# uzh-rpg/ess

Measured on AMD Instinct MI355X. Metric: UDA train-step throughput (voxel grids/s = N*B*T/step_time), higher is better.
Workload: dtype f16 forward / bf16 backward

## Files before the change

ess_amd/csrc/conv_bf16.hip:

```cpp
#include "conv_bf16_common.h"
#include <atomic>

namespace {

using namespace essconv;

__global__ void pack_weights_bf16_kernel(const float* w, const float* w2, __bf16* out, int64_t total, int cot, int ck,
                                         int n_chunks, int ks, int cin, int cout, int epi, int hid, int w_kind, int split, int f16) {
  const int64_t i = (int64_t)blockIdx.x * blockDim.x + threadIdx.x;
  if (i >= total) return;
  int64_t t = i;
  const int kp = t & 7; t >>= 3;
  const int col = t % cot; t /= cot;
  const int cb8 = ck >> 3;
  const int cb = t % cb8; t /= cb8;
  const int tap = t % (ks * ks); t /= ks * ks;
  int lo = 0;
  if (split) { lo = (int)(t & 1); t >>= 1; }
  const int ch = t % n_chunks;
  const int ct = t / n_chunks;
  const int c = ch * ck + cb * 8 + kp;
  int sel;
  const int row = map_row(ct * cot + col, epi, hid, cout, &sel);
  float v = 0.f;
// ... 339 lines not shown
    const size_t lds2 = 2 * (size_t)pl.lds_bytes;
    WidePick wp;
    if (wide_pick(d, pl, g, a, c8, &wp)) {
      ConvKArgs t = a;
      t.tiles_x = wp.tiles_x; t.n_tiles = wp.tiles_x * wp.tiles_y;
      const int cus = tuning().cus;
      t.persist = wp.tiles > cus ? 1 : 0;
      t.slab = pl.cout_tile;
      conv_bf16_launch_wide(wp.mbw, wp.cw, d->epilogue, dim3((unsigned)(wp.tiles > cus ? cus : wp.tiles)), st, t);
      return ess_launch_status("conv2d_forward(bf16, wide tile)");
    }
    if (lds2 <= 160 * 1024) {
      static const int persist = [] { const char* e = getenv("ESS_WS_PERSIST"); return e ? atoi(e) : 1; }();
      const int per_cu_lds = (int)((160 * 1024) / lds2), per_cu = (mb == 4 ? 1 : 2) < per_cu_lds ? (mb == 4 ? 1 : 2) : per_cu_lds;
      const int slots = tuning().cus * per_cu;
      if (persist && (int)grid.x > slots) {
        ConvKArgs t = a;
        t.persist = 1;
        conv_bf16_launch_ws(mb, d->epilogue, c8, dim3((unsigned)slots), lds2, st, t);
        return ess_launch_status("conv2d_forward(bf16, wave-specialised, persistent)");
      }
      conv_bf16_launch_ws(mb, d->epilogue, c8, grid, lds2, st, a);
      return ess_launch_status("conv2d_forward(bf16, wave-specialised)");
    }
  }
  const int key = d->ksize * 10 + d->stride;
  ESS_CHECK_ARG(!a.split || split_generic, "conv(bf16): split operands reached the generic tile kernel (k%d s%d, %zu B of LDS for two stages)",
                d->ksize, d->stride, 2 * (size_t)pl.lds_bytes);
  if (c8)
    ESS_CHECK_ARG(d->epilogue == ESS_EPI_LINEAR && (key == 11 || key == 12 || key == 31 || key == 32),
                  "conv(bf16): the generic tile kernel stages BF16_C8 sources for 1x1 and 3x3 LINEAR convolutions only");
  ESS_CHECK_ARG(key == 11 || key == 12 || key == 31 || key == 32 || key == 51 || key == 52 || key == 71 || key == 72,
                "conv: no kernel for k%d s%d", d->ksize, d->stride);
  conv_bf16_launch_generic(key, mb, pl.ck / 8, d->epilogue, c8, grid, pl.lds_bytes, st, a);
  return ess_launch_status("conv2d_forward(bf16)");
}

}
```

ess_amd/csrc/conv_bf16_generic.hip:

```cpp
#include "conv_bf16_common.h"

namespace {

using namespace essconv;

template <int KS, int S, int MB, int EPI, int CB8, bool SRCBF = false, bool H = false>
__global__ __launch_bounds__(256) void conv_bf16_kernel(const ConvKArgs a) {
  static_assert(!H || SRCBF, "half operands come as F16_C8 tensors");
  extern __shared__ __attribute__((aligned(16))) u32x4 smem16[];
  constexpr int COT = MB * 32;
  constexpr int CK = CB8 * 8;
  constexpr int KPC = kpc(KS, S);
  constexpr int WSZ = KS * KS * CB8 * COT;
  constexpr int WV = (WSZ + 255) / 256;
  constexpr bool WPRE = WV <= 5;
  const int tid = threadIdx.x, lane = tid & 63, wave = tid >> 6, half = lane >> 5, p = lane & 31;
  const int BW = 1 << a.bwl, WX = 1 << a.wxl, RB = 32 >> a.bwl;
  const int TW = WX << a.bwl, TH = (4 >> a.wxl) * NBW * RB;
  const int logical = xcd_remap(blockIdx.x, gridDim.x);
  const int ct = logical % a.n_cout_tiles;
  const int sp = logical / a.n_cout_tiles;
  const int tile = sp % a.n_tiles, n = sp / a.n_tiles;
  const int ty = tile / a.tiles_x, tx = tile - ty * a.tiles_x;
  const int y0 = ty * TH, x0 = tx * TW;
  u32x4* in_t = smem16;
  u32x4* w_t = smem16 + CB8 * a.plane;

  const int ox = p & (BW - 1), oy = p >> a.bwl;
  const int wx = wave & (WX - 1), wy = wave >> a.wxl;
  const int lx = wx * BW + ox;
  int ly[NBW], boff[NBW];
#pragma unroll
  for (int nb = 0; nb < NBW; ++nb) {
    ly[nb] = (wy * NBW + nb) * RB + oy;
    boff[nb] = half * a.plane + ly[nb] * S * a.row_pitch + lx;
  }

  f32x16 acc[MB][NBW];
#pragma unroll
  for (int mb = 0; mb < MB; ++mb)
#pragma unroll
// ... 33 lines not shown
    }
  }
  struct Raw8 { float v[8]; };
  struct Pre { typename std::conditional<SRCBF, u32x4, Raw8>::type d; };
  const size_t hw0 = pl0 / 4, hw1 = pl1 / 4;
  const int nb0 = (a.C0 + 7) >> 3, nb1 = (a.C1 + 7) >> 3;
  const u32x4* s0 = (const u32x4*)a.src0 + (size_t)n * nb0 * hw0;
  const u32x4* s1 = a.C1 ? (const u32x4*)a.src1 + (size_t)n * nb1 * hw1 : s0;
  auto load_vec = [&](int ch, int cb, int k) -> Pre {
    const int c0 = ch * CK + cb * 8;
    const bool first = c0 < a.C0 || a.C1 == 0;
    Pre r;
    if constexpr (SRCBF) {
      const int bi = (first ? c0 : c0 - a.C0) >> 3, nbs = first ? nb0 : nb1;
      const u32x4* sp = (first ? s0 : s1) + (size_t)(bi < nbs ? bi : 0) * (first ? hw0 : hw1);
      r.d = sp[first ? v_o0[k] : v_o1[k]];
    } else {
      const unsigned pls = first ? pl0 : pl1;
      const unsigned cbase = (unsigned)(first ? c0 : c0 - a.C0) * pls;
      const unsigned off = (first ? v_o0[k] : v_o1[k]) + cbase;
#pragma unroll
      for (int j = 0; j < 8; ++j)
        r.d.v[j] = __builtin_bit_cast(float, __builtin_amdgcn_raw_buffer_load_b32(first ? r0 : r1, (int)(off + j * pls), 0, 0));
    }
    return r;
  };
  auto to_lds = [&](int ch, int cb, int k, const Pre& r, bool x_lo = false) -> u32x4 {
    if constexpr (SRCBF) {
      const int c0 = ch * CK + cb * 8;
      const bool first = c0 < a.C0 || a.C1 == 0;
      const unsigned blk_ok = ((first ? c0 : c0 - a.C0) >> 3) < (first ? nb0 : nb1) ? 0xffffffffu : 0u;
      const unsigned m = (first ? v_k0[k] : v_k1[k]) & blk_ok;
      u32x4 v = r.d;
      v[0] &= m; v[1] &= m; v[2] &= m; v[3] &= m;
      return v;
    } else {
      if (x_lo) {
        float lo[8];
#pragma unroll
        for (int j = 0; j < 8; ++j) lo[j] = r.d.v[j] - (float)(__bf16)r.d.v[j];
        return pack8(lo);
      }
      return pack8(r.d.v);
    }
  };

  Pre pre[CB8][KPC];
  u32x4 wpre[WPRE ? WV : 1];
  const bool split = !SRCBF && a.split;
  const int nvc = split ? 3 * a.n_chunks : a.n_chunks;
  const u32x4* wbase = (const u32x4*)a.wpk + (size_t)ct * a.n_chunks * WSZ * (split ? 2 : 1);
  auto wslab = [&](int vc) { return split ? 2 * (vc / 3) + ((vc % 3) == 2 ? 1 : 0) : vc; };
#pragma unroll
  for (int cb = 0; cb < CB8; ++cb)
#pragma unroll
    for (int k = 0; k < KPC; ++k) pre[cb][k] = load_vec(0, cb, k);
  if constexpr (WPRE) {
#pragma unroll
    for (int it = 0; it < WV; ++it) { const int i = tid + it * 256; wpre[it] = wbase[i < WSZ ? i : 0]; }
  }

  for (int vc = 0; vc < nvc; ++vc) {
    const int ch = split ? vc / 3 : vc;
    const bool x_lo = split && (vc - 3 * ch) == 1;
    __syncthreads();
#pragma unroll
// ... 46 lines not shown
#pragma unroll
            for (int nb = 0; nb < NBW; ++nb)
              acc[mb][nb] = ess_mfma16<H>(af[mb], bfr[nb], acc[mb][nb]);
        }
      }
    }
  }
  conv_epilogue<MB, EPI, true, H>(a, acc, ct, n, half, x0 + lx, y0, ly);
}

template <int KS, int S, int MB, int CB8>
void launch_epi(int epi, dim3 grid, size_t lds, hipStream_t st, const ConvKArgs& a) {
  if constexpr (KS == 3 && S == 1) {
    switch (epi) {
      case ESS_EPI_LSTM: { ess_allow_lds(conv_bf16_kernel<KS, S, MB, ESS_EPI_LSTM, CB8>, lds); hipLaunchKernelGGL((conv_bf16_kernel<KS, S, MB, ESS_EPI_LSTM, CB8>), grid, dim3(256), lds, st, a); } return;
      case ESS_EPI_GRU_UR: { ess_allow_lds(conv_bf16_kernel<KS, S, MB, ESS_EPI_GRU_UR, CB8>, lds); hipLaunchKernelGGL((conv_bf16_kernel<KS, S, MB, ESS_EPI_GRU_UR, CB8>), grid, dim3(256), lds, st, a); } return;
      case ESS_EPI_GRU_OUT: { ess_allow_lds(conv_bf16_kernel<KS, S, MB, ESS_EPI_GRU_OUT, CB8>, lds); hipLaunchKernelGGL((conv_bf16_kernel<KS, S, MB, ESS_EPI_GRU_OUT, CB8>), grid, dim3(256), lds, st, a); } return;
      default: break;
    }
  }
  { ess_allow_lds(conv_bf16_kernel<KS, S, MB, ESS_EPI_LINEAR, CB8>, lds); hipLaunchKernelGGL((conv_bf16_kernel<KS, S, MB, ESS_EPI_LINEAR, CB8>), grid, dim3(256), lds, st, a); }
}

template <int KS, int S, int MB, int CB8>
void launch_c8(dim3 grid, size_t lds, hipStream_t st, const ConvKArgs& a) {
  if (a.f16) {
    ess_allow_lds(conv_bf16_kernel<KS, S, MB, ESS_EPI_LINEAR, CB8, true, true>, lds);
    hipLaunchKernelGGL((conv_bf16_kernel<KS, S, MB, ESS_EPI_LINEAR, CB8, true, true>), grid, dim3(256), lds, st, a);
    return;
  }
  ess_allow_lds(conv_bf16_kernel<KS, S, MB, ESS_EPI_LINEAR, CB8, true>, lds);
  hipLaunchKernelGGL((conv_bf16_kernel<KS, S, MB, ESS_EPI_LINEAR, CB8, true>), grid, dim3(256), lds, st, a);
}
template <int KS, int S>
void launch_mb_c8(int mb, int cb8, dim3 grid, size_t lds, hipStream_t st, const ConvKArgs& a) {
  if constexpr (KS == 1 && S == 1) {
    if (cb8 == 4) {
      if (mb == 2) launch_c8<KS, S, 2, 4>(grid, lds, st, a);
      else launch_c8<KS, S, 1, 4>(grid, lds, st, a);
      return;
    }
  }
  if (mb == 2) launch_c8<KS, S, 2, 2>(grid, lds, st, a);
  else launch_c8<KS, S, 1, 2>(grid, lds, st, a);
}

template <int KS, int S>
void launch_mb(int mb, int cb8, int epi, dim3 grid, size_t lds, hipStream_t st, const ConvKArgs& a) {
  if constexpr (KS == 1 && S == 1) {
    if (cb8 == 4) {
      if (mb == 2) launch_epi<KS, S, 2, 4>(epi, grid, lds, st, a);
      else launch_epi<KS, S, 1, 4>(epi, grid, lds, st, a);
      return;
    }
  }
  if (mb == 2) launch_epi<KS, S, 2, 2>(epi, grid, lds, st, a);
  else launch_epi<KS, S, 1, 2>(epi, grid, lds, st, a);
}
}

namespace essconv {

void conv_bf16_launch_generic(int key, int mb, int cb8, int epi, bool c8, dim3 grid, size_t lds, hipStream_t st, const ConvKArgs& a) {
  if (c8) {
    switch (key) {
      case 11: launch_mb_c8<1, 1>(mb, cb8, grid, lds, st, a); break;
      case 12: launch_mb_c8<1, 2>(mb, cb8, grid, lds, st, a); break;
      case 31: launch_mb_c8<3, 1>(mb, cb8, grid, lds, st, a); break;
      default: launch_mb_c8<3, 2>(mb, cb8, grid, lds, st, a); break;
// ... 17 lines not shown
```

ess_amd/csrc/conv_common.h:

```cpp
#pragma once
#include "common.h"
#include <stdlib.h>

#ifndef ESS_EPI_AUX
#define ESS_EPI_AUX 2
#endif
#ifndef ESS_GRU_AUX
#define ESS_GRU_AUX 2
#endif
#ifndef ESS_C8_AUX
#define ESS_C8_AUX 0
#endif
namespace essconv {

constexpr int NBW = 2;

struct ConvKArgs {
  const float* src0;
  const float* src1;
  const void* wpk;
  const float* scale;
  const float* shift;
  const float* residual;
  const float* aux0;
  const float* aux1;
  float* out;
  float* out2;
  int N, Hin, Win, C0, C1, mode0, mode1;
  int Cout, Hout, Wout, pad;
  int bwl, wxl, tiles_x, n_tiles, n_cout_tiles;
  int IH, IW, row_pitch, par_off, plane;
  int ck, n_chunks;
  int act, hid, out_split;
  void* out_bf;
  int fmt0, fmt1;
  int fmt_out;
  int fmt_res;
  int out_f16;
  int persist;
  int slab;
  int split;
  int deep;
  int f16;
  int hilo;
};

template <bool H> __device__ __forceinline__ uint2 ess_cvt4(float v0, float v1, float v2, float v3);
template <bool H> __device__ __forceinline__ void ess_up4(uint2 r, float (&f)[4]);


#ifndef ESS_EPI_STAMP
#define ESS_EPI_STAMP(i_) do { } while (0)
#endif
typedef __amdgpu_buffer_rsrc_t ess_rsrc;
constexpr unsigned ESS_OOB = 0x80000000u;
__device__ __forceinline__ ess_rsrc ess_make_rsrc(const void* p, size_t bytes) {
  return __builtin_amdgcn_make_buffer_rsrc((void*)p, 0, (int)(unsigned)bytes, 0x00020000);
}
__device__ __forceinline__ _Float16 ess_f16_sat(float v) {
  const float c = __builtin_amdgcn_fmed3f(v, -65504.f, 65504.f);
  return (_Float16)(v != v ? v : c);
}
template <> __device__ __forceinline__ uint2 ess_cvt4<false>(float v0, float v1, float v2, float v3) {
  typedef __bf16 bf16x4 __attribute__((ext_vector_type(4)));
  bf16x4 b;
  b[0] = (__bf16)v0; b[1] = (__bf16)v1; b[2] = (__bf16)v2; b[3] = (__bf16)v3;
  return __builtin_bit_cast(uint2, b);
}
template <> __device__ __forceinline__ uint2 ess_cvt4<true>(float v0, float v1, float v2, float v3) {
  typedef _Float16 f16x4 __attribute__((ext_vector_type(4)));
  f16x4 h;
  h[0] = ess_f16_sat(v0); h[1] = ess_f16_sat(v1); h[2] = ess_f16_sat(v2); h[3] = ess_f16_sat(v3);
  return __builtin_bit_cast(uint2, h);
}
__device__ __forceinline__ uint2 ess_cvt4_lo(float v0, float v1, float v2, float v3) {
  typedef _Float16 f16x4 __attribute__((ext_vector_type(4)));
  f16x4 h;
// ... 1253 lines not shown
          if (S == 1) {
            int rp = IW;
            if (BW == 16) while (rp & 15) ++rp;
            if (BW == 8) while ((rp & 15) != 8) ++rp;
            g.row_pitch = rp; g.par_off = 0;
          } else {
            int pw = (IW + 1) / 2;
            if (BW == 16) while (pw & 3) ++pw;
            if (BW == 8) while ((pw & 3) != 2) ++pw;
            g.row_pitch = 2 * pw; g.par_off = pw;
          }
          g.plane = IH * g.row_pitch;
        } else {
          if (S == 1) {
            int rp = IW;
            if (BW < 32) while ((rp & 31) != BW) ++rp;
            g.row_pitch = rp; g.par_off = 0;
          } else {
            int pw = (IW + 1) / 2;
            if (BW < 32) while (((4 * pw) & 31) != BW) ++pw;
            g.row_pitch = 2 * pw; g.par_off = pw;
          }
          g.plane = (IH * g.row_pitch + 3) & ~3;
        }
        best = g;
      }
    }
  }
  return best;
}

inline int validate(const EssConvDesc* d) {
  ESS_CHECK_ARG(d != nullptr, "conv: null descriptor");
  if (d->compute == ESS_COMPUTE_F16) {
    ESS_CHECK_ARG(d->fmt0 != ESS_FMT_BF16_C8 && d->fmt1 != ESS_FMT_BF16_C8 && d->fmt_out != ESS_FMT_BF16_C8 && d->fmt_res != ESS_FMT_BF16_C8,
                  "conv(f16): 16-bit tensors of a half-operand convolution are ESS_FMT_F16_C8");
    ESS_CHECK_ARG(d->act != ESS_ACT_SUMPOOL2 || d->epilogue != ESS_EPI_LINEAR, "conv(f16): no pooled (data-gradient) form");
    ESS_CHECK_ARG(d->mode0 != ESS_SRC_ZERO_UP2 && d->mode1 != ESS_SRC_ZERO_UP2, "conv(f16): no zero-inserted sources");
    if (d->epilogue == ESS_EPI_LINEAR && d->fmt_out == ESS_FMT_F16_C8_HILO) {
      ESS_CHECK_ARG(d->out_split == 0 && (d->act == ESS_ACT_NONE || d->act == ESS_ACT_RELU) && (d->C_out % 64) == 0,
                    "conv(f16): a [hi | lo] output needs act in {none, relu}, no out_split, C_out %% 64 == 0");
      const ResolvedDesc rt = resolve_compute(d);
      const int cot = pick_mb(&rt.d) * 32;
      ESS_CHECK_ARG((d->C_out % cot) == 0, "conv(f16): a [hi | lo] output needs whole channel tiles: C_out %d is not a multiple of the plan's %d-channel tile",
                    d->C_out, cot);
    }
    if (d->epilogue == ESS_EPI_LSTM) ESS_CHECK_ARG(d->act == 0 || d->act == ESS_LSTM_H_HILO, "conv(f16, LSTM): act is 0 or ESS_LSTM_H_HILO");
    if (d->epilogue == ESS_EPI_GRU_UR) ESS_CHECK_ARG(d->act == ESS_GRU_U_F32 || d->act == ESS_GRU_U_F16, "conv(f16, GRU_UR): act is ESS_GRU_U_F32 or ESS_GRU_U_F16");
    const ResolvedDesc r = resolve_compute(d);
    return validate(&r.d);
  }
  ESS_CHECK_ARG(d->fmt_out != ESS_FMT_F16_C8_HILO, "conv: ESS_FMT_F16_C8_HILO is an output format of ESS_COMPUTE_F16");
  ESS_CHECK_ARG(d->N > 0 && d->H_in > 0 && d->W_in > 0 && d->C0 > 0 && d->C1 >= 0 && d->C_out > 0, "conv: bad extents");
  ESS_CHECK_ARG(d->ksize == 1 || d->ksize == 3 || d->ksize == 5 || d->ksize == 7, "conv: ksize %d unsupported", d->ksize);
  ESS_CHECK_ARG(d->stride == 1 || d->stride == 2, "conv: stride %d unsupported", d->stride);
  ESS_CHECK_ARG(d->H_out == (d->H_in + 2 * d->pad - d->ksize) / d->stride + 1 &&
                    d->W_out == (d->W_in + 2 * d->pad - d->ksize) / d->stride + 1,
                "conv: output extent %dx%d inconsistent with input %dx%d k%d s%d p%d", d->H_out, d->W_out, d->H_in,
                d->W_in, d->ksize, d->stride, d->pad);
  for (int s = 0; s < 2; ++s) {
    const int m = s ? d->mode1 : d->mode0;
    ESS_CHECK_ARG(m >= 0 && m <= (s ? 2 : 3), "conv: bad source mode");
    if (m == ESS_SRC_NEAREST_UP2 || m == ESS_SRC_ZERO_UP2) ESS_CHECK_ARG(!(d->H_in & 1) && !(d->W_in & 1), "conv: x2 source needs even extent");
  }
  if (d->mode0 == ESS_SRC_S2D)
    ESS_CHECK_ARG(d->ksize == 3 && d->stride == 1 && d->pad == 1 && d->C1 == 0 && (d->C0 % 128) == 0 && (d->C_out % 64) == 0 &&
// ... 150 lines not shown
```

ess_amd/csrc/conv_fwd.hip:

```cpp
#include "conv_common.h"

namespace {

using namespace essconv;

constexpr int kpc32(int ks, int s) { return stage_kpc(ks, s); }
constexpr unsigned OOB32 = 0x80000000u;

template <int KS, int S, int MB, int EPI, int CB>
__global__ __launch_bounds__(256) void conv_f32_kernel(const ConvKArgs a) {
  extern __shared__ __attribute__((aligned(16))) float smem[];
  constexpr int COT = MB * 32;
  constexpr int KPC = kpc32(KS, S);
  constexpr int WSZ = KS * KS * CB * COT;
  constexpr int WV = (WSZ / 4 + 255) / 256;
  const int tid = threadIdx.x, lane = tid & 63, wave = tid >> 6, half = lane >> 5, p = lane & 31;
  const int BW = 1 << a.bwl, WX = 1 << a.wxl, RB = 32 >> a.bwl;
  const int TW = WX << a.bwl, TH = (4 >> a.wxl) * NBW * RB;
  const int logical = xcd_remap(blockIdx.x, gridDim.x);
  const int ct = logical % a.n_cout_tiles;
  const int sp = logical / a.n_cout_tiles;
  const int tile = sp % a.n_tiles, n = sp / a.n_tiles;
  const int ty = tile / a.tiles_x, tx = tile - ty * a.tiles_x;
  const int y0 = ty * TH, x0 = tx * TW;
// ... 157 lines not shown
  const ResolvedDesc rd = resolve_compute(d);
  d = &rd.d;
  EssConvPlan pl;
  make_plan(d, &pl, rd.split);
  if (is_bf16(d)) return conv_bf16_pack_weights(d, pl, w_kind, w, w2, packed, (hipStream_t)stream, rd.split, rd.f16);
  const int64_t total = pl.packed_elems;
  hipLaunchKernelGGL(pack_weights_kernel, dim3((unsigned)ceil_div64(total, 256)), dim3(256), 0, (hipStream_t)stream, w, w2,
                     (float*)packed, total, pl.cout_tile, pl.ck, pl.n_chunks, d->ksize, d->C0 + d->C1, d->C_out, d->epilogue,
                     d->hidden, w_kind);
  return ess_launch_status("pack_weights");
}

extern "C" int ess_conv2d_pack_weights_multi(const EssConvDesc* descs, const int32_t* w_kinds, const float* const* w,
                                             void* const* packed, int32_t count, ess_stream_t stream) {
  ESS_CHECK_ARG(descs && w_kinds && w && packed && count > 0, "pack_weights_multi: bad arguments");
  return conv_bf16_pack_weights_multi(descs, w_kinds, w, packed, count, (hipStream_t)stream);
}

extern "C" int ess_conv2d_pack_rows(const EssConvDesc* d, const float* v, const float* v2, float fill, float* packed,
                                    ess_stream_t stream) {
  int rc = validate(d);
  if (rc) return rc;
  ESS_CHECK_ARG(v && packed, "pack_rows: null pointer");
  ESS_CHECK_ARG(d->epilogue != ESS_EPI_GRU_UR || v2, "pack_rows: GRU_UR needs the reset-gate vector as v2");
  const ResolvedDesc rd = resolve_compute(d);
  d = &rd.d;
  EssConvPlan pl;
  make_plan(d, &pl, rd.split);
  hipLaunchKernelGGL(pack_rows_kernel, dim3(ceil_div(pl.rows_padded, 256)), dim3(256), 0, (hipStream_t)stream, v, v2, fill,
                     packed, pl.rows_padded, d->epilogue, d->hidden, d->C_out);
  return ess_launch_status("pack_rows");
}

extern "C" int ess_conv2d_forward(const EssConvDesc* d, const void* src0, const void* src1, const void* packed_w,
                                  const float* scale, const float* shift, const void* residual, const float* aux0,
                                  const float* aux1, void* out, void* out2, void* out_bf16, ess_stream_t stream) {
  EssConvDesc dcopy;
  bool out_f16 = false;
  if (d && d->fmt_out == ESS_FMT_F16_C8 && d->compute != ESS_COMPUTE_F16) {
    ESS_CHECK_ARG(d->act != ESS_ACT_SUMPOOL2 && d->out_split == 0 && (d->fmt_res == ESS_FMT_F32_NCHW || d->fmt_res == ESS_FMT_BF16_C8),
                  "conv: an F16_C8 output takes no SUMPOOL2 / out_split; a residual comes as BF16_C8");
    dcopy = *d;
    dcopy.fmt_out = ESS_FMT_BF16_C8;
    if (residual) dcopy.fmt_res = ESS_FMT_BF16_C8;
    d = &dcopy;
    out_f16 = true;
  }
  int rc = validate(d);
  if (rc) return rc;
  const ResolvedDesc rd = resolve_compute(d);
  d = &rd.d;
  ESS_CHECK_ARG(src0 && packed_w, "conv: null pointer");
  ESS_CHECK_ARG(d->mode0 != ESS_SRC_S2D || (d->fmt0 == ESS_FMT_BF16_C8 && d->fmt_out == ESS_FMT_BF16_C8), "conv: an ESS_SRC_S2D source is a BF16_C8 tensor, and so is the output");
  ESS_CHECK_ARG(out || (out_bf16 && d->out_split == 0 && (d->epilogue == ESS_EPI_LINEAR || d->epilogue == ESS_EPI_LSTM || d->epilogue == ESS_EPI_GRU_OUT)),
                "conv: `out` may only be NULL when the BF16_C8 copy is requested (LINEAR / LSTM / GRU_OUT epilogues)");
  ESS_CHECK_ARG(d->C1 == 0 || src1, "conv: second source missing");
  if (d->epilogue != ESS_EPI_LINEAR) ESS_CHECK_ARG(shift && !scale && !residual, "conv: a recurrent epilogue takes a bias (shift) and no scale / residual");
  if (d->epilogue == ESS_EPI_LSTM) ESS_CHECK_ARG(out2, "conv: the LSTM epilogue needs the second output (c')");
  if (d->epilogue == ESS_EPI_GRU_UR) ESS_CHECK_ARG(out2 || out_bf16 || !aux0, "conv: GRU_UR needs an output for r*h (out2 or out_bf16)");
  if (d->epilogue == ESS_EPI_GRU_OUT) ESS_CHECK_ARG(aux1, "conv: GRU_OUT needs u (aux1); h_prev (aux0) may be NULL = zeros");
  if (d->out_split > 0) ESS_CHECK_ARG(out2, "conv: out_split needs out2");
  if (out_bf16)
    ESS_CHECK_ARG(d->compute == ESS_COMPUTE_BF16 && d->out_split == 0, "conv: the BF16_C8 output copy exists for bf16 compute, no out_split");
  if (d->act == ESS_ACT_SUMPOOL2)
    ESS_CHECK_ARG(out && !scale && !residual && !out_bf16, "conv: SUMPOOL2 takes no scale / residual / BF16_C8 copy");
  if (d->fmt_out == ESS_FMT_BF16_C8) {
    ESS_CHECK_ARG(out && !out_bf16, "conv: a BF16_C8 output goes to `out` (no separate copy)");
    ESS_CHECK_ARG(((((uintptr_t)out) | ((uintptr_t)out2) | ((uintptr_t)residual)) & 15) == 0, "conv: BF16_C8 tensors must be 16-byte aligned");
  }
  ESS_CHECK_ARG(!residual || d->fmt_res == d->fmt_out, "conv: the residual must come in the output's format");
  EssConvPlan pl;
  make_plan(d, &pl, rd.split);
  ESS_CHECK_ARG(pl.lds_bytes <= 160 * 1024, "conv: LDS tile %d B exceeds 160 KiB", pl.lds_bytes);
  if (d->epilogue == ESS_EPI_GRU_UR && d->act == ESS_GRU_U_F16 && d->fmt_out == ESS_FMT_F32_C8)
    ESS_CHECK_ARG(shift && d->fmt0 == ESS_FMT_BF16_C8 && (d->hidden % (pl.cout_tile / 2)) == 0 && out && !out2 && (!aux0 || d->fmt_res == ESS_FMT_F32_C8),
                  "conv(GRU_UR): an F16_C8 update gate (ESS_GRU_U_F16 with channel-blocked outputs) needs BF16_C8 sources, a bias, hidden %% %d == 0, "
                  "no fp32 r*h output and a channel-blocked h_prev", pl.cout_tile / 2);
  const Geom g = choose_geom(d);
  ConvKArgs a{};
  a.src0 = (const float*)src0; a.src1 = (const float*)src1; a.wpk = packed_w;
  a.out_bf = out_bf16; a.fmt0 = d->fmt0; a.fmt1 = d->C1 ? d->fmt1 : d->fmt0; a.scale = scale; a.shift = shift; a.residual = (const float*)residual;
  a.aux0 = aux0; a.aux1 = aux1; a.out = (float*)out; a.out2 = (float*)out2; a.fmt_out = d->fmt_out; a.fmt_res = d->fmt_res;
#ifdef ESS_ABLATE
  { static const int abl = [] { const char* b = getenv("ESS_WS_ABL"); return b ? atoi(b) & ~1 : 0; }(); a.deep = abl; }
#endif
  a.out_f16 = out_f16 ? 1 : 0;
  a.split = rd.split ? 1 : 0;
  a.f16 = rd.f16 ? 1 : 0;
  a.hilo = rd.hilo ? 1 : 0;
  if (rd.hilo && d->epilogue == ESS_EPI_LINEAR)
    ESS_CHECK_ARG(!residual && (d->C_out % pl.cout_tile) == 0 && d->fmt_out == ESS_FMT_BF16_C8, "conv(f16): a [hi | lo] output takes no residual and whole channel tiles");
  if (rd.hilo && d->epilogue == ESS_EPI_GRU_OUT)
    ESS_CHECK_ARG(out_bf16 && shift && d->fmt_res == ESS_FMT_F32_C8 && aux1 && (!out || d->fmt_out == ESS_FMT_F32_C8) && (d->hidden % pl.cout_tile) == 0,
                  "conv(f16, GRU_OUT): a [hi | lo] copy of h' exists in the straight-line form only (channel-blocked states, whole tiles of hidden channels)");
  if (rd.hilo && d->epilogue == ESS_EPI_LSTM)
    ESS_CHECK_ARG(out_bf16 && shift && d->fmt_out == ESS_FMT_F32_C8 && (!aux0 || d->fmt_res == ESS_FMT_F32_C8) && (d->hidden % (8 * (pl.cout_tile / 32))) == 0 && pl.cout_tile >= 64,
                  "conv(f16, LSTM): a [hi | lo] copy of h' exists in the lean form only (channel-blocked cell states, whole hidden blocks per tile)");
  a.N = d->N; a.Hin = d->H_in; a.Win = d->W_in; a.C0 = d->C0; a.C1 = d->C1; a.mode0 = d->mode0; a.mode1 = d->mode1;
  a.Cout = d->C_out; a.Hout = d->H_out; a.Wout = d->W_out; a.pad = d->pad;
  a.bwl = g.bwl; a.wxl = g.wxl; a.tiles_x = g.tiles_x; a.n_tiles = g.tiles_x * g.tiles_y; a.n_cout_tiles = pl.n_cout_tiles;
  a.IH = g.IH; a.IW = g.IW; a.row_pitch = g.row_pitch; a.par_off = g.par_off; a.plane = g.plane;
  a.ck = pl.ck; a.n_chunks = pl.n_chunks; a.act = d->act; a.hid = d->hidden; a.out_split = d->out_split;
  hipStream_t st = (hipStream_t)stream;
  if (is_bf16(d)) return conv_bf16_launch(d, pl, g, a, st);
  ESS_CHECK_ARG(g.IH * g.IW <= kpc32(d->ksize, d->stride) * 256, "conv: input tile of %d positions exceeds the staging capacity",
                g.IH * g.IW);
  ESS_CHECK_ARG((int64_t)(d->C0 > d->C1 ? d->C0 : d->C1) * d->H_in * d->W_in * 4 < (int64_t)1 << 31,
                "conv: one sample of a source must stay below 2 GiB (32-bit buffer offsets)");
  const dim3 grid((unsigned)(g.tiles_x * g.tiles_y * pl.n_cout_tiles * d->N));
  const int mb = pl.cout_tile / 32;
  const int key = d->ksize * 10 + d->stride;
  switch (key) {
    case 11: launch_mb<1, 1>(mb, pl.ck, d->epilogue, grid, pl.lds_bytes, st, a); break;
    case 12: launch_mb<1, 2>(mb, pl.ck, d->epilogue, grid, pl.lds_bytes, st, a); break;
    case 31: launch_mb<3, 1>(mb, pl.ck, d->epilogue, grid, pl.lds_bytes, st, a); break;
    case 32: launch_mb<3, 2>(mb, pl.ck, d->epilogue, grid, pl.lds_bytes, st, a); break;
    case 51: launch_mb<5, 1>(mb, pl.ck, d->epilogue, grid, pl.lds_bytes, st, a); break;
    case 52: launch_mb<5, 2>(mb, pl.ck, d->epilogue, grid, pl.lds_bytes, st, a); break;
    case 71: launch_mb<7, 1>(mb, pl.ck, d->epilogue, grid, pl.lds_bytes, st, a); break;
    case 72: launch_mb<7, 2>(mb, pl.ck, d->epilogue, grid, pl.lds_bytes, st, a); break;
    default: ess_set_error("conv: no kernel for k%d s%d", d->ksize, d->stride); return ESS_ENOTSUP;
  }
  return ess_launch_status("conv2d_forward");
}
```

ess_amd/csrc/conv_wgrad.hip:

```cpp
#include "conv_wgrad_common.h"
#include <stdlib.h>

namespace {


__device__ __forceinline__ float load_virtual(const WgradArgs& a, int n, int c, int gy, int gx) {
  const bool first = c < a.C0;
  const int mode = first ? a.mode0 : a.mode1;
  const int sh = mode != ESS_SRC_DIRECT ? 1 : 0;
  const int Hp = a.Hin >> sh, Wp = a.Win >> sh;
  const float* sp = first ? a.src0 : a.src1;
  const int cc = first ? c : c - a.C0, Cs = first ? a.C0 : a.C1;
  const bool ok = gy >= 0 && gy < a.Hin && gx >= 0 && gx < a.Win && !(mode == ESS_SRC_ZERO_UP2 && ((gy | gx) & 1));
  const int cy = min(max(gy, 0), a.Hin - 1) >> sh, cx = min(max(gx, 0), a.Win - 1) >> sh;
  const float t = sp[(((size_t)n * Cs + cc) * Hp + cy) * Wp + cx];
  return ok ? t : 0.f;
}

__device__ __forceinline__ void load8_virtual(const WgradArgs& a, int n, int c, int gy, int gx, bool valid, float (&f)[8]) {
  const bool first = c < a.C0;
  const int mode = first ? a.mode0 : a.mode1;
  const float* sp = first ? a.src0 : a.src1;
  const int cc = first ? c : c - a.C0, Cs = first ? a.C0 : a.C1;
  const bool rowok = valid && gy >= 0 && gy < a.Hin;
// ... 762 lines not shown
struct WPlan {
  EssConvDesc d;
  WRoute route;
  bool phases;
  WgradBArgs args;
  unsigned grid;
  int lds_bytes;
  size_t ws_bytes;
};

inline bool k3s1p1(const EssConvDesc* d) { return d->ksize == 3 && d->stride == 1 && d->pad == 1; }

inline bool s2_phases(const EssConvDesc* d) {
  return d->fmt0 == ESS_FMT_BF16_C8 && d->fmt_out == ESS_FMT_BF16_C8 && d->ksize == 3 && d->stride == 2 && d->pad == 1 && d->C1 == 0 &&
         d->mode0 == ESS_SRC_DIRECT && d->H_in == 2 * d->H_out && d->W_in == 2 * d->W_out;
}
inline EssConvDesc s2_phase_desc(const EssConvDesc* d) {
  EssConvDesc p = *d;
  p.stride = 1; p.H_in = d->H_out; p.W_in = d->W_out; p.mode1 = ESS_SRC_DIRECT;
  return p;
}
inline TapMap s2_phase_taps(int p, int q) {
  TapMap tm{};
  tm.mapped = 1;
  for (int t = 0; t < 9; ++t) {
    const int kyp = t / 3, kxp = t % 3;
    const int ky = p == 0 ? (kyp == 1 ? 1 : -1) : (kyp == 0 ? 0 : kyp == 1 ? 2 : -1);
    const int kx = q == 0 ? (kxp == 1 ? 1 : -1) : (kxp == 0 ? 0 : kxp == 1 ? 2 : -1);
    tm.m[t] = (signed char)((ky < 0 || kx < 0) ? -1 : ky * 3 + kx);
  }
  return tm;
}

int wvalidate(const EssConvDesc* d) {
  ESS_CHECK_ARG(d != nullptr, "wgrad: null descriptor");
  ESS_CHECK_ARG(d->epilogue == ESS_EPI_LINEAR && d->out_split == 0, "wgrad: only plain convolutions have a weight gradient here");
  ESS_CHECK_ARG(d->mode0 >= ESS_SRC_DIRECT && d->mode0 <= ESS_SRC_ZERO_UP2 && d->mode1 >= ESS_SRC_DIRECT && d->mode1 <= ESS_SRC_ZERO_UP2,
                "wgrad: source modes DIRECT / NEAREST_UP2 / ZERO_UP2 only (the space-to-depth form exists for the frozen encoder's forward)");
  const int cin = d->C0 + d->C1;
  const bool taps = cin == 1 && d->ksize == 7;
  ESS_CHECK_ARG(taps || d->ksize == 1 || d->ksize == 3, "wgrad: k=%d with C_in=%d unsupported", d->ksize, cin);
  ESS_CHECK_ARG(d->stride == 1 || d->stride == 2, "wgrad: stride %d unsupported", d->stride);
  const bool xc8 = d->fmt0 == ESS_FMT_BF16_C8, dc8 = d->fmt_out == ESS_FMT_BF16_C8;
  ESS_CHECK_ARG(d->compute == ESS_COMPUTE_FP32 || d->compute == ESS_COMPUTE_BF16 || d->compute == ESS_COMPUTE_BF16X3, "wgrad: bad compute type");
  if (xc8 || dc8) {
    ESS_CHECK_ARG(d->compute == ESS_COMPUTE_BF16, "wgrad: BF16_C8 tensors need bf16 compute");
    ESS_CHECK_ARG(d->C1 == 0 || d->fmt1 == d->fmt0, "wgrad: both sources of a concat must use the same format");
    ESS_CHECK_ARG(d->C1 == 0 || (d->C0 % 8) == 0, "wgrad: the first BF16_C8 source of a concat must have a multiple of 8 channels");
    if (xc8 && dc8)
      ESS_CHECK_ARG(k3s1p1(d) || (d->ksize == 1 && d->pad == 0 && d->mode0 == ESS_SRC_DIRECT && d->C1 == 0) || s2_phases(d),
                    "wgrad(BF16_C8): 3x3 / stride 1 / pad 1, 3x3 / stride 2 / pad 1 on even extents (one direct source) and 1x1 / pad 0 convolutions only");
    else if (xc8)
      ESS_CHECK_ARG(d->ksize == 1 && d->stride == 1 && d->pad == 0 && d->C1 == 0 && d->mode0 == ESS_SRC_DIRECT && d->C_out <= 32 && cin <= 32,
                    "wgrad(BF16_C8 X, fp32 dY): the 1x1 head only (C_in, C_out <= 32)");
    else
      ESS_CHECK_ARG(taps, "wgrad(fp32 X, BF16_C8 dY): the 7x7 single-channel stem only");
  }
  return ESS_OK;
}

WRoute wroute(const EssConvDesc* d) {
  const int cin = d->C0 + d->C1, KS = d->ksize;
  const bool xc8 = d->fmt0 == ESS_FMT_BF16_C8, dc8 = d->fmt_out == ESS_FMT_BF16_C8;
  if (xc8 && dc8) return KS == 3 ? W_C8_K3 : W_C8_K1;
  if (xc8) return W_SMALL1X1_C8X;
  const bool k1s1p0 = KS == 1 && d->stride == 1 && d->pad == 0;
  if (k1s1p0 && d->C1 == 0 && d->mode0 == ESS_SRC_DIRECT && d->C_out <= 16 && cin <= 64)
    return cin <= 32 && ((d->H_out * d->W_out) % 64) == 0 ? W_SMALL1X1_MFMA : W_SMALL1X1;
  const bool rows8 = (d->W_in % 8) == 0 && (d->W_out % 8) == 0 && d->mode0 != ESS_SRC_ZERO_UP2 && d->mode1 != ESS_SRC_ZERO_UP2;
  if (d->compute == ESS_COMPUTE_BF16 && k3s1p1(d)) return rows8 ? W_BF16_K3_FAST : W_BF16_K3;
  if (d->compute == ESS_COMPUTE_BF16 && k1s1p0 && rows8) return W_BF16_K1;
  if (cin == 1 && KS == 7) return W_TAPS7;
  return W_F32_TILE;
}

WPlan wplan(const EssConvDesc* desc) {
  WPlan w{};
  w.d = *desc;
  if (desc->compute == ESS_COMPUTE_BF16X3) {
    w.args.split = k3s1p1(desc);
    w.d.compute = w.args.split ? ESS_COMPUTE_BF16 : ESS_COMPUTE_FP32;
  }
  w.phases = s2_phases(&w.d);
  if (w.phases) w.d = s2_phase_desc(&w.d);
  const EssConvDesc* d = &w.d;
  w.route = wroute(d);
  WgradArgs& a = w.args.w;
  a.N = d->N; a.Hin = d->H_in; a.Win = d->W_in; a.C0 = d->C0; a.C1 = d->C1; a.mode0 = d->mode0; a.mode1 = d->mode1;
  a.Cout = d->C_out; a.Hout = d->H_out; a.Wout = d->W_out;
  a.pad = (w.route == W_BF16_K1 || w.route == W_C8_K1) ? 1 : d->pad;
  a.dy_c8 = d->fmt_out == ESS_FMT_BF16_C8;
  a.ps = w.phases;
  const int cin = d->C0 + d->C1, KS = d->ksize, S = d->stride;
  const bool wide = tile128(w.route);
  const int npx = wide ? 128 : 64;
  double best = 1e300;
  for (int twl = 5; twl >= (wide ? 4 : 3); --twl) {
    const int tw = 1 << twl, th = npx >> twl;
    const double c = (double)ceil_div(d->W_out, tw) * tw * ceil_div(d->H_out, th) * th + 1e-3 * (5 - twl);
    if (c < best) { best = c; a.twl = twl; }
  }
  if (w.route == W_C8_K3) a.twl = 4;
  const int tw = 1 << a.twl, th = npx >> a.twl;
  a.tiles_x = ceil_div(d->W_out, tw); a.tiles_y = ceil_div(d->H_out, th);
  a.ntiles = d->N * a.tiles_x * a.tiles_y;
  a.IH = (th - 1) * S + KS; a.IW = (tw - 1) * S + KS;
  a.plx = (a.IH * a.IW) | 1;
  a.ci_tiles = w.route == W_TAPS7 ? 1 : ceil_div(cin, 64);
  a.npairs = ceil_div(d->C_out, 64) * a.ci_tiles;
  const size_t slab_floats = (size_t)KS * KS * d->C_out * cin + d->C_out;
  int ns = wide ? ceil_div(256, a.npairs) : ceil_div(2048, a.npairs);
  if (ns > a.ntiles) ns = a.ntiles;
  const size_t cap = ((size_t)64 << 20) / (slab_floats * 4);
  if ((size_t)ns > cap) ns = (int)(cap ? cap : 1);
  if (ns < 1) ns = 1;
  if (w.route == W_SMALL1X1 || w.route == W_SMALL1X1_C8X) {
    const int chunks = d->N * ceil_div(d->H_out * d->W_out, 128);
    ns = chunks < 1024 ? chunks : 1024;
  } else if (w.route == W_SMALL1X1_MFMA) {
    const int groups = d->N * (d->H_out * d->W_out / 64);
    ns = groups < 4 * 512 ? ceil_div(groups, 4) : 512;
  }
  a.nsplit = ns;
  w.grid = (unsigned)(a.npairs * ns);
  w.ws_bytes = (size_t)ns * slab_floats * 4;
  w.lds_bytes = (64 * 65 + (w.route == W_TAPS7 ? a.IH * a.IW : 64 * a.plx)) * 4;
  if (wide) {
    w.args.rv = tw / 8 + 2;
    w.args.pyv = (th * tw / 8) | 1;
    w.args.pxv = ((th + 2) * w.args.rv) | 1;
    w.lds_bytes = 64 * (w.args.pyv + w.args.pxv) * 16 * (w.route == W_BF16_K3 ? 1 : 2);
  }
  return w;
}

struct WgradSet { const void* x0; const void* x1; const void* dy; };

WgradBArgs wfill(const WPlan& w, const WgradSet& s, void* workspace, bool bias, int ph) {
  WgradBArgs b = w.args;
  WgradArgs& a = b.w;
  a.src0 = (const float*)s.x0; a.src1 = a.C1 ? (const float*)s.x1 : nullptr; a.dy = (const float*)s.dy;
  a.ws = (float*)workspace;
  a.ws_b = bias ? a.ws + (size_t)a.nsplit * w.d.ksize * w.d.ksize * a.Cout * (a.C0 + a.C1) : nullptr;
  a.pp = ph >> 1; a.pq = ph & 1;
  return b;
}

template <typename K, typename... A>
int wgo(K kernel, dim3 grid, int lds_bytes, hipStream_t st, const A&... args) {
  const int rc = wgrad_raise_lds(kernel, lds_bytes);
  if (rc) return rc;
  hipLaunchKernelGGL(kernel, grid, dim3(256), lds_bytes, st, args...);
  return ESS_OK;
}

int wlaunch(const WPlan& w, WRoute route, const WgradBArgs& b, hipStream_t st) {
  const EssConvDesc& d = w.d;
  const dim3 grid(w.grid);
  const int px = d.H_out * d.W_out, nsplit = b.w.nsplit;
  int rc = ESS_OK;
  switch (route) {
    case W_F32_TILE: {
      const auto kernel = d.ksize == 3 ? (d.stride == 1 ? wgrad_f32_kernel<3, 1> : wgrad_f32_kernel<3, 2>)
                                       : (d.stride == 1 ? wgrad_f32_kernel<1, 1> : wgrad_f32_kernel<1, 2>);
      rc = wgo(kernel, grid, w.lds_bytes, st, b.w);
      break;
    }
    case W_TAPS7: rc = wgo(wgrad_taps_kernel<7, 2>, grid, w.lds_bytes, st, b.w); break;
    case W_BF16_K3: rc = wgo(wgrad_bf16_k3s1_kernel, grid, w.lds_bytes, st, b); break;
    case W_BF16_K3_FAST: rc = wgo(wgrad_bf16_k3s1_fast_kernel<9>, grid, w.lds_bytes, st, b); break;
    case W_BF16_K1: rc = wgo(wgrad_bf16_k3s1_fast_kernel<1>, grid, w.lds_bytes, st, b); break;
    case W_C8_K3: rc = wgrad_c8_k3_launch(b, grid, st); break;
    case W_C8_K1: rc = wgrad_c8_k1_launch(b, d.stride, w.lds_bytes, grid, st); break;
    case W_SMALL1X1: rc = wgo(wgrad_small1x1_kernel, dim3(nsplit), 0, st, b.w, ceil_div(px, 128), d.N * ceil_div(px, 128)); break;
// ... 29 lines not shown
  EssConvDesc c = *d;
  c.compute = ESS_COMPUTE_BF16;
  c.fmt0 = c.fmt1 = c.fmt_out = ESS_FMT_BF16_C8;
  return c;
}
struct SplitCopy { int C, H, W; size_t bytes; };
struct SplitLayout { size_t slabs, total; SplitCopy t[3]; };
SplitLayout split_layout(const EssConvDesc* d) {
  const EssConvDesc dc = c8_desc(d);
  const int s0 = d->mode0 != ESS_SRC_DIRECT ? 1 : 0, s1 = d->mode1 != ESS_SRC_DIRECT ? 1 : 0;
  SplitLayout s{(wplan(&dc).ws_bytes + 255) & ~(size_t)255, 0,
                {{d->C0, d->H_in >> s0, d->W_in >> s0, 0}, {d->C1, d->H_in >> s1, d->W_in >> s1, 0}, {d->C_out, d->H_out, d->W_out, 0}}};
  s.total = s.slabs;
  for (SplitCopy& t : s.t) {
    t.bytes = (((size_t)d->N * ((t.C + 7) / 8) * t.H * t.W * 16) + 255) & ~(size_t)255;
    s.total += 2 * t.bytes;
  }
  return s;
}

int wgrad_split_via_c8(const EssConvDesc* d, const WgradSet& s, float* dw, float* db, int accumulate, void* workspace, size_t workspace_bytes,
                       hipStream_t st);

int wgrad_run(const EssConvDesc* d, int n_sets, const WgradSet* sets, int bias_mask, float* dw, float* db, int accumulate, void* workspace,
              size_t workspace_bytes, hipStream_t st) {
  int rc = wvalidate(d);
  if (rc) return rc;
  ESS_CHECK_ARG(dw && workspace, "wgrad: null pointer");
  uintptr_t bits = 0;
  for (int q = 0; q < n_sets; ++q) {
    ESS_CHECK_ARG(sets[q].x0 && sets[q].dy, "wgrad: null pointer");
    ESS_CHECK_ARG(d->C1 == 0 || sets[q].x1, "wgrad: second source missing");
    bits |= (uintptr_t)sets[q].x0 | (uintptr_t)sets[q].dy | (d->C1 ? (uintptr_t)sets[q].x1 : 0);
  }
  if (split_via_c8(d)) {
    for (int q = 0; q < n_sets; ++q)
      if ((rc = wgrad_split_via_c8(d, sets[q], dw, ((bias_mask >> q) & 1) ? db : nullptr, q ? 1 : accumulate, workspace, workspace_bytes, st))) return rc;
    return ESS_OK;
  }
  const WPlan w = wplan(d);
  ESS_CHECK_ARG(workspace_bytes >= w.ws_bytes, "wgrad: workspace too small");
  ESS_CHECK_ARG(w.lds_bytes <= 160 * 1024, "wgrad: LDS tile %d B too large", w.lds_bytes);
  if (w.d.fmt0 == ESS_FMT_BF16_C8 || w.d.fmt_out == ESS_FMT_BF16_C8)
    ESS_CHECK_ARG((bits & 15) == 0, "wgrad: BF16_C8 tensors must be 16-byte aligned");
  if (w.route == W_TAPS7) {
    ESS_CHECK_ARG(w.d.stride == 2, "wgrad: 7x7 stem variant is stride 2 only");
    ESS_CHECK_ARG(!db, "wgrad: the stem variant has no bias gradient");
  }
  const bool one_launch = n_sets > 1 && w.route == W_C8_K3 && !w.phases;
  for (int q = 0; q < (one_launch ? 1 : n_sets); ++q) {
    const bool misaligned = (((uintptr_t)sets[q].x0 | (uintptr_t)sets[q].dy) & 15) != 0;
    const WRoute route = (w.route == W_SMALL1X1_MFMA && misaligned) ? W_SMALL1X1 : w.route;
    for (int ph = 0; ph < (w.phases ? 4 : 1); ++ph) {
      const bool bias = db && ph == 0 && (one_launch || ((bias_mask >> q) & 1));
      WgradBArgs b = wfill(w, sets[q], workspace, bias, ph);
      if (one_launch) {
        b.npass = n_sets; b.bias_mask = bias_mask;
        for (int i = 0; i < n_sets; ++i) { b.p_dy[i] = sets[i].dy; b.p_x0[i] = sets[i].x0; b.p_x1[i] = d->C1 ? sets[i].x1 : nullptr; }
      }
      if ((rc = wlaunch(w, route, b, st))) return rc;
      if ((rc = wreduce(w, b.w, dw, db, (q || accumulate) ? 1 : 0, w.phases ? s2_phase_taps(ph >> 1, ph & 1) : TapMap{}, st))) return rc;
    }
  }
  return ESS_OK;
}

int wgrad_split_via_c8(const EssConvDesc* d, const WgradSet& s, float* dw, float* db, int accumulate, void* workspace,
                              size_t workspace_bytes, hipStream_t st) {
  int rc;
  ESS_CHECK_ARG((((uintptr_t)workspace) & 255) == 0, "wgrad: the workspace must be 256-byte aligned");
  const SplitLayout sl = split_layout(d);
  ESS_CHECK_ARG(workspace_bytes >= sl.total, "wgrad: workspace too small");
  const void* src[3] = {s.x0, s.x1, s.dy};
  char* hi[3]; char* lo[3];
  char* p = (char*)workspace + sl.slabs;
  for (int i = 0; i < 3; ++i) {
    const SplitCopy& t = sl.t[i];
    hi[i] = p; lo[i] = p + t.bytes; p += 2 * t.bytes;
    if (t.C && (rc = ess_split_bf16_c8_internal((const float*)src[i], hi[i], lo[i], d->N, t.C, t.H, t.W, st))) return rc;
  }
  const EssConvDesc dc = c8_desc(d);
  const WgradSet sets[3] = {{hi[0], hi[1], hi[2]}, {lo[0], lo[1], hi[2]}, {hi[0], hi[1], lo[2]}};
  const int bias_mask = 0b101;
  static const bool fused = env_on("ESS_X3_WGRAD_FUSED");
  if (fused) return wgrad_run(&dc, 3, sets, bias_mask, dw, db, accumulate, workspace, sl.slabs, st);
  for (int q = 0; q < 3; ++q)
    if ((rc = wgrad_run(&dc, 1, &sets[q], (bias_mask >> q) & 1, dw, db, q ? 1 : accumulate, workspace, sl.slabs, st))) return rc;
  return ESS_OK;
}

}

extern "C" size_t ess_conv2d_wgrad_workspace(const EssConvDesc* d) {
  if (wvalidate(d)) return 0;
  return split_via_c8(d) ? split_layout(d).total : wplan(d).ws_bytes;
}

extern "C" int ess_conv2d_wgrad(const EssConvDesc* d, const void* src0, const void* src1, const void* dy, float* dw, float* db,
                                int accumulate, void* workspace, size_t workspace_bytes, ess_stream_t stream) {
  const WgradSet s{src0, src1, dy};
  return wgrad_run(d, 1, &s, 1, dw, db, accumulate, workspace, workspace_bytes, (hipStream_t)stream);
}

extern "C" int ess_conv2d_wgrad_sets(const EssConvDesc* d, int32_t n_sets, const void* const* src0, const void* const* src1,
                                     const void* const* dy, float* dw, float* db, int32_t accumulate, void* workspace,
                                     size_t workspace_bytes, ess_stream_t stream) {
  ESS_CHECK_ARG(d && src0 && dy && n_sets >= 1 && n_sets <= 3, "wgrad_sets: 1 to 3 sets");
  WgradSet sets[3];
  for (int q = 0; q < n_sets; ++q) {
    ESS_CHECK_ARG(src0[q] && dy[q] && (d->C1 == 0 || (src1 && src1[q])), "wgrad_sets: null tensor in set %d", q);
    sets[q] = WgradSet{src0[q], d->C1 ? src1[q] : nullptr, dy[q]};
  }
  return wgrad_run(d, n_sets, sets, (1 << n_sets) - 1, dw, db, accumulate, workspace, workspace_bytes, (hipStream_t)stream);
}
```

ess_amd/csrc/conv_wgrad_c8.hip:

```cpp
#include "conv_wgrad_common.h"
#include <stdlib.h>
#include <type_traits>

namespace {

struct Quad { u32x4w v[4]; };

__device__ __forceinline__ void quad_transpose(const Quad& q, uint2 (&out)[8]) {
#pragma unroll
  for (int d = 0; d < 4; ++d) {
    out[2 * d].x = __builtin_amdgcn_perm(q.v[1][d], q.v[0][d], 0x05040100u);
    out[2 * d].y = __builtin_amdgcn_perm(q.v[3][d], q.v[2][d], 0x05040100u);
    out[2 * d + 1].x = __builtin_amdgcn_perm(q.v[1][d], q.v[0][d], 0x07060302u);
    out[2 * d + 1].y = __builtin_amdgcn_perm(q.v[3][d], q.v[2][d], 0x07060302u);
  }
}

template <int OFF>
__device__ __forceinline__ void lds_read128(u32x4w& d, unsigned addr) {
  asm volatile("ds_read_b128 %0, %1 offset:%2" : "=v"(d) : "v"(addr), "n"(OFF));
}

template <int TAPS, int TWL>
__global__ __launch_bounds__(256) void wgrad_c8_kernel(const WgradBArgs b, int sx_abl) {
// ... 433 lines not shown
    unit(std::integral_constant<int, 22>{}, Yes{});
    unit(std::integral_constant<int, 23>{}, Yes{});
    a_addr = a_next;
    x_addr = x_next;
  }
  if (ntl > 0) {
    if (ntl - 1 < 30) ESS_TR(3 + ntl - 1);
    if (b.npass > 1) want_b = want_b0 && ((b.bias_mask >> ((split + (ntl - 1) * nsplit) / a.ntiles)) & 1);
    static_for<0, 24>([&](auto uc) { unit(uc, No{}); });
  }
  ESS_TR(34);
  const int ci = cit * 64 + ib * 32 + p, co0 = cot * 64 + cb * 32 + 4 * half;
  float* wsp = a.ws + ((size_t)split * 9 * a.Cout + co0) * Cin + ci;
  const int tap_stride = a.Cout * Cin;
  if (ci < Cin) {
#pragma unroll
    for (int r = 0; r < 16; ++r) {
      const int dco = (r & 3) + 8 * (r >> 2);
      if (co0 + dco < a.Cout) {
        float* q = wsp + dco * Cin;
#pragma unroll
        for (int t = 0; t < 9; ++t) q[t * tap_stride] = acc[t][r];
      }
    }
  }
  if (want_b) {
    bsum += __shfl_xor(bsum, 32, 64);
    const int co = cot * 64 + cb * 32 + p;
    if (half == 0 && co < a.Cout) a.ws_b[(size_t)split * a.Cout + co] = bsum;
  }
  ESS_TR(37);
}

__global__ __launch_bounds__(256) void wgrad_small1x1_c8_kernel(const WgradArgs a, int chunks_per_img, int total_chunks) {
  constexpr int P = 128, PP = P + 1;
  __shared__ float dy_s[32 * PP];
  __shared__ float x_s[32 * PP];
  float* red = dy_s;
  const int tid = threadIdx.x, lane = tid & 63, wave = tid >> 6, half = lane >> 5, p = lane & 31;
  const int Cin = a.C0, Cout = a.Cout, nbi = (Cin + 7) >> 3;
  const size_t HW = (size_t)a.Hout * a.Wout;
  f32x16 acc;
#pragma unroll
  for (int r = 0; r < 16; ++r) acc[r] = 0.f;
  float bsum = 0.f;
  for (int i = tid; i < 32 * PP; i += 256) { dy_s[i] = 0.f; x_s[i] = 0.f; }
  for (int chunk = blockIdx.x; chunk < total_chunks; chunk += gridDim.x) {
    const int n = chunk / chunks_per_img;
    const size_t px0 = (size_t)(chunk - n * chunks_per_img) * P;
    __syncthreads();
    for (int i = tid; i < nbi * P; i += 256) {
      const int blk = i / P, j = i - blk * P;
      const size_t px = px0 + j;
      const u32x4w v = ((const u32x4w*)a.src0)[((size_t)n * nbi + blk) * HW + (px < HW ? px : HW - 1)];
      const unsigned m = px < HW ? 0xffffffffu : 0u;
#pragma unroll
      for (int q = 0; q < 4; ++q) {
        x_s[(blk * 8 + 2 * q) * PP + j] = __builtin_bit_cast(float, (v[q] << 16) & m);
        x_s[(blk * 8 + 2 * q + 1) * PP + j] = __builtin_bit_cast(float, v[q] & 0xffff0000u & m);
      }
    }
    for (int i = tid; i < Cout * P; i += 256) {
      const int r = i / P, j = i - r * P;
      const size_t px = px0 + j;
      const float t = a.dy[((size_t)n * Cout + r) * HW + (px < HW ? px : HW - 1)];
      dy_s[r * PP + j] = px < HW ? t : 0.f;
    }
    __syncthreads();
    const float* dp = dy_s + p * PP + wave * 32 + half;
    const float* xp = x_s + p * PP + wave * 32 + half;
#pragma unroll 8
    for (int kk = 0; kk < 16; ++kk) {
      const float d1 = dp[2 * kk], x1 = xp[2 * kk];
      bsum += d1;
      acc = __builtin_amdgcn_mfma_f32_32x32x2f32(d1, x1, acc, 0, 0, 0);
    }
  }
  __syncthreads();
  float* redb = x_s;
#pragma unroll
  for (int r = 0; r < 16; ++r) red[wave * 1024 + r * 64 + lane] = acc[r];
  bsum += __shfl_xor(bsum, 32, 64);
  if (half == 0) redb[wave * 32 + p] = bsum;
  __syncthreads();
  for (int i = tid; i < 16 * 64; i += 256) {
    const int r = i >> 6, l = i & 63;
    const int co = (r & 3) + 8 * (r >> 2) + 4 * (l >> 5), ci = l & 31;
    if (co < Cout && ci < Cin)
      a.ws[(size_t)blockIdx.x * Cout * Cin + co * Cin + ci] = (red[i] + red[1024 + i]) + (red[2048 + i] + red[3072 + i]);
  }
  if (a.ws_b && tid < Cout) a.ws_b[(size_t)blockIdx.x * Cout + tid] = (redb[tid] + redb[32 + tid]) + (redb[64 + tid] + redb[96 + tid]);
}

}

int wgrad_c8_k3_launch(const WgradBArgs& b, dim3 grid, hipStream_t st) {
  if (b.w.twl != 4) { ess_set_error("wgrad(BF16_C8, 3x3): stride 1, 16-wide pixel tiles"); return ESS_EINVAL; }
  constexpr int NST = 4, lds = NST * DmaGeom::STAGE;
  static_assert(lds <= 160 * 1024, "LDS stages of the weight-gradient kernel");
  const int rc = wgrad_raise_lds(wgrad_c8_ws_kernel<NST>, lds);
  if (rc) return rc;
  hipLaunchKernelGGL((wgrad_c8_ws_kernel<NST>), grid, dim3(512), lds, st, b);
  return ess_launch_status("conv2d_wgrad(BF16_C8, LDS-DMA, loader waves)");
}

int wgrad_c8_k1_launch(const WgradBArgs& b, int sx, int lds_bytes, dim3 grid, hipStream_t st) {
  if (b.w.twl != 4 && b.w.twl != 5) { ess_set_error("wgrad(BF16_C8): pixel tiles are 16 or 32 wide"); return ESS_EINVAL; }
  const auto kernel = b.w.twl == 5 ? wgrad_c8_kernel<1, 5> : wgrad_c8_kernel<1, 4>;
  const int rc = wgrad_raise_lds(kernel, lds_bytes);
  if (rc) return rc;
  hipLaunchKernelGGL(kernel, grid, dim3(256), lds_bytes, st, b, sx);
  return ess_launch_status("conv2d_wgrad(BF16_C8)");
}

int wgrad_small1x1_c8_launch(const WgradArgs& a, int nsplit, hipStream_t st) {
  const int per_img = ceil_div(a.Hout * a.Wout, 128);
  hipLaunchKernelGGL(wgrad_small1x1_c8_kernel, dim3(nsplit), dim3(256), 0, st, a, per_img, a.N * per_img);
  return ess_launch_status("conv2d_wgrad(1x1 head, BF16_C8)");
}

#ifdef ESS_WG_TRACE
extern "C" int ess_debug_wgrad_trace(unsigned long long* host_out, size_t n) {
  return (int)hipMemcpyFromSymbol(host_out, HIP_SYMBOL(g_wg_trace), n * sizeof(unsigned long long));
}
#endif
```

ess_amd/csrc/conv_wgrad_common.h:

```cpp
#pragma once
#include "common.h"

struct WgradArgs {
  const float* src0;
  const float* src1;
  const float* dy;
  float* ws;
  float* ws_b;
  int N, Hin, Win, C0, C1, mode0, mode1, Cout, Hout, Wout, pad;
  int twl;
  int tiles_x, tiles_y, ntiles;
  int IH, IW, plx;
  int ci_tiles, npairs, nsplit;
  int dy_c8;
  int ps, pp, pq;
};

constexpr unsigned OOBW = 0x80000000u;
typedef __bf16 bf16x8w __attribute__((ext_vector_type(8)));
typedef unsigned int u32x4w __attribute__((ext_vector_type(4)));


__device__ __forceinline__ u32x4w cvt8(const float (&v)[8]) {
  bf16x8w b;
#pragma unroll
  for (int j = 0; j < 8; ++j) b[j] = (__bf16)v[j];
  return __builtin_bit_cast(u32x4w, b);
}
__device__ __forceinline__ u32x4w cvt8_lo(const float (&v)[8]) {
  bf16x8w b;
#pragma unroll
  for (int j = 0; j < 8; ++j) b[j] = (__bf16)(v[j] - (float)(__bf16)v[j]);
  return __builtin_bit_cast(u32x4w, b);
}
__device__ __forceinline__ u32x4w shift_left1(u32x4w lo, u32x4w hi) {
  u32x4w r;
  r[0] = __builtin_amdgcn_alignbyte(hi[0], lo[3], 2);
  r[1] = __builtin_amdgcn_alignbyte(hi[1], hi[0], 2);
  r[2] = __builtin_amdgcn_alignbyte(hi[2], hi[1], 2);
  r[3] = __builtin_amdgcn_alignbyte(hi[3], hi[2], 2);
  return r;
}
__device__ __forceinline__ u32x4w shift_right1(u32x4w lo, u32x4w hi) {
  u32x4w r;
  r[0] = __builtin_amdgcn_alignbyte(lo[1], lo[0], 2);
  r[1] = __builtin_amdgcn_alignbyte(lo[2], lo[1], 2);
  r[2] = __builtin_amdgcn_alignbyte(lo[3], lo[2], 2);
  r[3] = __builtin_amdgcn_alignbyte(hi[0], lo[3], 2);
// ... 32 lines not shown
```

ess_amd/csrc/norm_c8.hip:

```cpp
#include <atomic>
#include "common.h"
#include <stdlib.h>

#ifndef ESS_REDUCE1_U
#define ESS_REDUCE1_U 4
#endif
namespace {

typedef unsigned int u32x4n __attribute__((ext_vector_type(4)));
typedef __bf16 bf16x8n __attribute__((ext_vector_type(8)));

__device__ __forceinline__ void unpack8(u32x4n v, float (&f)[8]) {
#pragma unroll
  for (int q = 0; q < 4; ++q) {
    f[2 * q] = __builtin_bit_cast(float, v[q] << 16);
    f[2 * q + 1] = __builtin_bit_cast(float, v[q] & 0xffff0000u);
  }
}
__device__ __forceinline__ void unpack8h(u32x4n v, float (&f)[8]) {
  typedef _Float16 f16x2n __attribute__((ext_vector_type(2)));
#pragma unroll
  for (int q = 0; q < 4; ++q) {
    const unsigned w = v[q];
    const f16x2n h = __builtin_bit_cast(f16x2n, w);
// ... 389 lines not shown
  for (int j = 0; j < 8; ++j) {
    const double a = wave_sum_d(s0[j]), b = wave_sum_d(s1[j]);
    if (lane == 0) { redd[w * 16 + 2 * j] = a; redd[w * 16 + 2 * j + 1] = b; }
  }
  __syncthreads();
  if (threadIdx.x < 16) {
    double t = 0;
    for (int i = 0; i < 4; ++i) t += redd[i * 16 + threadIdx.x];
    sums[((size_t)g * nsl + sl) * 16 + threadIdx.x] = t;
  }
}

__device__ __forceinline__ void group_total8(const double* sums, int g, int nsl, double (&t0)[8], double (&t1)[8]) {
  __shared__ double part[64 * 16];
  __shared__ double tot[16];
  const int j = threadIdx.x & 15, k0 = threadIdx.x >> 4, ng = blockDim.x >> 4;
  {
    const double* p = sums + (size_t)g * nsl * 16 + j;
    double t = 0;
    for (int k = k0; k < nsl; k += ng) t += p[(size_t)k * 16];
    part[k0 * 16 + j] = t;
  }
  __syncthreads();
  if (threadIdx.x < 16) {
    double t = 0;
    for (int i = 0; i < ng; ++i) t += part[i * 16 + threadIdx.x];
    tot[threadIdx.x] = t;
  }
  __syncthreads();
#pragma unroll
  for (int jj = 0; jj < 8; ++jj) { t0[jj] = tot[2 * jj]; t1[jj] = tot[2 * jj + 1]; }
}

__global__ __launch_bounds__(256) void in_apply_c8_kernel(const u32x4n* __restrict__ x, const u32x4n* __restrict__ res,
                                                          u32x4n* __restrict__ y, float* __restrict__ stats, const double* sums,
                                                          int nsl, int CB, int C, int hw, float eps, int relu) {
  const int xf16 = relu >> 8;
  relu &= 0xff;
  const int g = blockIdx.x, n = g / CB, cb = g - n * CB;
  double t0[8], t1[8];
  group_total8(sums, g, nsl, t0, t1);
  float mean[8], rstd[8];
#pragma unroll
  for (int j = 0; j < 8; ++j) {
    const double m = t0[j] / hw;
    double var = t1[j] / hw - m * m;
    if (var < 0) var = 0;
    mean[j] = (float)m;
    rstd[j] = (float)(1.0 / sqrt(var + (double)eps));
  }
  if (blockIdx.y == 0 && threadIdx.x == 0) {
#pragma unroll
    for (int j = 0; j < 8; ++j)
      if (cb * 8 + j < C) { stats[2 * ((size_t)n * C + cb * 8 + j)] = mean[j]; stats[2 * ((size_t)n * C + cb * 8 + j) + 1] = rstd[j]; }
  }
  const size_t base = (size_t)g * hw;
  constexpr int U = 4;
  const int stride = gridDim.y * 256;
  for (int i = blockIdx.y * 256 + threadIdx.x; i < hw; i += stride * U) {
    u32x4n xv[U], rv[U];
#pragma unroll
    for (int u = 0; u < U; ++u) {
      const int ii = i + u * stride, ic = ii < hw ? ii : hw - 1;
      xv[u] = x[base + ic];
      if (res) rv[u] = res[base + ic];
    }
#pragma unroll
    for (int u = 0; u < U; ++u) {
      const int ii = i + u * stride;
      if (ii >= hw) continue;
      float f[8], rf[8];
      unpack8x(xv[u], f, xf16);
      if (res) unpack8(rv[u], rf);
#pragma unroll
      for (int j = 0; j < 8; ++j) {
        float t = (f[j] - mean[j]) * rstd[j];
        if (relu) t = fmaxf(t, 0.f);
        if (res) t += rf[j];
        f[j] = cb * 8 + j < C ? t : 0.f;
      }
      y[base + ii] = pack8n(f);
    }
  }
}

__global__ __launch_bounds__(256) void in_apply_c8_mix_kernel(const u32x4n* __restrict__ x, const u32x4n* __restrict__ res,
                                                              u32x4n* __restrict__ y, u32x4n* __restrict__ y16, float* __restrict__ stats,
                                                              const double* sums, int nsl, int CB, int C, int hw, float eps, int flags) {
  const int relu = flags & 1, xf16 = (flags >> 8) & 1, rf16 = (flags >> 9) & 1, hilo = (flags >> 10) & 1, rpair = (flags >> 11) & 1;
  const int g = blockIdx.x, n = g / CB, cb = g - n * CB;
  double t0[8], t1[8];
  group_total8(sums, g, nsl, t0, t1);
  float mean[8], rstd[8];
#pragma unroll
  for (int j = 0; j < 8; ++j) {
    const double m = t0[j] / hw;
    double var = t1[j] / hw - m * m;
    if (var < 0) var = 0;
    mean[j] = (float)m;
    rstd[j] = (float)(1.0 / sqrt(var + (double)eps));
  }
  if (blockIdx.y == 0 && threadIdx.x == 0) {
#pragma unroll
    for (int j = 0; j < 8; ++j)
      if (cb * 8 + j < C) { stats[2 * ((size_t)n * C + cb * 8 + j)] = mean[j]; stats[2 * ((size_t)n * C + cb * 8 + j) + 1] = rstd[j]; }
  }
  const size_t base = (size_t)g * hw;
  const size_t xbase = hilo ? ((size_t)n * 2 * CB + cb) * hw : base, xlo = xbase + (size_t)CB * hw;
  const size_t rbase = rpair ? ((size_t)n * 2 * CB + cb) * hw : base;
  constexpr int U = 4;
  const int stride = gridDim.y * 256;
  for (int i = blockIdx.y * 256 + threadIdx.x; i < hw; i += stride * U) {
    u32x4n xv[U], rv[U], xl[U];
#pragma unroll
    for (int u = 0; u < U; ++u) {
      const int ii = i + u * stride, ic = ii < hw ? ii : hw - 1;
      xv[u] = x[xbase + ic];
      if (hilo) xl[u] = x[xlo + ic];
      if (res) rv[u] = res[rbase + ic];
    }
#pragma unroll
    for (int u = 0; u < U; ++u) {
      const int ii = i + u * stride;
      if (ii >= hw) continue;
      float f[8], rf[8];
      unpack8x(xv[u], f, xf16);
      if (hilo) {
        float l[8];
        unpack8h(xl[u], l);
#pragma unroll
        for (int j = 0; j < 8; ++j) f[j] += l[j];
      }
      if (res) unpack8x(rv[u], rf, rf16);
#pragma unroll
      for (int j = 0; j < 8; ++j) {
        float t = (f[j] - mean[j]) * rstd[j];
        if (relu) t = fmaxf(t, 0.f);
        if (res) t += rf[j];
        f[j] = cb * 8 + j < C ? t : 0.f;
// ... 269 lines not shown
  return ess_launch_status("instnorm_forward_c8(split)");
}

extern "C" int ess_instnorm_forward_c8_mixed(const void* x, const void* residual, void* y, void* y16, float* stats, int32_t N, int32_t C,
                                             int32_t hw, float eps, int32_t relu, int32_t x_fmt, int32_t res_f16, void* workspace,
                                             size_t workspace_bytes, ess_stream_t stream) {
  ESS_CHECK_ARG(x && y16 && stats && N > 0 && C > 0 && hw > 0, "instnorm_forward_c8_mixed: bad arguments");
  ESS_CHECK_ARG(relu == 0 || relu == 1, "instnorm_forward_c8_mixed: relu must be 0 or 1");
  ESS_CHECK_ARG(x_fmt >= 0 && x_fmt <= 2, "instnorm_forward_c8_mixed: x_fmt is 0 (BF16_C8), 1 (F16_C8) or 2 (F16_C8 [hi | lo])");
  ESS_CHECK_ARG(res_f16 >= 0 && res_f16 <= 2, "instnorm_forward_c8_mixed: res_f16 is 0 (BF16_C8), 1 (F16_C8) or 2 (a [hi | lo] half pair: its hi parts are added)");
  ESS_CHECK_ARG(al16(x, residual, y, y16), "instnorm_forward_c8_mixed: C8 tensors must be 16-byte aligned");
  hipStream_t st = (hipStream_t)stream;
  const int flags = (relu & 1) | (x_fmt ? 0x100 : 0) | (res_f16 ? 0x200 : 0) | (res_f16 == 2 ? 0x800 : 0);
  const int CB = (C + 7) / 8, groups = N * CB;
  const u32x4n* xs = (const u32x4n*)x; const u32x4n* rs = (const u32x4n*)residual; u32x4n* ys = (u32x4n*)y; u32x4n* hs = (u32x4n*)y16;
  if (hw <= 256 * MAXV) {
    if (x_fmt == 2) {
      if (hw <= 512 * 10) hipLaunchKernelGGL((in_fwd_c8_mix_kernel<512, 10, true>), dim3(groups), dim3(512), 0, st, xs, rs, ys, hs, stats, CB, C, hw, eps, flags);
      else hipLaunchKernelGGL((in_fwd_c8_mix_kernel<256, MAXV, true>), dim3(groups), dim3(256), 0, st, xs, rs, ys, hs, stats, CB, C, hw, eps, flags);
    } else {
      if (hw <= 512 * 10) hipLaunchKernelGGL((in_fwd_c8_mix_kernel<512, 10, false>), dim3(groups), dim3(512), 0, st, xs, rs, ys, hs, stats, CB, C, hw, eps, flags);
      else hipLaunchKernelGGL((in_fwd_c8_mix_kernel<256, MAXV, false>), dim3(groups), dim3(256), 0, st, xs, rs, ys, hs, stats, CB, C, hw, eps, flags);
    }
    return ess_launch_status("instnorm_forward_c8_mixed");
  }
  int rc = need_ws(workspace, ess_norm_workspace_c8(groups), workspace_bytes, "instnorm_forward_c8_mixed");
  if (rc) return rc;
  const int nsl = split_for8(groups, hw);
  hipLaunchKernelGGL((c8_reduce_kernel<0>), dim3(groups, nsl), dim3(256), 0, st, xs, nullptr, nullptr, nullptr, (double*)workspace, hw, 1,
                     0, CB, C, 1, flags & 0x100, 0, nullptr, nullptr, x_fmt == 2 ? 2 * CB : 0);
  hipLaunchKernelGGL(in_apply_c8_mix_kernel, dim3(groups, chunks_for8(groups, hw)), dim3(256), 0, st, xs, rs, ys, hs, stats,
                     (const double*)workspace, nsl, CB, C, hw, eps, flags | (x_fmt == 2 ? 0x400 : 0));
  return ess_launch_status("instnorm_forward_c8_mixed(split)");
}

extern "C" int ess_instnorm_backward_c8(const void* x, const void* dy, const float* stats, void* dx, int32_t N, int32_t C,
                                        int32_t hw, int32_t relu, int32_t x_f16, void* workspace, size_t workspace_bytes, ess_stream_t stream) {
  ESS_CHECK_ARG(x && dy && stats && dx && N > 0 && C > 0 && hw > 0, "instnorm_backward_c8: bad arguments");
  ESS_CHECK_ARG(relu == 0 || relu == 1, "instnorm_backward_c8: relu must be 0 or 1");
  ESS_CHECK_ARG(al16(x, dy, dx), "instnorm_backward_c8: BF16_C8 tensors must be 16-byte aligned");
  hipStream_t st = (hipStream_t)stream;
  ESS_CHECK_ARG(x_f16 >= 0 && x_f16 <= 2, "instnorm_backward_c8: x_f16 is 0 (BF16_C8), 1 (F16_C8) or 2 (a [hi | lo] half pair: its hi parts are read)");
  const int xcb = x_f16 == 2 ? 2 * ((C + 7) / 8) : 0;
  relu = (relu & 1) | (x_f16 ? 0x100 : 0);
  const int CB = (C + 7) / 8, groups = N * CB;
  const u32x4n* xs = (const u32x4n*)x; const u32x4n* gs = (const u32x4n*)dy; u32x4n* ds = (u32x4n*)dx;
  if (hw <= 256 * MAXV) {
    const int th = in_small_threads();
    if (th == 1024 && hw <= 1024 * 5) hipLaunchKernelGGL((in_bwd_c8_kernel<1024, 5>), dim3(groups), dim3(1024), 0, st, xs, gs, stats, ds, CB, C, hw, relu, xcb);
    else if (th == 512 && hw <= 512 * 10) hipLaunchKernelGGL((in_bwd_c8_kernel<512, 10>), dim3(groups), dim3(512), 0, st, xs, gs, stats, ds, CB, C, hw, relu, xcb);
    else hipLaunchKernelGGL((in_bwd_c8_kernel<256, MAXV>), dim3(groups), dim3(256), 0, st, xs, gs, stats, ds, CB, C, hw, relu, xcb);
    return ess_launch_status("instnorm_backward_c8");
  }
  int rc = need_ws(workspace, ess_norm_workspace_c8(groups), workspace_bytes, "instnorm_backward_c8");
  if (rc) return rc;
  const int nsl = split_for8(groups, hw);
  hipLaunchKernelGGL((c8_reduce_kernel<1>), dim3(groups, nsl), dim3(256), 0, st, xs, nullptr, gs, stats, (double*)workspace, hw, 1, 0, CB,
                     C, 1, relu, 0, nullptr, nullptr, xcb);
  hipLaunchKernelGGL(in_bwd_apply_c8_kernel, dim3(groups, chunks_for8(groups, hw)), dim3(256), 0, st, xs, gs, stats,
                     (const double*)workspace, nsl, ds, CB, C, hw, relu, xcb);
  return ess_launch_status("instnorm_backward_c8(split)");
}

extern "C" int ess_batchnorm_train_forward_c8(const void* x, const void* residual, const float* gamma, const float* beta,
                                              float* running_mean, float* running_var, float momentum, float eps, void* y,
                                              float* stats, int32_t N, int32_t C, int32_t hw, int32_t relu, int32_t x_f16, void* workspace,
// ... 40 lines not shown
```

ess_amd/csrc/seg_head.hip:

```cpp
#include "common.h"

namespace {

typedef __bf16 bf16x8 __attribute__((ext_vector_type(8)));
typedef _Float16 f16x8 __attribute__((ext_vector_type(8)));

struct SegHeadArgs {
  const void* x;
  const float* w;
  const float* b;
  const uint8_t* palette;
  uint8_t* labels;
  uint8_t* colour;
  float* conf;
  int N, C, K, Hs, Ws, y0, x0, h, w_, Ho, Wo;
};

template <int FMT>
__device__ __forceinline__ float round_operand(float v) {
  if constexpr (FMT == ESS_FMT_BF16_C8) return (float)(__bf16)v;
  else if constexpr (FMT == ESS_FMT_F16_C8) {
    const float c = __builtin_amdgcn_fmed3f(v, -65504.f, 65504.f);
    return (float)(_Float16)(v != v ? v : c);
  } else return v;
}

constexpr int SH_PALETTE_BYTES = 64 * 3;

__device__ __forceinline__ float exp_nonpos(float x) {
  x = fmaxf(x, -87.3f);
  const float L2E_HI = 1.44269502e+0f, L2E_LO = 1.92596299e-8f;
  const float t = x * L2E_HI;
  const float e = fmaf(x, L2E_HI, -t) + x * L2E_LO;
  const float p = __builtin_amdgcn_exp2f(t);
  return fmaf(p, e * 0.693147181f, p);
}

template <int FMT, int KM>
__global__ __launch_bounds__(256) void seg_head_kernel(const SegHeadArgs a) {
  extern __shared__ float lds[];
  const int CB = (a.C + 7) >> 3, CP = CB * 8;
  float* lw = lds;
  float* lb = lds + KM * CP;
  uint8_t* lp = (uint8_t*)(lb + KM);
  for (int i = threadIdx.x; i < KM * CP; i += blockDim.x) {
    const int cb = i / (KM * 8), k = (i >> 3) % KM, c = cb * 8 + (i & 7);
    lw[i] = (k < a.K && c < a.C) ? round_operand<FMT>(a.w[k * a.C + c]) : 0.f;
  }
  for (int i = threadIdx.x; i < KM; i += blockDim.x) lb[i] = i < a.K ? a.b[i] : -INFINITY;
  if (a.palette)
    for (int i = threadIdx.x; i < a.K * 3; i += blockDim.x) lp[i] = a.palette[i];
  __syncthreads();

  const float sy = (float)a.h / (float)a.Ho, sx = (float)a.w_ / (float)a.Wo;
  const size_t plane = (size_t)a.Hs * a.Ws;
  const size_t total = (size_t)a.N * a.Ho * a.Wo;
  for (size_t i = (size_t)blockIdx.x * blockDim.x + threadIdx.x; i < total; i += (size_t)gridDim.x * blockDim.x) {
    const int ox = (int)(i % a.Wo);
    const size_t r = i / a.Wo;
    const int oy = (int)(r % a.Ho);
    const size_t n = r / a.Ho;
    const int iy = a.y0 + min((int)floorf(oy * sy), a.h - 1), ix = a.x0 + min((int)floorf(ox * sx), a.w_ - 1);
    const size_t px = (size_t)iy * a.Ws + ix;
    float z[KM];
#pragma unroll
    for (int k = 0; k < KM; ++k) z[k] = lb[k];
    for (int cb = 0; cb < CB; ++cb) {
      float v[8];
      if constexpr (FMT == ESS_FMT_F32_NCHW) {
        const float* xp = (const float*)a.x + (n * a.C + (size_t)cb * 8) * plane + px;
#pragma unroll
        for (int j = 0; j < 8; ++j) v[j] = (cb * 8 + j < a.C) ? xp[(size_t)j * plane] : 0.f;
      } else {
        const uint4 q = ((const uint4*)a.x)[(n * CB + cb) * plane + px];
        if constexpr (FMT == ESS_FMT_BF16_C8) {
          const bf16x8 t = __builtin_bit_cast(bf16x8, q);
#pragma unroll
          for (int j = 0; j < 8; ++j) v[j] = (float)t[j];
        } else {
          const f16x8 t = __builtin_bit_cast(f16x8, q);
#pragma unroll
          for (int j = 0; j < 8; ++j) v[j] = (float)t[j];
        }
      }
      const float* wr = lw + cb * (KM * 8);
#pragma unroll
      for (int k = 0; k < KM; ++k) {
        const f32x4 w0 = *(const f32x4*)(wr + k * 8), w1 = *(const f32x4*)(wr + k * 8 + 4);
        float s = z[k];
        s = fmaf(w0[0], v[0], s);
        s = fmaf(w0[1], v[1], s);
        s = fmaf(w0[2], v[2], s);
        s = fmaf(w0[3], v[3], s);
        s = fmaf(w1[0], v[4], s);
        s = fmaf(w1[1], v[5], s);
        s = fmaf(w1[2], v[6], s);
        s = fmaf(w1[3], v[7], s);
        z[k] = s;
      }
    }
    float best = z[0];
    int bi = 0;
#pragma unroll
    for (int k = 1; k < KM; ++k)
      if (z[k] > best) { best = z[k]; bi = k; }
    a.labels[i] = (uint8_t)bi;
    if (a.colour) {
      uint8_t* cp = a.colour + i * 3;
      cp[0] = lp[bi * 3];
      cp[1] = lp[bi * 3 + 1];
      cp[2] = lp[bi * 3 + 2];
    }
    if (a.conf) {
      float s = 0.f;
#pragma unroll
      for (int k = 0; k < KM; ++k) s += exp_nonpos(z[k] - best);
      a.conf[i] = 1.0f / s;
    }
  }
}

inline unsigned wave_uniform_grid(size_t total, int cap) {
  size_t g = (total + 255) / 256;
  if (g > (size_t)cap) g = cap;
  return (unsigned)(g < 1 ? 1 : g);
}

inline int km_of(int K) { return K <= 4 ? 4 : K <= 8 ? 8 : K <= 12 ? 12 : K <= 16 ? 16 : K <= 20 ? 20 : K <= 32 ? 32 : 64; }
inline size_t lds_of(int K, int C) { return (size_t)km_of(K) * (((C + 7) >> 3) * 8) * 4 + (size_t)km_of(K) * 4 + SH_PALETTE_BYTES; }

template <int FMT>
int launch(const SegHeadArgs& a, hipStream_t st) {
  const size_t total = (size_t)a.N * a.Ho * a.Wo;
  const unsigned grid = wave_uniform_grid(total, 2048);
  const size_t lds = lds_of(a.K, a.C);
#define ESS_SH(KM_) hipLaunchKernelGGL((seg_head_kernel<FMT, KM_>), dim3(grid), dim3(256), lds, st, a)
  switch (km_of(a.K)) {
    case 4: ESS_SH(4); break;
    case 8: ESS_SH(8); break;
    case 12: ESS_SH(12); break;
    case 16: ESS_SH(16); break;
    case 20: ESS_SH(20); break;
    case 32: ESS_SH(32); break;
    default: ESS_SH(64); break;
  }
#undef ESS_SH
  return ess_launch_status("seg_head");
}

}

extern "C" int ess_seg_head(const void* x, int32_t fmt, const float* weight, const float* bias, const uint8_t* palette, uint8_t* labels,
                            uint8_t* colour, float* confidence, int32_t N, int32_t C, int32_t K, int32_t H, int32_t W, int32_t win_y0,
                            int32_t win_x0, int32_t win_h, int32_t win_w, int32_t H_out, int32_t W_out, ess_stream_t stream) {
  ESS_CHECK_ARG(x && weight && bias && labels, "seg_head: x, weight, bias and labels are required");
  ESS_CHECK_ARG(fmt == ESS_FMT_F32_NCHW || fmt == ESS_FMT_BF16_C8 || fmt == ESS_FMT_F16_C8, "seg_head: source format %d unsupported", fmt);
  ESS_CHECK_ARG(N > 0 && C > 0 && H > 0 && W > 0 && H_out > 0 && W_out > 0, "seg_head: bad extents N=%d C=%d H=%d W=%d H_out=%d W_out=%d", N, C,
                H, W, H_out, W_out);
  ESS_CHECK_ARG(K > 0 && K <= 64, "seg_head: K=%d unsupported (1..64)", K);
  ESS_CHECK_ARG(C <= 4096 && lds_of(K, C) <= 64 * 1024, "seg_head: K=%d x C=%d weights do not fit 64 KiB of LDS", K, C);
  ESS_CHECK_ARG(win_y0 >= 0 && win_x0 >= 0 && win_h > 0 && win_w > 0 && (int64_t)win_y0 + win_h <= H && (int64_t)win_x0 + win_w <= W,
                "seg_head: window (%d, %d, %d, %d) leaves the %d x %d plane", win_y0, win_x0, win_h, win_w, H, W);
  ESS_CHECK_ARG(!colour || palette, "seg_head: colour needs a palette");
  ESS_CHECK_ARG(fmt == ESS_FMT_F32_NCHW || ((uintptr_t)x & 15) == 0, "seg_head: a C8 source must be 16-byte aligned");
  SegHeadArgs a{x, weight, bias, palette, labels, colour, confidence, N, C, K, H, W, win_y0, win_x0, win_h, win_w, H_out, W_out};
  hipStream_t st = (hipStream_t)stream;
  if (fmt == ESS_FMT_BF16_C8) return launch<ESS_FMT_BF16_C8>(a, st);
  if (fmt == ESS_FMT_F16_C8) return launch<ESS_FMT_F16_C8>(a, st);
  return launch<ESS_FMT_F32_NCHW>(a, st);
}
```

ess_amd/functional.py:

```python
import os
import weakref

import torch

from . import copies, hip

DIRECT_GRAD_ACCUM = False

class direct_grad_accum:

    def __init__(self, on):
        self.on = bool(on)

    def __enter__(self):
        global DIRECT_GRAD_ACCUM
        self.prev, DIRECT_GRAD_ACCUM = DIRECT_GRAD_ACCUM, self.on

    def __exit__(self, *a):
        global DIRECT_GRAD_ACCUM
        DIRECT_GRAD_ACCUM = self.prev


def _direct(p):
    return DIRECT_GRAD_ACCUM and getattr(p, '_ess_direct_grad', False) and p.is_leaf and p.grad is not None and p.grad.is_contiguous()
# ... 378 lines not shown
                wd, c_dg, split = columns(weight, [(0, C0)]), C0, 0
            pool0 = s == 1 and need0 and mode0 == hip.SRC_NEAREST_UP2 and (C1 == 0 or mode1 == hip.SRC_DIRECT) and \
                not (Hv & 1) and not (Wv & 1)
            if c8in and ((mode0 == hip.SRC_NEAREST_UP2 and need0 and not pool0) or (mode1 == hip.SRC_NEAREST_UP2 and need1)):
                raise hip.EssHipError('Conv2dFn(BF16_C8): only the first source may be nearest-upsampled (pooled data-gradient)')
            if s == 1:
                dspec = hip.conv_spec(N, spec.H_out, spec.W_out, Cout, 0, c_dg, k, 1, k - 1 - p, out_split=split,
                                      act=hip.ACT_SUMPOOL2 if pool0 else hip.ACT_NONE)
            else:
                if (Hv & 1) or (Wv & 1):
                    raise hip.EssHipError('data-gradient of a stride-2 conv needs even input extents')
                dspec = hip.conv_spec(N, 2 * spec.H_out, 2 * spec.W_out, Cout, 0, c_dg, k, 1, k - 1 - p,
                                      mode0=hip.SRC_ZERO_UP2, out_split=split)
            assert (dspec.H_out, dspec.W_out) == (Hv, Wv), (dspec.H_out, dspec.W_out, Hv, Wv)
            dv0 = _empty_act(N, C0, Hv // 2 if (s == 1 and pool0) else Hv, Wv // 2 if (s == 1 and pool0) else Wv, dy.device, c8in)
            dv1 = _empty_act(N, C1, Hv, Wv, dy.device, c8in) if split > 0 else None
            fuse_skip = d_skip is not None and need0 and C1 == 0 and mode0 == hip.SRC_DIRECT
            hip.conv_forward(dspec, dy, None, packed_weight(dspec, wd, kind=hip.W_TRANSPOSED),
                             residual=d_skip.contiguous() if fuse_skip else None, out=dv0, out2=dv1, src_fmt=_fmt(dy),
                             out_fmt=_fmt(dv0))
            if fuse_skip:
                d_skip = None
            if need0:
                d0 = hip.sumpool2x2(dv0) if (mode0 == hip.SRC_NEAREST_UP2 and not (s == 1 and pool0)) else dv0
            if need1:
                d1 = hip.sumpool2x2(dv1) if mode1 == hip.SRC_NEAREST_UP2 else dv1
        if needw or needb:
            dw, db = _weight_gradient(ctx, x0, x1, weight, dy, needw, needb)
        if d_skip is not None and need0:
            d0 = d_skip if d0 is None else (hip.add_bf16(d0, d_skip.contiguous()) if c8in else hip.add(d0, d_skip.contiguous()))
        return d0, d1, dw, db, None, None, None, None, None, None, None


def _weight_gradient(ctx, x0, x1, weight, dy, needw, needb):
    spec = ctx.spec
    (N, Hv, Wv, C0, C1, mode0, mode1, Cout, k, s, p, _, _, _, _, _) = spec.key
    c8in = hip.is_c8(x0)
    even2 = s == 2 and C1 == 0 and mode0 == hip.SRC_DIRECT and not (Hv & 1) and not (Wv & 1)
    phases = even2 and k == 3 and p == 1
    wspec, wx0 = spec, x0
    if even2 and k == 1 and p == 0 and not c8in:
        wspec, wx0 = hip.conv_spec(N, Hv // 2, Wv // 2, C0, 0, Cout, 1, 1, 0), x0[:, :, ::2, ::2].contiguous()
    bias = ctx.bias_ref() if ctx.bias_ref is not None else None
    grads = _direct(weight) and (not needb or (bias is not None and _direct(bias)))
    if needw and grads and not (s == 2 and k == 3 and not (phases and c8in)):
        db_t = bias.grad if needb else None
        defer = WGRAD_DEFER is not None and c8in and hip.is_c8(dy) and k == 3 and s == 1 and p == 1
        held = WGRAD_DEFER.pop(id(weight), None) if defer else None
        if held is not None and held[0].key == spec.key and held[4] is weight:
            hip.conv_wgrad_sets(spec, [(held[1], held[2], held[3]), (x0, x1, dy)], weight.grad, db_t, accumulate=True)
        elif defer and held is None and WGRAD_STASHING:
            WGRAD_DEFER[id(weight)] = (spec, x0, x1, dy, weight, db_t)
            return None, None
        else:
            if held is not None:
                hip.conv_wgrad(held[0], held[1], held[2], held[3], weight.grad, held[5], accumulate=True)
            hip.conv_wgrad(wspec, wx0, x1, dy, weight.grad, db_t, accumulate=True)
        if GRAD_READY_HOOK is not None:
            GRAD_READY_HOOK(weight)
        return None, None
    dw = torch.empty_like(weight)
    db = torch.empty(Cout, dtype=torch.float32, device=dy.device) if ctx.has_bias else None
    if phases and not c8in:
        _wgrad_stride2_by_phases(x0, dy, dw, db)
    else:
        hip.conv_wgrad(wspec, wx0, x1, dy, dw, db)
    if not needw:
        dw = None
    if not needb:
        db = None
    if dw is not None and grads:
        hip.add(weight.grad, dw, out=weight.grad)
        if db is not None:
            hip.add(bias.grad, db, out=bias.grad)
        dw = db = None
        if GRAD_READY_HOOK is not None:
            GRAD_READY_HOOK(weight)
    return dw, db


def _wgrad_stride2_by_phases(x, dy, dw, db):
    N, C, H, W = x.shape[0], _channels(x), x.shape[2], x.shape[3]
    Cout = _channels(dy)
    Ho, Wo = H // 2, W // 2
    spec = hip.conv_spec(N, Ho, Wo, C, 0, Cout, 3, 1, 1)
    tmp = torch.empty_like(dw)
    for p in (0, 1):
        for q in (0, 1):
            hip.conv_wgrad(spec, x[:, :, p::2, q::2].contiguous(), None, dy, tmp, db if (p, q) == (0, 0) else None)
            kys = (1,) if p == 0 else (0, 2)
            kxs = (1,) if q == 0 else (0, 2)
            for ky in kys:
                for kx in kxs:
                    dw[:, :, ky, kx] = tmp[:, :, 0 if ky == 0 else 1, 0 if kx == 0 else 1]


def conv2d(x0, weight, bias=None, stride=1, pad=0, x1=None, mode0=hip.SRC_DIRECT, mode1=hip.SRC_DIRECT, out_c8=None, half=False):
    return Conv2dFn.apply(x0, x1, weight, bias, stride, pad, mode0, mode1, False, out_c8, half)

# ... 16 lines not shown
                if h is not None:
                    res = h[0]
            y, y16, stats = hip.instnorm_forward_c8_mixed(xin, _channels(x), res, relu, eps, x_fmt)
            copies.attach(y, h16=(y16, False))
            ctx.relu, ctx.x_f16 = relu, x_fmt
            ctx.save_for_backward(xin, stats)
            return y
        if _blocked(x):
            y, stats = hip.instnorm_forward_c8(x, _channels(x), residual, relu, eps, x_f16)
        else:
            y, stats = hip.instnorm_forward(x, residual, relu, eps)
        ctx.relu, ctx.x_f16 = relu, x_f16
        ctx.save_for_backward(x, stats)
        return y

    @staticmethod
    def backward(ctx, dy):
        x, stats = ctx.saved_tensors
        dy = dy.contiguous()
        dx = None
        if ctx.needs_input_grad[0]:
            if _blocked(dy):
                dx = hip.instnorm_backward_c8(x, _channels(dy), dy, stats, ctx.relu, ctx.x_f16)
            else:
                dx = hip.instnorm_backward(x, dy, stats, ctx.relu)
        dres = dy if ctx.needs_input_grad[1] else None
        return dx, dres, None, None, None


def instance_norm(x, residual=None, relu=False, eps=1e-5, x_f16=False):
    return InstanceNormFn.apply(x, residual, relu, eps, x_f16)


_MASK_FROM_X = os.environ.get('ESS_BN_MASK_FROM_X', '1') != '0'


class BatchNormTrainFn(torch.autograd.Function):

    @staticmethod
    def forward(ctx, x, residual, gamma, beta, running_mean, running_var, momentum, eps, relu, x_f16=False):
        x_f16 = bool(x_f16) or hip.is_f16_c8(x)
        ctx.x_f16 = x_f16
        if _blocked(x):
            y, stats = hip.batchnorm_train_forward_c8(x, _channels(x), residual, gamma.detach(), beta.detach(), running_mean,
                                                      running_var, momentum, eps, relu, x_f16)
        else:
            y, stats = hip.batchnorm_train_forward(x, residual, gamma.detach(), beta.detach(), running_mean, running_var,
                                                   momentum, eps, relu)
        ctx.relu = relu
        ctx.has_res = residual is not None
        ctx.beta_ref = weakref.ref(beta)
        ctx.save_for_backward(x, y, gamma, stats)
        return y

    @staticmethod
    def backward(ctx, dy):
        x, y, gamma, stats = ctx.saved_tensors
        dy = dy.contiguous()
        need_dx, need_dres, need_g, need_b = ctx.needs_input_grad[0:4]
        beta = ctx.beta_ref()
        if _blocked(x):
            C = _channels(x)
            mask_beta = beta.detach() if (ctx.relu and not ctx.has_res and beta is not None and _MASK_FROM_X) else None
            bwd = lambda *a, **k: hip.batchnorm_train_backward_c8(x, C, *a, x_f16=ctx.x_f16, beta=mask_beta, **k)
        else:
            bwd = lambda *a, **k: hip.batchnorm_train_backward(x, *a, **k)
# ... 106 lines not shown
```

ess_amd/hip.py:

```python
import ctypes
import os
from ctypes import POINTER, Structure, byref, c_char_p, c_float, c_int, c_int32, c_int64, c_size_t, c_void_p

import numpy as np
import torch

from . import copies

_HERE = os.path.dirname(os.path.abspath(__file__))
LIB_PATH = os.path.join(_HERE, 'libess_hip.so')

SRC_DIRECT, SRC_NEAREST_UP2, SRC_ZERO_UP2, SRC_S2D = 0, 1, 2, 3
EPI_LINEAR, EPI_LSTM, EPI_GRU_UR, EPI_GRU_OUT = 0, 1, 2, 3
ACT_NONE, ACT_RELU, ACT_SIGMOID, ACT_TANH, ACT_SUMPOOL2 = 0, 1, 2, 3, 4
W_CONV, W_TRANSPOSED, W_ROWS, W_CONV5_S2D = 0, 1, 2, 3
GRU_U_F32, GRU_U_F16 = 0, 1
COMPUTE_FP32, COMPUTE_BF16, COMPUTE_BF16X3, COMPUTE_F16 = 0, 1, 2, 3
FMT_F32_NCHW, FMT_BF16_C8, FMT_F32_C8, FMT_F16_C8, FMT_F16_C8_HILO = 0, 1, 2, 3, 4
LSTM_H_HILO = 1
GRU_H_HILO = 2

_default_compute = COMPUTE_FP32
_mixed = False


def set_compute(kind):
    global _default_compute, _mixed
    _mixed = kind == 'mixed'
    if _mixed:
        kind = 'bf16'
    _default_compute = {'fp32': COMPUTE_FP32, 'bf16': COMPUTE_BF16, 'bf16x3': COMPUTE_BF16X3, COMPUTE_FP32: COMPUTE_FP32,
                        COMPUTE_BF16: COMPUTE_BF16, COMPUTE_BF16X3: COMPUTE_BF16X3}[kind]


def get_compute():
    return {COMPUTE_FP32: 'fp32', COMPUTE_BF16: 'bf16', COMPUTE_BF16X3: 'bf16x3'}[_default_compute]


def mixed():
    return _mixed


def compute_name():
    return 'mixed' if _mixed else get_compute()

EXPORTS = [
    'ess_last_error', 'ess_version', 'ess_conv2d_plan', 'ess_conv2d_pack_weights', 'ess_conv2d_pack_rows',
    'ess_conv2d_forward', 'ess_to_bf16_c8', 'ess_conv2d_wgrad_workspace', 'ess_conv2d_wgrad', 'ess_conv2d_wgrad_sets', 'ess_norm_workspace', 'ess_instnorm_forward',
    'ess_instnorm_backward', 'ess_batchnorm_train_forward', 'ess_batchnorm_train_backward',
    'ess_upsample_bilinear2x_add', 'ess_sumpool2x2', 'ess_add', 'ess_event_normalize', 'ess_task_loss_workspace',
    'ess_task_loss', 'ess_sym_js_loss', 'ess_l1_loss', 'ess_radam_step', 'ess_argmax_confusion', 'ess_resize_nearest', 'ess_conv2d_pack_weights_multi',
    'ess_voxel_grid_trilinear', 'ess_voxel_grid_trilinear_workspace', 'ess_voxel_grid_temporal', 'ess_voxel_normalize_workspace', 'ess_voxel_normalize',
    'ess_from_bf16_c8', 'ess_norm_workspace_c8', 'ess_instnorm_forward_c8', 'ess_instnorm_backward_c8', 'ess_batchnorm_train_forward_c8',
    'ess_batchnorm_train_backward_c8', 'ess_l1_loss_c8', 'ess_augment_image_label', 'ess_radam_step_dev', 'ess_upsample_bilinear2x_add_c8',
    'ess_upsample_bilinear2x_add_c8_from_c8', 'ess_add_bf16', 'ess_event_normalize_slices', 'ess_sum_scalars',
    'ess_label_confusion', 'ess_augment_perspective_filter', 'ess_tuning_set', 'ess_tuning_get', 'ess_conv2d_s2d_preferred',
    'ess_to_f16_c8', 'ess_bf16_c8_to_f16_c8', 'ess_f16_c8_to_bf16_c8', 'ess_instnorm_forward_c8_mixed', 'ess_seg_head',
    'ess_event_normalize_samples', 'ess_state_carry_masked', 'ess_state_carry_indexed',
    'ess_event_ingest_workspace', 'ess_event_ingest', 'ess_event_ingest_columns', 'ess_event_ingest_ring',
    'ess_event_ingest_columns_trilinear', 'ess_event_ingest_ring_trilinear',
]


class EssConvDesc(Structure):
    _fields_ = [(n, c_int32) for n in (
        'N', 'H_in', 'W_in', 'C0', 'C1', 'mode0', 'mode1', 'C_out', 'H_out', 'W_out', 'ksize', 'stride', 'pad',
        'epilogue', 'act', 'hidden', 'out_split', 'compute', 'fmt0', 'fmt1', 'fmt_out', 'fmt_res')]


class EssConvPlan(Structure):
    _fields_ = [('cout_tile', c_int32), ('ck', c_int32), ('n_chunks', c_int32), ('n_cout_tiles', c_int32),
                ('packed_elems', c_int64), ('packed_bytes', c_int64), ('rows_padded', c_int32), ('lds_bytes', c_int32)]


class EssHipError(RuntimeError):
    pass


_lib = None


def lib():
    global _lib
    if _lib is None:
        if not os.path.exists(LIB_PATH):
            raise EssHipError(f'{LIB_PATH} not found: build it with `python -c "import __graft_entry__ as g; g.build()"` '
                              '(hipcc --offload-arch=gfx950). ess_amd has no CPU or eager fallback.')
        L = ctypes.CDLL(LIB_PATH)
        L.ess_last_error.restype = c_char_p
        L.ess_conv2d_wgrad_workspace.restype = c_size_t
        L.ess_conv2d_wgrad_workspace.argtypes = [POINTER(EssConvDesc)]
        L.ess_task_loss_workspace.restype = c_size_t
        L.ess_task_loss_workspace.argtypes = [c_int32]
# ... 32 lines not shown
            'ess_task_loss': [P, P, P, P, F, I, I, I, I, I, I, P, c_size_t, P],
            'ess_sym_js_loss': [P, P, P, P, F, I, I, I, P, c_size_t, P],
            'ess_l1_loss': [P, P, P, P, F, I64, P, c_size_t, P],
            'ess_radam_step': [P, P, P, P, I64, F, F, F, F, F, I, P],
            'ess_argmax_confusion': [P, P, P, P, I, I, I, I, P],
            'ess_resize_nearest': [P, P, I, I, I, I, I, P],
            'ess_conv2d_pack_weights_multi': [P, P, P, P, I, P],
            'ess_voxel_grid_trilinear': [P, P, P, P, P, I64, I, I, I, I, P, P, c_size_t, I64, P],
            'ess_voxel_grid_temporal': [P, P, P, P, P, I64, I, I, I, I, I, P, P],
            'ess_voxel_normalize': [P, I, I64, I, P, c_size_t, P],
            'ess_from_bf16_c8': [P, P, I, I, I, I, P],
            'ess_instnorm_forward_c8': [P, P, P, P, I, I, I, F, I, I, P, c_size_t, P],
            'ess_instnorm_backward_c8': [P, P, P, P, I, I, I, I, I, P, c_size_t, P],
            'ess_batchnorm_train_forward_c8': [P, P, P, P, P, P, F, F, P, P, I, I, I, I, I, P, c_size_t, P],
            'ess_batchnorm_train_backward_c8': [P, P, P, P, P, P, P, P, P, P, I, I, I, I, I, I, P, c_size_t, P],
            'ess_l1_loss_c8': [P, P, P, P, F, I64, I64, P, c_size_t, P],
            'ess_to_f16_c8': [P, P, I, I, I, I, I, P],
            'ess_bf16_c8_to_f16_c8': [P, P, I64, P],
            'ess_f16_c8_to_bf16_c8': [P, P, I, I, I, I, I, P],
            'ess_instnorm_forward_c8_mixed': [P, P, P, P, P, I, I, I, F, I, I, I, P, c_size_t, P],
            'ess_augment_image_label': [P, P, P, P, P, P, I, I, I, I, I, P],
            'ess_radam_step_dev': [P, P, P, P, I64, F, F, F, P, P],
            'ess_upsample_bilinear2x_add_c8': [P, P, P, I, I, I, I, P],
            'ess_upsample_bilinear2x_add_c8_from_c8': [P, P, P, I, I, I, I, P],
            'ess_seg_head': [P, I, P, P, P, P, P, P, I, I, I, I, I, I, I, I, I, I, I, P],
            'ess_event_normalize_samples': [P, P, I, I64, P, P, P],
            'ess_state_carry_masked': [P, P, P, I, I, P, P],
            'ess_state_carry_indexed': [P, P, P, I, I, I, I, P, P, P],
            'ess_event_ingest': [P, P, I64, I, I, I, I, P, c_size_t, P, P],
            'ess_event_ingest_columns': [P, P, P, P, P, P, I64, I, I, I, I, P, c_size_t, P, P],
            'ess_event_ingest_ring': [P, P, P, P, P, P, P, P, I64, I, I, I, I, I, P, c_size_t, P, P],
            'ess_event_ingest_columns_trilinear': [P, P, P, P, P, P, I64, I, I, I, I, P, c_size_t, P, P, P, I, I, I, P],
            'ess_event_ingest_ring_trilinear': [P, P, P, P, P, P, P, P, I64, I, I, I, I, I, P, c_size_t, P, P, P, I, I, I, P],
        }
        for name, argtypes in sig.items():
            fn = getattr(L, name)
            fn.argtypes = argtypes
            fn.restype = c_int
        _lib = L
    return _lib


def _check(rc, what):
    if rc != 0:
        raise EssHipError(f'{what} failed (rc={rc}): {lib().ess_last_error().decode()}')


def stream():
    return c_void_p(torch.cuda.current_stream().cuda_stream)


def ptr(t, dtype=torch.float32, allow_none=True):
    if t is None:
        if not allow_none:
            raise EssHipError('required tensor is None')
        return c_void_p(0)
    if not t.is_cuda:
        raise EssHipError('ess_amd kernels need CUDA(HIP) tensors; there is no CPU path (got a CPU tensor)')
    if t.dtype != dtype:
        raise EssHipError(f'expected {dtype}, got {t.dtype}')
    if not t.is_contiguous():
        raise EssHipError('expected a contiguous tensor')
    return c_void_p(t.data_ptr())


_desc_cache = {}
# ... 243 lines not shown
    dres = torch.empty_like(x) if need_dres else None
    ws = workspace(lib().ess_norm_workspace(C), x.device, 'norm')
    _check(lib().ess_batchnorm_train_backward(ptr(x), ptr(y), ptr(dy), ptr(gamma), ptr(stats), ptr(dx), ptr(dres),
                                              ptr(dgamma), ptr(dbeta), int(accumulate), N, C, H * W, int(relu),
                                              c_void_p(ws.data_ptr()), c_size_t(ws.numel()), stream()),
           'ess_batchnorm_train_backward')
    return dx, dres


def instnorm_forward_c8(x, C, residual, relu, eps=1e-5, x_f16=False):
    N, CB, H, W, _ = x.shape
    y = torch.empty(x.shape, dtype=torch.bfloat16, device=x.device)
    stats = torch.empty(N * C, 2, dtype=torch.float32, device=x.device)
    L = lib()
    xdt, xf = torch.bfloat16, int(bool(x_f16))
    ws = workspace(L.ess_norm_workspace_c8(N * CB), x.device, 'norm8')
    _check(L.ess_instnorm_forward_c8(ptr(x, xdt), ptr(residual, torch.bfloat16), ptr(y, torch.bfloat16), ptr(stats), N, C,
                                     H * W, c_float(eps), int(relu), xf, c_void_p(ws.data_ptr()), c_size_t(ws.numel()), stream()),
           'ess_instnorm_forward_c8')
    return y, stats


def instnorm_backward_c8(x, C, dy, stats, relu, x_f16=False):
    N, CB, H, W, _ = x.shape
    if int(x_f16) == 2:
        CB //= 2
    dx = torch.empty(N, CB, H, W, 8, dtype=torch.bfloat16, device=x.device)
    L = lib()
    xdt, xf = x.dtype, int(x_f16)
    ws = workspace(L.ess_norm_workspace_c8(N * CB), x.device, 'norm8')
    _check(L.ess_instnorm_backward_c8(ptr(x, xdt), ptr(dy, torch.bfloat16), ptr(stats), ptr(dx, torch.bfloat16), N, C, H * W,
                                      int(relu), xf, c_void_p(ws.data_ptr()), c_size_t(ws.numel()), stream()), 'ess_instnorm_backward_c8')
    return dx


def batchnorm_train_forward_c8(x, C, residual, gamma, beta, running_mean, running_var, momentum, eps, relu, x_f16=False):
    N, CB, H, W, _ = x.shape
    y = torch.empty(x.shape, dtype=torch.bfloat16, device=x.device)
    stats = torch.empty(2, C, 2, dtype=torch.float32, device=x.device)
    L = lib()
    xdt, xf = torch.bfloat16, int(bool(x_f16))
    ws = workspace(L.ess_norm_workspace_c8(CB), x.device, 'norm8')
    _check(L.ess_batchnorm_train_forward_c8(ptr(x, xdt), ptr(residual, torch.bfloat16), ptr(gamma), ptr(beta),
                                            ptr(running_mean), ptr(running_var), c_float(momentum), c_float(eps),
                                            ptr(y, torch.bfloat16), ptr(stats), N, C, H * W, int(relu), xf, c_void_p(ws.data_ptr()),
                                            c_size_t(ws.numel()), stream()), 'ess_batchnorm_train_forward_c8')
    return y, stats


def batchnorm_train_backward_c8(x, C, y, dy, gamma, stats, relu, need_dx=True, need_dres=False, dgamma=None, dbeta=None,
                                accumulate=False, x_f16=False, beta=None):
    if stats.numel() != 4 * C:
        raise EssHipError(f'batchnorm_train_backward_c8: stats must be the forward\'s [2, C, 2] tensor, got {tuple(stats.shape)}')
    N, CB, H, W, _ = x.shape
    dx = torch.empty(x.shape, dtype=torch.bfloat16, device=x.device) if need_dx else None
    dres = torch.empty(x.shape, dtype=torch.bfloat16, device=x.device) if need_dres else None
    L = lib()
    xdt, xf = torch.bfloat16, int(bool(x_f16))
    ws = workspace(L.ess_norm_workspace_c8(CB), x.device, 'norm8')
    _check(L.ess_batchnorm_train_backward_c8(ptr(x, xdt), ptr(y, torch.bfloat16), ptr(dy, torch.bfloat16), ptr(gamma), ptr(beta),
                                             ptr(stats), ptr(dx, torch.bfloat16), ptr(dres, torch.bfloat16), ptr(dgamma), ptr(dbeta),
                                             int(accumulate), N, C, H * W, int(relu), xf, c_void_p(ws.data_ptr()), c_size_t(ws.numel()),
                                             stream()), 'ess_batchnorm_train_backward_c8')
    return dx, dres


# ... 496 lines not shown
NORM_SPLIT_BY_PLANE = 1 << 30


def tuning_set(key, value):
    _check(lib().ess_tuning_set(key.encode(), int(value)), 'ess_tuning_set')


def tuning_get(key):
    v = c_int32(0)
    _check(lib().ess_tuning_get(key.encode(), byref(v)), 'ess_tuning_get')
    return v.value


def label_confusion(pred, labels, conf, ignore_index=255):
    if pred.shape != labels.shape or pred.dtype != torch.int64 or labels.dtype != torch.int64:
        raise EssHipError(f'label_confusion: int64 tensors of one shape expected, got {pred.dtype}{tuple(pred.shape)} / {labels.dtype}{tuple(labels.shape)}')
    if pred.numel():
        _check(lib().ess_label_confusion(ptr(pred, torch.int64), ptr(labels, torch.int64), ptr(conf, torch.int64),
                                         c_int64(pred.numel()), conf.shape[0], int(ignore_index), stream()), 'ess_label_confusion')
    return conf


def argmax_confusion(logits, labels=None, conf=None, ignore_index=255, want_pred=True):
    N, K, H, W = logits.shape
    pred = torch.empty(N, H, W, dtype=torch.int64, device=logits.device) if want_pred else None
    _check(lib().ess_argmax_confusion(ptr(logits), ptr(labels, torch.int64), ptr(pred, torch.int64), ptr(conf, torch.int64),
                                      N, K, H * W, int(ignore_index), stream()), 'ess_argmax_confusion')
    return pred


SEG_HEAD_MAX_K = 64


def seg_head(x, C, weight, bias, out_hw=None, window=None, palette=None, want_confidence=False):
    if not torch.is_tensor(x) or not x.is_cuda:
        raise EssHipError('seg_head: x must be a CUDA(HIP) tensor; there is no CPU path')
    if x.dim() == 5 and x.shape[-1] == 8 and x.dtype in (torch.bfloat16, torch.float16):
        fmt = FMT_F16_C8 if (x.dtype == torch.float16 or is_f16_c8(x)) else FMT_BF16_C8
        N, nb, H, W, _ = x.shape
        if not 0 < C <= nb * 8:
            raise EssHipError(f'seg_head: C={C} channels do not fit the source\'s {nb} blocks of 8')
        if nb != (C + 7) // 8:
            raise EssHipError(f'seg_head: C={C} channels need {(C + 7) // 8} blocks of 8, x has {nb}')
    elif x.dim() == 4 and x.dtype == torch.float32:
        fmt = FMT_F32_NCHW
        N, Cx, H, W = x.shape
        if Cx != C:
            raise EssHipError(f'seg_head: C={C} but x has {Cx} channels')
    else:
        raise EssHipError(f'seg_head: x must be fp32 NCHW, BF16_C8 or F16_C8, got {x.dtype}{tuple(x.shape)}')
    if weight.dim() == 4 and weight.shape[2:] == (1, 1):
        weight = weight.view(weight.shape[0], weight.shape[1])
    if weight.dim() != 2 or weight.shape[1] != C:
        raise EssHipError(f'seg_head: weight must be [K, C={C}], got {tuple(weight.shape)}')
    K = weight.shape[0]
    if not 0 < K <= SEG_HEAD_MAX_K:
        raise EssHipError(f'seg_head: weight has K={K} classes, at most {SEG_HEAD_MAX_K} are supported')
    if bias is None or tuple(bias.shape) != (K,):
        raise EssHipError(f'seg_head: bias must be [K={K}], got {None if bias is None else tuple(bias.shape)}')
    if palette is not None and (not torch.is_tensor(palette) or palette.dtype != torch.uint8 or tuple(palette.shape) != (K, 3)):
        got = f'{palette.dtype}{tuple(palette.shape)}' if torch.is_tensor(palette) else type(palette).__name__
        raise EssHipError(f'seg_head: palette must be a uint8 [K={K}, 3] tensor, got {got}')
    y0, x0, h, w = (0, 0, H, W) if window is None else (int(v) for v in window)
    if y0 < 0 or x0 < 0 or h <= 0 or w <= 0 or y0 + h > H or x0 + w > W:
        raise EssHipError(f'seg_head: window {(y0, x0, h, w)} leaves the {H} x {W} source plane')
    Ho, Wo = (h, w) if out_hw is None else (int(out_hw[0]), int(out_hw[1]))
    if Ho <= 0 or Wo <= 0:
        raise EssHipError(f'seg_head: out_hw {(Ho, Wo)} is empty')
    dev = x.device
    labels = torch.empty(N, Ho, Wo, dtype=torch.uint8, device=dev)
    colour = torch.empty(N, Ho, Wo, 3, dtype=torch.uint8, device=dev) if palette is not None else None
    conf = torch.empty(N, Ho, Wo, dtype=torch.float32, device=dev) if want_confidence else None
    _check(lib().ess_seg_head(ptr(x, x.dtype, allow_none=False), fmt, ptr(weight.detach(), allow_none=False), ptr(bias.detach(), allow_none=False),
                              ptr(palette, torch.uint8), ptr(labels, torch.uint8), ptr(colour, torch.uint8), ptr(conf), N, C, K, H, W,
                              y0, x0, h, w, Ho, Wo, stream()), 'ess_seg_head')
    return labels, colour, conf


def f16_blocks_empty(N, C, H, W, device, hilo=False):
    return torch.empty(N, ((C + 7) // 8) * (2 if hilo else 1), H, W, 8, dtype=torch.float16, device=device)


def h16_of(t):
    return copies.of(t).h16


def attach_h16(t, h16, hilo=False):
    return copies.attach(t, h16=(h16, bool(hilo)))


def to_f16_c8(x, hilo=False):
    N, C, H, W = x.shape
    y = f16_blocks_empty(N, C, H, W, x.device, hilo)
    _check(lib().ess_to_f16_c8(ptr(x), ptr(y, torch.float16), N, C, H, W, int(bool(hilo)), stream()), 'ess_to_f16_c8')
    return y


def bf16_c8_to_f16_c8(x):
    y = torch.empty(x.shape, dtype=torch.float16, device=x.device)
    _check(lib().ess_bf16_c8_to_f16_c8(ptr(x, torch.bfloat16), ptr(y, torch.float16), x.numel() // 8, stream()), 'ess_bf16_c8_to_f16_c8')
    return y


def f16_c8_to_bf16_c8(x, hilo=False):
    N, nb, H, W, _ = x.shape
# ... 43 lines not shown
```

ess_amd/models/style_networks.py:

```python
import torch
import torch.nn as nn

from .. import functional as Fn
from .. import copies, hip
from .submodules import InterpolationLayer


def gaussian_weights_init(m):
    if m.__class__.__name__.find('Conv') == 0:
        m.weight.data.normal_(0.0, 0.02)


class ReLUINSConv2d(nn.Module):

    def __init__(self, n_in, n_out, kernel_size, stride, padding=0):
        super().__init__()
        self.model = nn.Sequential(nn.Conv2d(n_in, n_out, kernel_size=kernel_size, stride=stride, padding=padding, bias=True),
                                   nn.InstanceNorm2d(n_out, affine=False), nn.ReLU(inplace=True))
        self.model.apply(gaussian_weights_init)

    def forward_fused(self, x, skip=None, up=False):
        c = self.model[0]
        pre = Fn.pre_norm_fmt() if hip.is_c8(x) else None
        y = Fn.conv2d(x, c.weight, c.bias, c.stride[0], c.padding[0], x1=skip,
                      mode0=hip.SRC_NEAREST_UP2 if up else hip.SRC_DIRECT, out_c8=pre, half=True)
        return Fn.instance_norm(y, None, True, self.model[1].eps, x_f16=pre == Fn.PRE_NORM)

    def forward(self, x):
        return self.forward_fused(x)


class INSResBlock(nn.Module):

    def conv3x3(self, inplanes, out_planes, stride=1):
        return [nn.Conv2d(inplanes, out_planes, kernel_size=3, stride=stride, padding=1)]

    def __init__(self, inplanes, planes, stride=1, dropout=0.0):
        super().__init__()
        if dropout > 0:
            raise NotImplementedError('INSResBlock dropout is never enabled by SemSegE2VID')
        layers = self.conv3x3(inplanes, planes, stride) + [nn.InstanceNorm2d(planes), nn.ReLU(inplace=True)]
        layers += self.conv3x3(planes, planes) + [nn.InstanceNorm2d(planes)]
        self.model = nn.Sequential(*layers)
        self.model.apply(gaussian_weights_init)

    def forward(self, x, first=False):
        c1, c2 = self.model[0], self.model[3]
        pre = Fn.pre_norm_fmt() if hip.is_c8(x) else None
        pre1 = pre
        if first and pre == Fn.PRE_NORM and Fn.mixed() and c1.out_channels % 64 == 0:
            pre1 = Fn.PRE_NORM_HILO
        y, skip = Fn.conv2d_passthrough(x, c1.weight, c1.bias, c1.stride[0], 1, out_c8=pre1, half=True)
        if copies.of(skip).h16 is None:
            copies.carry(skip, x, 'h16')
        y = Fn.instance_norm(y, None, True, self.model[1].eps, x_f16=pre == Fn.PRE_NORM)
        y = Fn.conv2d(y, c2.weight, c2.bias, 1, 1, out_c8=pre, half=True)
        return Fn.instance_norm(y, skip, False, self.model[4].eps, x_f16=pre == Fn.PRE_NORM)


# ... 7 lines not shown
            raise ValueError("skip_connect=True only works with skip_type='concat' (decoder_scale_2 is built for "
                             "2x channels, reference :25)")
        self.skip_connect, self.skip_type, self.input_index_map = skip_connect, skip_type, input_index_map
        self.index_coords = None
        tch = input_c
        if skip_connect:
            blocks = [INSResBlock(tch, tch) for _ in range(5)]
            blocks += [ReLUINSConv2d(tch, tch // 2, kernel_size=3, stride=1, padding=1)]
            self.decoder_scale_1 = nn.Sequential(*blocks)
            self.decoder_scale_2 = nn.Sequential(ReLUINSConv2d(tch, tch // 2, kernel_size=3, stride=1, padding=1),
                                                 ReLUINSConv2d(tch // 2, tch // 4, kernel_size=3, stride=1, padding=1))
            tch //= 2
            self.decoder_scale_3 = nn.Sequential(ReLUINSConv2d(tch, tch // 2, kernel_size=3, stride=1, padding=1),
                                                 ReLUINSConv2d(tch // 2, tch // 2, kernel_size=3, stride=1, padding=1))
            tch //= 2
            self.decoder_scale_4 = nn.Sequential(ReLUINSConv2d(tch, tch // 2, kernel_size=3, stride=1, padding=1))
            tch //= 2
        else:
            self.decoder_scale_1 = nn.Sequential(*[INSResBlock(tch, tch) for _ in range(3)])
            for name in ('decoder_scale_2', 'decoder_scale_3', 'decoder_scale_4'):
                setattr(self, name, nn.Sequential(InterpolationLayer(scale_factor=2, mode='nearest'),
                                                  ReLUINSConv2d(tch, tch // 2, kernel_size=3, stride=1, padding=1)))
                tch //= 2
        self.decoder_scale_5 = nn.Sequential(nn.Conv2d(tch, output_c, kernel_size=1, stride=1, padding=0))

    def update_skip_dict(self, skips, x, sz_in):
        rem, scale = sz_in % x.shape[3], sz_in // x.shape[3]
        assert rem == 0
        skips[scale] = x

    def forward(self, input_dict):
        sz_in = input_dict[1].shape[3]
        out = {8: input_dict[8]}
        x = self._trunk(input_dict, out, sz_in)
        c5 = self.decoder_scale_5[0]
        x = Fn.conv2d(x, c5.weight, c5.bias, 1, 0, out_c8=False, half=True)
        self.update_skip_dict(out, x, sz_in)
        return out

    def _trunk(self, input_dict, out, sz_in):
        x = input_dict[8]
        c8 = Fn.c8_mode()
        lat = (lambda t, deep=False: Fn.as_c8(t, want_hilo=deep).contiguous()) if c8 else (lambda t, deep=False: t.contiguous())
        x = lat(x, True)

        def record(x):
            if out is None:
                return x
            x, xo = Fn.fork(x)
            self.update_skip_dict(out, xo, sz_in)
            return x

        if self.skip_connect:
            x = self.decoder_scale_1[0](x, first=True)
            for blk in list(self.decoder_scale_1)[1:]:
                x = blk(x)
            x = self.decoder_scale_2[0].forward_fused(x, lat(input_dict[4]), up=True)
            x = record(self.decoder_scale_2[1](x))
            x = self.decoder_scale_3[0].forward_fused(x, lat(input_dict[2]), up=True)
            x = record(self.decoder_scale_3[1](x))
            x = self.decoder_scale_4[0].forward_fused(x, None, up=True)
        else:
            x = self.decoder_scale_1[0](x, first=True)
            for blk in list(self.decoder_scale_1)[1:]:
                x = blk(x)
            x = record(self.decoder_scale_2[1].forward_fused(x, None, up=True))
            x = record(self.decoder_scale_3[1].forward_fused(x, None, up=True))
            x = self.decoder_scale_4[1].forward_fused(x, None, up=True)
        return x

    def predict(self, input_dict, out_hw=None, window=None, palette=None, want_confidence=False):
        with torch.no_grad():
            x = self._trunk(input_dict, None, input_dict[1].shape[3])
            c5 = self.decoder_scale_5[0]
            if hip.is_c8(x):
                C = x.shape[1] * 8
                if hip.mixed():
                    h, hilo = Fn.half_of(x)
                    if hilo:
                        raise hip.EssHipError('SemSegE2VID.predict: the last activation came as a [hi | lo] half pair')
                    x = h
            else:
                C = x.shape[1]
            return hip.seg_head(x.contiguous(), C, c5.weight, c5.bias, out_hw=out_hw, window=window, palette=palette,
                                want_confidence=want_confidence)


_PENDING_BN_COUNTERS = []


def flush_bn_counters():
    if _PENDING_BN_COUNTERS:
        with torch.no_grad():
            torch._foreach_add_(_PENDING_BN_COUNTERS, 1)
        _PENDING_BN_COUNTERS.clear()


class _ConvBN(nn.Module):

    @staticmethod
    def run(conv, bn, x, residual=None, relu=True, passthrough=False):
        out_c8 = Fn.c8_mode()
        if bn.training:
            pre = Fn.pre_norm_fmt()
            if passthrough:
                y, skip = Fn.Conv2dFn.apply(x, None, conv.weight, None, conv.stride[0], conv.padding[0], hip.SRC_DIRECT,
                                            hip.SRC_DIRECT, True, pre)
# ... 126 lines not shown
```

include/ess_hip.h:

```cpp
#ifndef ESS_HIP_H
#define ESS_HIP_H

#include <stddef.h>
#include <stdint.h>

#ifdef __cplusplus
extern "C" {
#endif

typedef void* ess_stream_t;

enum { ESS_OK = 0, ESS_EINVAL = -22, ESS_ENOTSUP = -95, ESS_ELAUNCH = -5 };

enum { ESS_SRC_DIRECT = 0, ESS_SRC_NEAREST_UP2 = 1, ESS_SRC_ZERO_UP2 = 2,
       ESS_SRC_S2D = 3  };
enum {
  ESS_EPI_LINEAR = 0,
  ESS_EPI_LSTM = 1,
  ESS_EPI_GRU_UR = 2,
  ESS_EPI_GRU_OUT = 3
};
enum { ESS_ACT_NONE = 0, ESS_ACT_RELU = 1, ESS_ACT_SIGMOID = 2, ESS_ACT_TANH = 3, ESS_ACT_SUMPOOL2 = 4 };
enum { ESS_COMPUTE_FP32 = 0, ESS_COMPUTE_BF16 = 1,
       ESS_COMPUTE_BF16X3 = 2,
       ESS_COMPUTE_F16 = 3 };
enum { ESS_FMT_F32_NCHW = 0, ESS_FMT_BF16_C8 = 1, ESS_FMT_F16_C8 = 3, ESS_FMT_F16_C8_HILO = 4,
       ESS_FMT_F32_C8 = 2  };
enum { ESS_GRU_U_F32 = 0, ESS_GRU_U_F16 = 1 };
enum { ESS_LSTM_H_HILO = 1 };
enum { ESS_GRU_H_HILO = 2 };
enum {
  ESS_W_CONV = 0,
  ESS_W_TRANSPOSED = 1,
  ESS_W_ROWS = 2,
  ESS_W_CONV5_S2D = 3
};

typedef struct EssConvDesc {
  int32_t N;
  int32_t H_in, W_in;
  int32_t C0, C1;
  int32_t mode0, mode1;
  int32_t C_out, H_out, W_out;
  int32_t ksize, stride, pad;
  int32_t epilogue;
  int32_t act;
  int32_t hidden;
  int32_t out_split;
  int32_t compute;
  int32_t fmt0, fmt1;
  int32_t fmt_out;
  int32_t fmt_res;
} EssConvDesc;

typedef struct EssConvPlan {
  int32_t cout_tile;
  int32_t ck;
  int32_t n_chunks, n_cout_tiles;
  int64_t packed_elems;
  int64_t packed_bytes;
  int32_t rows_padded;
  int32_t lds_bytes;
} EssConvPlan;

const char* ess_last_error(void);
int ess_version(void);

int ess_conv2d_plan(const EssConvDesc* d, EssConvPlan* plan);

int ess_conv2d_s2d_preferred(const EssConvDesc* d);

int ess_conv2d_pack_weights(const EssConvDesc* d, int w_kind, const float* w, const float* w2,
                            void* packed, ess_stream_t stream);
int ess_conv2d_pack_weights_multi(const EssConvDesc* descs, const int32_t* w_kinds, const float* const* w,
                                  void* const* packed, int32_t count, ess_stream_t stream);

int ess_conv2d_pack_rows(const EssConvDesc* d, const float* v, const float* v2, float fill,
                         float* packed, ess_stream_t stream);

int ess_conv2d_forward(const EssConvDesc* d, const void* src0, const void* src1, const void* packed_w,
                       const float* scale, const float* shift, const void* residual, const float* aux0,
                       const float* aux1, void* out, void* out2, void* out_bf16, ess_stream_t stream);

int ess_to_bf16_c8(const float* x, void* y, int32_t N, int32_t C, int32_t H, int32_t W, ess_stream_t stream);
int ess_from_bf16_c8(const void* x, float* y, int32_t N, int32_t C, int32_t H, int32_t W, ess_stream_t stream);
int ess_to_f16_c8(const float* x, void* y, int32_t N, int32_t C, int32_t H, int32_t W, int32_t hilo, ess_stream_t stream);
int ess_bf16_c8_to_f16_c8(const void* x, void* y, int64_t n_vec, ess_stream_t stream);
int ess_f16_c8_to_bf16_c8(const void* x, void* y, int32_t N, int32_t C, int32_t H, int32_t W, int32_t hilo, ess_stream_t stream);

size_t ess_conv2d_wgrad_workspace(const EssConvDesc* d);
int ess_conv2d_wgrad(const EssConvDesc* d, const void* src0, const void* src1, const void* dy,
                     float* dw, float* db, int accumulate, void* workspace, size_t workspace_bytes,
                     ess_stream_t stream);
int ess_conv2d_wgrad_sets(const EssConvDesc* d, int32_t n_sets, const void* const* src0, const void* const* src1,
                          const void* const* dy, float* dw, float* db, int32_t accumulate, void* workspace,
                          size_t workspace_bytes, ess_stream_t stream);

size_t ess_norm_workspace(int32_t groups);
int ess_instnorm_forward(const float* x, const float* residual, float* y, float* stats, int32_t planes,
                         int32_t hw, float eps, int32_t relu, void* workspace, size_t workspace_bytes,
                         ess_stream_t stream);
int ess_instnorm_backward(const float* x, const float* dy, const float* stats, float* dx, int32_t planes,
                          int32_t hw, int32_t relu, void* workspace, size_t workspace_bytes, ess_stream_t stream);

size_t ess_norm_workspace_c8(int32_t groups);
int ess_instnorm_forward_c8(const void* x, const void* residual, void* y, float* stats, int32_t N, int32_t C, int32_t hw,
                            float eps, int32_t relu, int32_t x_f16, void* workspace, size_t workspace_bytes, ess_stream_t stream);
int ess_instnorm_forward_c8_mixed(const void* x, const void* residual, void* y, void* y16, float* stats, int32_t N, int32_t C, int32_t hw,
                                  float eps, int32_t relu, int32_t x_fmt, int32_t res_f16, void* workspace, size_t workspace_bytes,
                                  ess_stream_t stream);
int ess_instnorm_backward_c8(const void* x, const void* dy, const float* stats, void* dx, int32_t N, int32_t C, int32_t hw,
                             int32_t relu, int32_t x_f16, void* workspace, size_t workspace_bytes, ess_stream_t stream);
int ess_batchnorm_train_forward_c8(const void* x, const void* residual, const float* gamma, const float* beta,
                                   float* running_mean, float* running_var, float momentum, float eps, void* y, float* stats,
                                   int32_t N, int32_t C, int32_t hw, int32_t relu, int32_t x_f16, void* workspace,
                                   size_t workspace_bytes, ess_stream_t stream);
int ess_batchnorm_train_backward_c8(const void* x, const void* y, const void* dy, const float* gamma, const float* beta,
                                    const float* stats, void* dx, void* d_residual, float* dgamma, float* dbeta, int32_t accumulate,
                                    int32_t N, int32_t C, int32_t hw, int32_t relu, int32_t x_f16, void* workspace,
                                    size_t workspace_bytes, ess_stream_t stream);

int ess_batchnorm_train_forward(const float* x, const float* residual, const float* gamma, const float* beta,
                                float* running_mean, float* running_var, float momentum, float eps, float* y,
                                float* stats, int32_t N, int32_t C, int32_t hw, int32_t relu, void* workspace,
                                size_t workspace_bytes, ess_stream_t stream);
int ess_batchnorm_train_backward(const float* x, const float* y, const float* dy, const float* gamma,
                                 const float* stats, float* dx, float* d_residual, float* dgamma, float* dbeta,
                                 int32_t accumulate, int32_t N, int32_t C, int32_t hw, int32_t relu,
                                 void* workspace, size_t workspace_bytes, ess_stream_t stream);

int ess_upsample_bilinear2x_add(const float* a, const float* b, float* y, int32_t planes, int32_t H,
                                int32_t W, ess_stream_t stream);
int ess_upsample_bilinear2x_add_c8(const float* a, const float* b, void* y, int32_t N, int32_t C, int32_t H, int32_t W,
                                   ess_stream_t stream);

int ess_upsample_bilinear2x_add_c8_from_c8(const void* a, const void* b, void* y, int32_t N, int32_t C, int32_t H, int32_t W,
                                           ess_stream_t stream);
int ess_sumpool2x2(const float* x, float* y, int32_t planes, int32_t H_out, int32_t W_out, int32_t accumulate,
                   ess_stream_t stream);
int ess_add(const float* a, const float* b, float* y, int64_t n, ess_stream_t stream);
int ess_sum_scalars(const float* const* terms, int32_t n, float* out, ess_stream_t stream);
int ess_add_bf16(const void* a, const void* b, const void* c, void* y, int64_t n_vectors, ess_stream_t stream);

int ess_event_normalize(const float* x, float* y, int64_t n, void* workspace, ess_stream_t stream);
int ess_event_normalize_slices(const float* x, float* y, int32_t B, int32_t T, int64_t chunk, void* workspace, ess_stream_t stream);
// ... 49 lines not shown
int ess_augment_perspective_filter(const float* img, const int64_t* label, const float* params, const int64_t* id_lut,
                                   float* scratch, float* out_img, int64_t* out_label, int32_t N, int32_t H, int32_t W,
                                   ess_stream_t stream);

size_t ess_task_loss_workspace(int32_t K);
int ess_task_loss(const float* logits, const int64_t* labels, float* loss, float* dlogits, float loss_scale,
                  int32_t N, int32_t K, int32_t hw, int32_t ignore_index, int32_t use_dice, int32_t use_ce,
                  void* workspace, size_t workspace_bytes, ess_stream_t stream);
#define ESS_LOSS_WORKSPACE_BYTES (8 * (1 + 2048))
int ess_sym_js_loss(const float* a, const float* b, float* loss, float* da, float loss_scale, int32_t N,
                    int32_t K, int32_t hw, void* workspace, size_t workspace_bytes, ess_stream_t stream);
int ess_l1_loss(const float* a, const float* b, float* loss, float* da, float loss_scale, int64_t n,
                void* workspace, size_t workspace_bytes, ess_stream_t stream);

int ess_l1_loss_c8(const void* a, const void* b, float* loss, void* da, float loss_scale, int64_t n_vectors, int64_t n,
                   void* workspace, size_t workspace_bytes, ess_stream_t stream);

int ess_radam_step(float* p, const float* g, float* exp_avg, float* exp_avg_sq, int64_t n, float lr,
                   float beta1, float beta2, float eps, float step_size, int32_t n_sma_ge5,
                   ess_stream_t stream);

int ess_radam_step_dev(float* p, const float* g, float* exp_avg, float* exp_avg_sq, int64_t n, float beta1, float beta2,
                       float eps, const float* hyper, ess_stream_t stream);

int ess_resize_nearest(const float* x, float* y, int32_t planes, int32_t H_in, int32_t W_in, int32_t H_out,
                       int32_t W_out, ess_stream_t stream);

int ess_argmax_confusion(const float* logits, const int64_t* labels, int64_t* pred_lbl, int64_t* conf,
                         int32_t N, int32_t K, int32_t hw, int32_t ignore_index, ess_stream_t stream);

int ess_seg_head(const void* x, int32_t fmt, const float* weight, const float* bias, const uint8_t* palette, uint8_t* labels,
                 uint8_t* colour, float* confidence, int32_t N, int32_t C, int32_t K, int32_t H, int32_t W, int32_t win_y0,
                 int32_t win_x0, int32_t win_h, int32_t win_w, int32_t H_out, int32_t W_out, ess_stream_t stream);

int ess_label_confusion(const int64_t* pred_lbl, const int64_t* labels, int64_t* conf, int64_t total, int32_t K,
                        int32_t ignore_index, ess_stream_t stream);

#define ESS_NORM_SPLIT_BY_PLANE (1 << 30)
int ess_tuning_set(const char* key, int32_t value);
int ess_tuning_get(const char* key, int32_t* value);

#ifdef __cplusplus
}
#endif
#endif
```

Baseline: 1716.

## Fuse decoder's final instance norm + ReLU into the 1x1 head conv's loads

Adds a norm-on-load source format so the last decoder block's instance-norm + ReLU is applied while the 1x1 head convolution, its weight gradient and the segmentation head load their input, using precomputed per-channel statistics. This removes writing and re-reading the normalized activation tensor at full decoder resolution. The cost is extra unpack/normalize/repack arithmetic in the conv and wgrad load paths, a separate statistics pass, and more kernel instantiations. Backward through the fused norm must also be handled by the new Python path.

```diff
diff --git a/ess_amd/csrc/conv_bf16.hip b/ess_amd/csrc/conv_bf16.hip
--- a/ess_amd/csrc/conv_bf16.hip
+++ b/ess_amd/csrc/conv_bf16.hip
@@ -395,6 +395,8 @@
                   "conv(bf16): the generic tile kernel stages BF16_C8 sources for 1x1 and 3x3 LINEAR convolutions only");
   ESS_CHECK_ARG(key == 11 || key == 12 || key == 31 || key == 32 || key == 51 || key == 52 || key == 71 || key == 72,
                 "conv: no kernel for k%d s%d", d->ksize, d->stride);
+  if (a.src_stats)
+    ESS_CHECK_ARG(c8 && key == 11 && d->C1 == 0 && d->epilogue == ESS_EPI_LINEAR, "conv(norm-on-load source): no kernel for this form");
   conv_bf16_launch_generic(key, mb, pl.ck / 8, d->epilogue, c8, grid, pl.lds_bytes, st, a);
   return ess_launch_status("conv2d_forward(bf16)");
 }
diff --git a/ess_amd/csrc/conv_bf16_generic.hip b/ess_amd/csrc/conv_bf16_generic.hip
--- a/ess_amd/csrc/conv_bf16_generic.hip
+++ b/ess_amd/csrc/conv_bf16_generic.hip
@@ -4,9 +4,10 @@
 
 using namespace essconv;
 
-template <int KS, int S, int MB, int EPI, int CB8, bool SRCBF = false, bool H = false>
+template <int KS, int S, int MB, int EPI, int CB8, bool SRCBF = false, bool H = false, bool NORM = false>
 __global__ __launch_bounds__(256) void conv_bf16_kernel(const ConvKArgs a) {
   static_assert(!H || SRCBF, "half operands come as F16_C8 tensors");
+  static_assert(!NORM || (SRCBF && KS == 1 && S == 1), "norm-on-load sources: C8 tensors through the 1x1 / stride-1 instantiations");
   extern __shared__ __attribute__((aligned(16))) u32x4 smem16[];
   constexpr int COT = MB * 32;
   constexpr int CK = CB8 * 8;
@@ -106,6 +107,13 @@
       const unsigned blk_ok = ((first ? c0 : c0 - a.C0) >> 3) < (first ? nb0 : nb1) ? 0xffffffffu : 0u;
       const unsigned m = (first ? v_k0[k] : v_k1[k]) & blk_ok;
       u32x4 v = r.d;
+      if constexpr (NORM) {
+        const int cc = c0 < a.C0 ? c0 : a.C0 - 8;
+        float f[8];
+        ess_unpack8_c8(v, a.src_f16, f);
+        ess_norm_map8(f, a.src_stats + 2 * ((size_t)n * a.C0 + cc), a.src_relu);
+        v = H ? pack8h(f) : pack8(f);
+      }
       v[0] &= m; v[1] &= m; v[2] &= m; v[3] &= m;
       return v;
     } else {
@@ -218,9 +226,24 @@
   ess_allow_lds(conv_bf16_kernel<KS, S, MB, ESS_EPI_LINEAR, CB8, true>, lds);
   hipLaunchKernelGGL((conv_bf16_kernel<KS, S, MB, ESS_EPI_LINEAR, CB8, true>), grid, dim3(256), lds, st, a);
 }
+template <int MB, int CB8>
+void launch_c8_norm(dim3 grid, size_t lds, hipStream_t st, const ConvKArgs& a) {
+  if (a.f16) {
+    ess_allow_lds(conv_bf16_kernel<1, 1, MB, ESS_EPI_LINEAR, CB8, true, true, true>, lds);
+    hipLaunchKernelGGL((conv_bf16_kernel<1, 1, MB, ESS_EPI_LINEAR, CB8, true, true, true>), grid, dim3(256), lds, st, a);
+    return;
+  }
+  ess_allow_lds(conv_bf16_kernel<1, 1, MB, ESS_EPI_LINEAR, CB8, true, false, true>, lds);
+  hipLaunchKernelGGL((conv_bf16_kernel<1, 1, MB, ESS_EPI_LINEAR, CB8, true, false, true>), grid, dim3(256), lds, st, a);
+}
 template <int KS, int S>
 void launch_mb_c8(int mb, int cb8, dim3 grid, size_t lds, hipStream_t st, const ConvKArgs& a) {
   if constexpr (KS == 1 && S == 1) {
+    if (a.src_stats) {
+      if (cb8 == 4) { if (mb == 2) launch_c8_norm<2, 4>(grid, lds, st, a); else launch_c8_norm<1, 4>(grid, lds, st, a); }
+      else { if (mb == 2) launch_c8_norm<2, 2>(grid, lds, st, a); else launch_c8_norm<1, 2>(grid, lds, st, a); }
+      return;
+    }
     if (cb8 == 4) {
       if (mb == 2) launch_c8<KS, S, 2, 4>(grid, lds, st, a);
       else launch_c8<KS, S, 1, 4>(grid, lds, st, a);
diff --git a/ess_amd/csrc/conv_common.h b/ess_amd/csrc/conv_common.h
--- a/ess_amd/csrc/conv_common.h
+++ b/ess_amd/csrc/conv_common.h
@@ -1,5 +1,6 @@
 #pragma once
 #include "common.h"
+#include "norm_on_load.h"
 #include <stdlib.h>
 
 #ifndef ESS_EPI_AUX
@@ -43,6 +44,9 @@
   int deep;
   int f16;
   int hilo;
+  const float* src_stats;
+  int src_relu;
+  int src_f16;
 };
 
 template <bool H> __device__ __forceinline__ uint2 ess_cvt4(float v0, float v1, float v2, float v3);
@@ -1362,6 +1366,13 @@
 
 inline int validate(const EssConvDesc* d) {
   ESS_CHECK_ARG(d != nullptr, "conv: null descriptor");
+  if (d->fmt0 & ~ESS_FMT_BASE_MASK) {
+    ESS_CHECK_NORM_SRC(d, "conv");
+    ESS_CHECK_ARG(d->compute == ESS_COMPUTE_BF16 || d->compute == ESS_COMPUTE_F16, "conv(norm-on-load source): bf16 or half operands only");
+    EssConvDesc c = *d;
+    c.fmt0 = c.fmt1 = d->compute == ESS_COMPUTE_F16 ? ESS_FMT_F16_C8 : ESS_FMT_BF16_C8;
+    return validate(&c);
+  }
   if (d->compute == ESS_COMPUTE_F16) {
     ESS_CHECK_ARG(d->fmt0 != ESS_FMT_BF16_C8 && d->fmt1 != ESS_FMT_BF16_C8 && d->fmt_out != ESS_FMT_BF16_C8 && d->fmt_res != ESS_FMT_BF16_C8,
                   "conv(f16): 16-bit tensors of a half-operand convolution are ESS_FMT_F16_C8");
diff --git a/ess_amd/csrc/conv_fwd.hip b/ess_amd/csrc/conv_fwd.hip
--- a/ess_amd/csrc/conv_fwd.hip
+++ b/ess_amd/csrc/conv_fwd.hip
@@ -213,11 +213,23 @@
   return ess_launch_status("pack_rows");
 }
 
-extern "C" int ess_conv2d_forward(const EssConvDesc* d, const void* src0, const void* src1, const void* packed_w,
-                                  const float* scale, const float* shift, const void* residual, const float* aux0,
-                                  const float* aux1, void* out, void* out2, void* out_bf16, ess_stream_t stream) {
-  EssConvDesc dcopy;
+static int conv2d_forward_run(const EssConvDesc* d, const void* src0, const void* src1, const void* packed_w,
+                              const float* scale, const float* shift, const void* residual, const float* aux0,
+                              const float* aux1, void* out, void* out2, void* out_bf16, const float* src_stats, ess_stream_t stream) {
+  EssConvDesc dcopy, ncopy;
   bool out_f16 = false;
+  int norm_fmt = 0;
+  if (d && (d->fmt0 & ~ESS_FMT_BASE_MASK)) {
+    int rc = validate(d);
+    if (rc) return rc;
+    ESS_CHECK_NORM_PTRS(src0, src_stats, "conv");
+    norm_fmt = d->fmt0;
+    ncopy = *d;
+    ncopy.fmt0 = ncopy.fmt1 = d->compute == ESS_COMPUTE_F16 ? ESS_FMT_F16_C8 : ESS_FMT_BF16_C8;
+    d = &ncopy;
+  } else {
+    ESS_CHECK_ARG(!src_stats, "conv: stats given for a source that is not ESS_FMT_NORM_ON_LOAD");
+  }
   if (d && d->fmt_out == ESS_FMT_F16_C8 && d->compute != ESS_COMPUTE_F16) {
     ESS_CHECK_ARG(d->act != ESS_ACT_SUMPOOL2 && d->out_split == 0 && (d->fmt_res == ESS_FMT_F32_NCHW || d->fmt_res == ESS_FMT_BF16_C8),
                   "conv: an F16_C8 output takes no SUMPOOL2 / out_split; a residual comes as BF16_C8");
@@ -269,6 +281,9 @@
   a.split = rd.split ? 1 : 0;
   a.f16 = rd.f16 ? 1 : 0;
   a.hilo = rd.hilo ? 1 : 0;
+  a.src_stats = src_stats;
+  a.src_relu = (norm_fmt & ESS_FMT_NORM_RELU) ? 1 : 0;
+  a.src_f16 = (norm_fmt & ESS_FMT_BASE_MASK) == ESS_FMT_F16_C8 ? 1 : 0;
   if (rd.hilo && d->epilogue == ESS_EPI_LINEAR)
     ESS_CHECK_ARG(!residual && (d->C_out % pl.cout_tile) == 0 && d->fmt_out == ESS_FMT_BF16_C8, "conv(f16): a [hi | lo] output takes no residual and whole channel tiles");
   if (rd.hilo && d->epilogue == ESS_EPI_GRU_OUT)
@@ -284,6 +299,7 @@
   a.ck = pl.ck; a.n_chunks = pl.n_chunks; a.act = d->act; a.hid = d->hidden; a.out_split = d->out_split;
   hipStream_t st = (hipStream_t)stream;
   if (is_bf16(d)) return conv_bf16_launch(d, pl, g, a, st);
+  ESS_CHECK_ARG(!src_stats, "conv(norm-on-load source): bf16 or half operands only");
   ESS_CHECK_ARG(g.IH * g.IW <= kpc32(d->ksize, d->stride) * 256, "conv: input tile of %d positions exceeds the staging capacity",
                 g.IH * g.IW);
   ESS_CHECK_ARG((int64_t)(d->C0 > d->C1 ? d->C0 : d->C1) * d->H_in * d->W_in * 4 < (int64_t)1 << 31,
@@ -304,3 +320,17 @@
   }
   return ess_launch_status("conv2d_forward");
 }
+
+extern "C" int ess_conv2d_forward(const EssConvDesc* d, const void* src0, const void* src1, const void* packed_w,
+                                  const float* scale, const float* shift, const void* residual, const float* aux0,
+                                  const float* aux1, void* out, void* out2, void* out_bf16, ess_stream_t stream) {
+  ESS_CHECK_ARG(!d || !(d->fmt0 & ~ESS_FMT_BASE_MASK), "conv: a norm-on-load source goes through ess_conv2d_forward_norm_src (it needs the statistics)");
+  return conv2d_forward_run(d, src0, src1, packed_w, scale, shift, residual, aux0, aux1, out, out2, out_bf16, nullptr, stream);
+}
+
+extern "C" int ess_conv2d_forward_norm_src(const EssConvDesc* d, const void* src0, const float* stats, const void* packed_w,
+                                           const float* scale, const float* shift, void* out, ess_stream_t stream) {
+  ESS_CHECK_ARG(d != nullptr, "conv: null descriptor");
+  ESS_CHECK_ARG(d->fmt0 & ESS_FMT_NORM_ON_LOAD, "conv(norm-on-load source): fmt0 does not carry ESS_FMT_NORM_ON_LOAD");
+  return conv2d_forward_run(d, src0, nullptr, packed_w, scale, shift, nullptr, nullptr, nullptr, out, nullptr, nullptr, stats, stream);
+}
diff --git a/ess_amd/csrc/conv_wgrad.hip b/ess_amd/csrc/conv_wgrad.hip
--- a/ess_amd/csrc/conv_wgrad.hip
+++ b/ess_amd/csrc/conv_wgrad.hip
@@ -818,8 +818,20 @@
   return tm;
 }
 
+inline EssConvDesc norm_src_plain(const EssConvDesc* d) {
+  EssConvDesc c = *d;
+  c.fmt0 = c.fmt1 = ESS_FMT_BF16_C8;
+  return c;
+}
+
 int wvalidate(const EssConvDesc* d) {
   ESS_CHECK_ARG(d != nullptr, "wgrad: null descriptor");
+  if (d->fmt0 & ~ESS_FMT_BASE_MASK) {
+    ESS_CHECK_NORM_SRC(d, "wgrad");
+    ESS_CHECK_ARG(d->fmt_out == ESS_FMT_F32_NCHW, "wgrad(norm-on-load source): the 1x1 head's form only (fp32 NCHW dY)");
+    const EssConvDesc c = norm_src_plain(d);
+    return wvalidate(&c);
+  }
   ESS_CHECK_ARG(d->epilogue == ESS_EPI_LINEAR && d->out_split == 0, "wgrad: only plain convolutions have a weight gradient here");
   ESS_CHECK_ARG(d->mode0 >= ESS_SRC_DIRECT && d->mode0 <= ESS_SRC_ZERO_UP2 && d->mode1 >= ESS_SRC_DIRECT && d->mode1 <= ESS_SRC_ZERO_UP2,
                 "wgrad: source modes DIRECT / NEAREST_UP2 / ZERO_UP2 only (the space-to-depth form exists for the frozen encoder's forward)");
@@ -863,6 +875,12 @@
 WPlan wplan(const EssConvDesc* desc) {
   WPlan w{};
   w.d = *desc;
+  if (desc->fmt0 & ESS_FMT_NORM_ON_LOAD) {
+    w.d = norm_src_plain(desc);
+    w.args.w.x_norm = 1;
+    w.args.w.x_relu = (desc->fmt0 & ESS_FMT_NORM_RELU) ? 1 : 0;
+    w.args.w.x_f16 = (desc->fmt0 & ESS_FMT_BASE_MASK) == ESS_FMT_F16_C8 ? 1 : 0;
+  }
   if (desc->compute == ESS_COMPUTE_BF16X3) {
     w.args.split = k3s1p1(desc);
     w.d.compute = w.args.split ? ESS_COMPUTE_BF16 : ESS_COMPUTE_FP32;
@@ -920,12 +938,13 @@
   return w;
 }
 
-struct WgradSet { const void* x0; const void* x1; const void* dy; };
+struct WgradSet { const void* x0; const void* x1; const void* dy; const float* stats = nullptr; };
 
 WgradBArgs wfill(const WPlan& w, const WgradSet& s, void* workspace, bool bias, int ph) {
   WgradBArgs b = w.args;
   WgradArgs& a = b.w;
   a.src0 = (const float*)s.x0; a.src1 = a.C1 ? (const float*)s.x1 : nullptr; a.dy = (const float*)s.dy;
+  a.x_stats = s.stats;
   a.ws = (float*)workspace;
   a.ws_b = bias ? a.ws + (size_t)a.nsplit * w.d.ksize * w.d.ksize * a.Cout * (a.C0 + a.C1) : nullptr;
   a.pp = ph >> 1; a.pq = ph & 1;
@@ -1021,6 +1040,8 @@
     ESS_CHECK_ARG(sets[q].x0 && sets[q].dy, "wgrad: null pointer");
     ESS_CHECK_ARG(d->C1 == 0 || sets[q].x1, "wgrad: second source missing");
     bits |= (uintptr_t)sets[q].x0 | (uintptr_t)sets[q].dy | (d->C1 ? (uintptr_t)sets[q].x1 : 0);
+    if (d->fmt0 & ESS_FMT_NORM_ON_LOAD) ESS_CHECK_NORM_PTRS(sets[q].x0, sets[q].stats, "wgrad");
+    else ESS_CHECK_ARG(!sets[q].stats, "wgrad: stats given for a source that is not ESS_FMT_NORM_ON_LOAD");
   }
   if (split_via_c8(d)) {
     for (int q = 0; q < n_sets; ++q)
@@ -1032,6 +1053,7 @@
   ESS_CHECK_ARG(w.lds_bytes <= 160 * 1024, "wgrad: LDS tile %d B too large", w.lds_bytes);
   if (w.d.fmt0 == ESS_FMT_BF16_C8 || w.d.fmt_out == ESS_FMT_BF16_C8)
     ESS_CHECK_ARG((bits & 15) == 0, "wgrad: BF16_C8 tensors must be 16-byte aligned");
+  ESS_CHECK_ARG(!w.args.w.x_norm || w.route == W_SMALL1X1_C8X, "wgrad(norm-on-load source): no kernel for this form");
   if (w.route == W_TAPS7) {
     ESS_CHECK_ARG(w.d.stride == 2, "wgrad: 7x7 stem variant is stride 2 only");
     ESS_CHECK_ARG(!db, "wgrad: the stem variant has no bias gradient");
@@ -1087,7 +1109,16 @@
 
 extern "C" int ess_conv2d_wgrad(const EssConvDesc* d, const void* src0, const void* src1, const void* dy, float* dw, float* db,
                                 int accumulate, void* workspace, size_t workspace_bytes, ess_stream_t stream) {
+  ESS_CHECK_ARG(!d || !(d->fmt0 & ~ESS_FMT_BASE_MASK), "wgrad: a norm-on-load source goes through ess_conv2d_wgrad_norm_src (it needs the statistics)");
   const WgradSet s{src0, src1, dy};
+  return wgrad_run(d, 1, &s, 1, dw, db, accumulate, workspace, workspace_bytes, (hipStream_t)stream);
+}
+
+extern "C" int ess_conv2d_wgrad_norm_src(const EssConvDesc* d, const void* src0, const float* stats, const void* dy, float* dw, float* db,
+                                         int accumulate, void* workspace, size_t workspace_bytes, ess_stream_t stream) {
+  ESS_CHECK_ARG(d != nullptr, "wgrad: null descriptor");
+  ESS_CHECK_ARG(d->fmt0 & ESS_FMT_NORM_ON_LOAD, "wgrad(norm-on-load source): fmt0 does not carry ESS_FMT_NORM_ON_LOAD");
+  const WgradSet s{src0, nullptr, dy, stats};
   return wgrad_run(d, 1, &s, 1, dw, db, accumulate, workspace, workspace_bytes, (hipStream_t)stream);
 }
 
@@ -1095,6 +1126,7 @@
                                      const void* const* dy, float* dw, float* db, int32_t accumulate, void* workspace,
                                      size_t workspace_bytes, ess_stream_t stream) {
   ESS_CHECK_ARG(d && src0 && dy && n_sets >= 1 && n_sets <= 3, "wgrad_sets: 1 to 3 sets");
+  ESS_CHECK_ARG(!(d->fmt0 & ~ESS_FMT_BASE_MASK), "wgrad_sets: no norm-on-load form");
   WgradSet sets[3];
   for (int q = 0; q < n_sets; ++q) {
     ESS_CHECK_ARG(src0[q] && dy[q] && (d->C1 == 0 || (src1 && src1[q])), "wgrad_sets: null tensor in set %d", q);
diff --git a/ess_amd/csrc/conv_wgrad_c8.hip b/ess_amd/csrc/conv_wgrad_c8.hip
--- a/ess_amd/csrc/conv_wgrad_c8.hip
+++ b/ess_amd/csrc/conv_wgrad_c8.hip
@@ -489,10 +489,12 @@
   ESS_TR(37);
 }
 
+template <bool NORM>
 __global__ __launch_bounds__(256) void wgrad_small1x1_c8_kernel(const WgradArgs a, int chunks_per_img, int total_chunks) {
   constexpr int P = 128, PP = P + 1;
   __shared__ float dy_s[32 * PP];
   __shared__ float x_s[32 * PP];
+  __shared__ float st_s[NORM ? 64 : 1];
   float* red = dy_s;
   const int tid = threadIdx.x, lane = tid & 63, wave = tid >> 6, half = lane >> 5, p = lane & 31;
   const int Cin = a.C0, Cout = a.Cout, nbi = (Cin + 7) >> 3;
@@ -505,16 +507,46 @@
   for (int chunk = blockIdx.x; chunk < total_chunks; chunk += gridDim.x) {
     const int n = chunk / chunks_per_img;
     const size_t px0 = (size_t)(chunk - n * chunks_per_img) * P;
+    u32x4w xv[NORM ? 2 : 1];
+    if constexpr (NORM) {
+      if (tid < 2 * Cin) st_s[tid] = a.x_stats[(size_t)n * 2 * Cin + tid];
+      const size_t px = px0 + (tid & (P - 1));
+#pragma unroll
+      for (int u = 0; u < 2; ++u) {
+        const int blk = (tid >> 7) + 2 * u;
+        xv[u] = ((const u32x4w*)a.src0)[((size_t)n * nbi + (blk < nbi ? blk : 0)) * HW + (px < HW ? px : HW - 1)];
+      }
+    }
     __syncthreads();
-    for (int i = tid; i < nbi * P; i += 256) {
-      const int blk = i / P, j = i - blk * P;
-      const size_t px = px0 + j;
-      const u32x4w v = ((const u32x4w*)a.src0)[((size_t)n * nbi + blk) * HW + (px < HW ? px : HW - 1)];
-      const unsigned m = px < HW ? 0xffffffffu : 0u;
-#pragma unroll
-      for (int q = 0; q < 4; ++q) {
-        x_s[(blk * 8 + 2 * q) * PP + j] = __builtin_bit_cast(float, (v[q] << 16) & m);
-        x_s[(blk * 8 + 2 * q + 1) * PP + j] = __builtin_bit_cast(float, v[q] & 0xffff0000u & m);
+    if constexpr (NORM) {
+      const int j = tid & (P - 1);
+      const unsigned m = px0 + j < HW ? 0xffffffffu : 0u;
+#pragma unroll
+      for (int u = 0; u < 2; ++u) {
+        const int blk = (tid >> 7) + 2 * u;
+        if (blk < nbi) {
+          float f[8];
+          ess_unpack8_c8(xv[u], a.x_f16, f);
+          ess_norm_map8(f, st_s + blk * 16, a.x_relu);
+          const u32x4w v = cvt8(f);
+#pragma unroll
+          for (int q = 0; q < 4; ++q) {
+            x_s[(blk * 8 + 2 * q) * PP + j] = __builtin_bit_cast(float, (v[q] << 16) & m);
+            x_s[(blk * 8 + 2 * q + 1) * PP + j] = __builtin_bit_cast(float, v[q] & 0xffff0000u & m);
+          }
+        }
+      }
+    } else {
+      for (int i = tid; i < nbi * P; i += 256) {
+        const int blk = i / P, j = i - blk * P;
+        const size_t px = px0 + j;
+        const u32x4w v = ((const u32x4w*)a.src0)[((size_t)n * nbi + blk) * HW + (px < HW ? px : HW - 1)];
+        const unsigned m = px < HW ? 0xffffffffu : 0u;
+#pragma unroll
+        for (int q = 0; q < 4; ++q) {
+          x_s[(blk * 8 + 2 * q) * PP + j] = __builtin_bit_cast(float, (v[q] << 16) & m);
+          x_s[(blk * 8 + 2 * q + 1) * PP + j] = __builtin_bit_cast(float, v[q] & 0xffff0000u & m);
+        }
       }
     }
     for (int i = tid; i < Cout * P; i += 256) {
@@ -572,7 +604,8 @@
 
 int wgrad_small1x1_c8_launch(const WgradArgs& a, int nsplit, hipStream_t st) {
   const int per_img = ceil_div(a.Hout * a.Wout, 128);
-  hipLaunchKernelGGL(wgrad_small1x1_c8_kernel, dim3(nsplit), dim3(256), 0, st, a, per_img, a.N * per_img);
+  if (a.x_norm) hipLaunchKernelGGL(wgrad_small1x1_c8_kernel<true>, dim3(nsplit), dim3(256), 0, st, a, per_img, a.N * per_img);
+  else hipLaunchKernelGGL(wgrad_small1x1_c8_kernel<false>, dim3(nsplit), dim3(256), 0, st, a, per_img, a.N * per_img);
   return ess_launch_status("conv2d_wgrad(1x1 head, BF16_C8)");
 }
 
diff --git a/ess_amd/csrc/conv_wgrad_common.h b/ess_amd/csrc/conv_wgrad_common.h
--- a/ess_amd/csrc/conv_wgrad_common.h
+++ b/ess_amd/csrc/conv_wgrad_common.h
@@ -1,5 +1,6 @@
 #pragma once
 #include "common.h"
+#include "norm_on_load.h"
 
 struct WgradArgs {
   const float* src0;
@@ -14,6 +15,8 @@
   int ci_tiles, npairs, nsplit;
   int dy_c8;
   int ps, pp, pq;
+  const float* x_stats;
+  int x_norm, x_relu, x_f16;
 };
 
 constexpr unsigned OOBW = 0x80000000u;
diff --git a/ess_amd/csrc/norm_c8.hip b/ess_amd/csrc/norm_c8.hip
--- a/ess_amd/csrc/norm_c8.hip
+++ b/ess_amd/csrc/norm_c8.hip
@@ -445,28 +445,40 @@
   for (int jj = 0; jj < 8; ++jj) { t0[jj] = tot[2 * jj]; t1[jj] = tot[2 * jj + 1]; }
 }
 
+__device__ __forceinline__ void in_finalize8(const double* sums, int g, int nsl, int hw, float eps, float (&mean)[8], float (&rstd)[8]) {
+  double t0[8], t1[8];
+  group_total8(sums, g, nsl, t0, t1);
+#pragma unroll
+  for (int j = 0; j < 8; ++j) {
+    const double m = t0[j] / hw;
+    double var = t1[j] / hw - m * m;
+    if (var < 0) var = 0;
+    mean[j] = (float)m;
+    rstd[j] = (float)(1.0 / sqrt(var + (double)eps));
+  }
+}
+__device__ __forceinline__ void in_store_stats8(float* __restrict__ stats, int n, int cb, int C, const float (&mean)[8], const float (&rstd)[8]) {
+#pragma unroll
+  for (int j = 0; j < 8; ++j)
+    if (cb * 8 + j < C) { stats[2 * ((size_t)n * C + cb * 8 + j)] = mean[j]; stats[2 * ((size_t)n * C + cb * 8 + j) + 1] = rstd[j]; }
+}
+
+__global__ __launch_bounds__(256) void in_stats_c8_kernel(float* __restrict__ stats, const double* sums, int nsl, int CB, int C, int hw, float eps) {
+  const int g = blockIdx.x, n = g / CB, cb = g - n * CB;
+  float mean[8], rstd[8];
+  in_finalize8(sums, g, nsl, hw, eps, mean, rstd);
+  if (threadIdx.x == 0) in_store_stats8(stats, n, cb, C, mean, rstd);
+}
+
 __global__ __launch_bounds__(256) void in_apply_c8_kernel(const u32x4n* __restrict__ x, const u32x4n* __restrict__ res,
                                                           u32x4n* __restrict__ y, float* __restrict__ stats, const double* sums,
                                                           int nsl, int CB, int C, int hw, float eps, int relu) {
   const int xf16 = relu >> 8;
   relu &= 0xff;
   const int g = blockIdx.x, n = g / CB, cb = g - n * CB;
-  double t0[8], t1[8];
-  group_total8(sums, g, nsl, t0, t1);
   float mean[8], rstd[8];
-#pragma unroll
-  for (int j = 0; j < 8; ++j) {
-    const double m = t0[j] / hw;
-    double var = t1[j] / hw - m * m;
-    if (var < 0) var = 0;
-    mean[j] = (float)m;
-    rstd[j] = (float)(1.0 / sqrt(var + (double)eps));
-  }
-  if (blockIdx.y == 0 && threadIdx.x == 0) {
-#pragma unroll
-    for (int j = 0; j < 8; ++j)
-      if (cb * 8 + j < C) { stats[2 * ((size_t)n * C + cb * 8 + j)] = mean[j]; stats[2 * ((size_t)n * C + cb * 8 + j) + 1] = rstd[j]; }
-  }
+  in_finalize8(sums, g, nsl, hw, eps, mean, rstd);
+  if (blockIdx.y == 0 && threadIdx.x == 0) in_store_stats8(stats, n, cb, C, mean, rstd);
   const size_t base = (size_t)g * hw;
   constexpr int U = 4;
   const int stride = gridDim.y * 256;
@@ -502,22 +514,9 @@
                                                               const double* sums, int nsl, int CB, int C, int hw, float eps, int flags) {
   const int relu = flags & 1, xf16 = (flags >> 8) & 1, rf16 = (flags >> 9) & 1, hilo = (flags >> 10) & 1, rpair = (flags >> 11) & 1;
   const int g = blockIdx.x, n = g / CB, cb = g - n * CB;
-  double t0[8], t1[8];
-  group_total8(sums, g, nsl, t0, t1);
   float mean[8], rstd[8];
-#pragma unroll
-  for (int j = 0; j < 8; ++j) {
-    const double m = t0[j] / hw;
-    double var = t1[j] / hw - m * m;
-    if (var < 0) var = 0;
-    mean[j] = (float)m;
-    rstd[j] = (float)(1.0 / sqrt(var + (double)eps));
-  }
-  if (blockIdx.y == 0 && threadIdx.x == 0) {
-#pragma unroll
-    for (int j = 0; j < 8; ++j)
-      if (cb * 8 + j < C) { stats[2 * ((size_t)n * C + cb * 8 + j)] = mean[j]; stats[2 * ((size_t)n * C + cb * 8 + j) + 1] = rstd[j]; }
-  }
+  in_finalize8(sums, g, nsl, hw, eps, mean, rstd);
+  if (blockIdx.y == 0 && threadIdx.x == 0) in_store_stats8(stats, n, cb, C, mean, rstd);
   const size_t base = (size_t)g * hw;
   const size_t xbase = hilo ? ((size_t)n * 2 * CB + cb) * hw : base, xlo = xbase + (size_t)CB * hw;
   const size_t rbase = rpair ? ((size_t)n * 2 * CB + cb) * hw : base;
@@ -853,6 +852,31 @@
   hipLaunchKernelGGL(in_apply_c8_mix_kernel, dim3(groups, chunks_for8(groups, hw)), dim3(256), 0, st, xs, rs, ys, hs, stats,
                      (const double*)workspace, nsl, CB, C, hw, eps, flags | (x_fmt == 2 ? 0x400 : 0));
   return ess_launch_status("instnorm_forward_c8_mixed(split)");
+}
+
+static bool in_split_path(int groups, int hw, bool mixed) {
+  if (hw <= 256 * MAXV) return false;
+  return mixed || !(hw <= 1024 * 19 && groups >= in1024_min_groups());
+}
+extern "C" int ess_instnorm_c8_split_path(int32_t N, int32_t C, int32_t hw, int32_t mixed) {
+  return N > 0 && C > 0 && hw > 0 && in_split_path(N * ((C + 7) / 8), hw, mixed != 0) ? 1 : 0;
+}
+
+extern "C" int ess_instnorm_stats_c8(const void* x, float* stats, int32_t N, int32_t C, int32_t hw, float eps, int32_t x_f16, int32_t mixed,
+                                     void* workspace, size_t workspace_bytes, ess_stream_t stream) {
+  ESS_CHECK_ARG(x && stats && N > 0 && C > 0 && hw > 0, "instnorm_stats_c8: bad arguments");
+  ESS_CHECK_ARG(x_f16 == 0 || x_f16 == 1, "instnorm_stats_c8: x_f16 is 0 (BF16_C8) or 1 (F16_C8); a [hi | lo] pair has no statistics-only form");
+  ESS_CHECK_ARG(al16(x), "instnorm_stats_c8: C8 tensors must be 16-byte aligned");
+  const int CB = (C + 7) / 8, groups = N * CB;
+  ESS_CHECK_ARG(in_split_path(groups, hw, mixed != 0), "instnorm_stats_c8: a plane of %d pixels (%d groups) takes a fused kernel, whose statistics these are not", hw, groups);
+  int rc = need_ws(workspace, ess_norm_workspace_c8(groups), workspace_bytes, "instnorm_stats_c8");
+  if (rc) return rc;
+  hipStream_t st = (hipStream_t)stream;
+  const int nsl = split_for8(groups, hw);
+  hipLaunchKernelGGL((c8_reduce_kernel<0>), dim3(groups, nsl), dim3(256), 0, st, (const u32x4n*)x, nullptr, nullptr, nullptr, (double*)workspace, hw, 1,
+                     0, CB, C, 1, x_f16 ? 0x100 : 0, 0);
+  hipLaunchKernelGGL(in_stats_c8_kernel, dim3(groups), dim3(256), 0, st, stats, (const double*)workspace, nsl, CB, C, hw, eps);
+  return ess_launch_status("instnorm_stats_c8");
 }
 
 extern "C" int ess_instnorm_backward_c8(const void* x, const void* dy, const float* stats, void* dx, int32_t N, int32_t C,
diff --git a/ess_amd/csrc/norm_on_load.h b/ess_amd/csrc/norm_on_load.h
--- /dev/null
+++ b/ess_amd/csrc/norm_on_load.h
@@ -0,0 +1,51 @@
+#pragma once
+#include "common.h"
+
+#define ESS_CHECK_NORM_SRC(d_, who_)                                                                                                   \
+  do {                                                                                                                                 \
+    const int base_ = (d_)->fmt0 & ESS_FMT_BASE_MASK;                                                                                  \
+    ESS_CHECK_ARG(((d_)->fmt0 & ~(ESS_FMT_BASE_MASK | ESS_FMT_NORM_ON_LOAD | ESS_FMT_NORM_RELU)) == 0 &&                              \
+                      (base_ == ESS_FMT_BF16_C8 || base_ == ESS_FMT_F16_C8),                                                           \
+                  who_ "(norm-on-load source): the pre-norm tensor is ESS_FMT_BF16_C8 or ESS_FMT_F16_C8");                              \
+    ESS_CHECK_ARG((d_)->ksize == 1 && (d_)->stride == 1 && (d_)->pad == 0, who_ "(norm-on-load source): ksize 1, stride 1, pad 0 only (got k%d s%d p%d)", \
+                  (d_)->ksize, (d_)->stride, (d_)->pad);                                                                               \
+    ESS_CHECK_ARG((d_)->C1 == 0 && (d_)->mode0 == ESS_SRC_DIRECT, who_ "(norm-on-load source): one direct source only (no second source, no upsampling)"); \
+    ESS_CHECK_ARG((d_)->epilogue == ESS_EPI_LINEAR, who_ "(norm-on-load source): LINEAR epilogue only");                                \
+    ESS_CHECK_ARG((d_)->C0 > 0 && ((d_)->C0 % 8) == 0, who_ "(norm-on-load source): C0 = %d is not a multiple of 8", (d_)->C0);         \
+  } while (0)
+
+#define ESS_CHECK_NORM_PTRS(x_, stats_, who_)                                                                                          \
+  do {                                                                                                                                 \
+    ESS_CHECK_ARG((x_) != nullptr && (((uintptr_t)(x_)) & 15) == 0, who_ "(norm-on-load source): the pre-norm tensor must be non-null and 16-byte aligned"); \
+    ESS_CHECK_ARG((stats_) != nullptr, who_ "(norm-on-load source): stats is null");                                                    \
+    ESS_CHECK_ARG((((uintptr_t)(stats_)) & 7) == 0, who_ "(norm-on-load source): stats must be 8-byte aligned ((mean, rstd) pairs)");    \
+  } while (0)
+
+#ifdef __HIPCC__
+typedef unsigned int ess_u32x4 __attribute__((ext_vector_type(4)));
+
+__device__ __forceinline__ void ess_unpack8_c8(ess_u32x4 v, int x_f16, float (&f)[8]) {
+  typedef _Float16 f16x2 __attribute__((ext_vector_type(2)));
+#pragma unroll
+  for (int q = 0; q < 4; ++q) {
+    const unsigned w = v[q];
+    if (x_f16) {
+      const f16x2 h = __builtin_bit_cast(f16x2, w);
+      f[2 * q] = (float)h[0];
+      f[2 * q + 1] = (float)h[1];
+    } else {
+      f[2 * q] = __builtin_bit_cast(float, w << 16);
+      f[2 * q + 1] = __builtin_bit_cast(float, w & 0xffff0000u);
+    }
+  }
+}
+
+__device__ __forceinline__ void ess_norm_map8(float (&f)[8], const float* st, int relu) {
+#pragma unroll
+  for (int j = 0; j < 8; ++j) {
+    float t = (f[j] - st[2 * j]) * st[2 * j + 1];
+    if (relu) t = fmaxf(t, 0.f);
+    f[j] = t;
+  }
+}
+#endif
diff --git a/ess_amd/csrc/seg_head.hip b/ess_amd/csrc/seg_head.hip
--- a/ess_amd/csrc/seg_head.hip
+++ b/ess_amd/csrc/seg_head.hip
@@ -1,4 +1,5 @@
 #include "common.h"
+#include "norm_on_load.h"
 
 namespace {
 
@@ -14,6 +15,8 @@
   uint8_t* colour;
   float* conf;
   int N, C, K, Hs, Ws, y0, x0, h, w_, Ho, Wo;
+  const float* stats;
+  int x_relu, x_f16;
 };
 
 template <int FMT>
@@ -36,13 +39,17 @@
   return fmaf(p, e * 0.693147181f, p);
 }
 
-template <int FMT, int KM>
+template <int FMT, int KM, bool NORM = false>
 __global__ __launch_bounds__(256) void seg_head_kernel(const SegHeadArgs a) {
+  static_assert(!NORM || FMT != ESS_FMT_F32_NCHW, "a norm-on-load source is a C8 tensor");
   extern __shared__ float lds[];
   const int CB = (a.C + 7) >> 3, CP = CB * 8;
   float* lw = lds;
   float* lb = lds + KM * CP;
   uint8_t* lp = (uint8_t*)(lb + KM);
+  float* ls = (float*)(lp + SH_PALETTE_BYTES);
+  if constexpr (NORM)
+    for (int i = threadIdx.x; i < a.N * a.C * 2; i += blockDim.x) ls[i] = a.stats[i];
   for (int i = threadIdx.x; i < KM * CP; i += blockDim.x) {
     const int cb = i / (KM * 8), k = (i >> 3) % KM, c = cb * 8 + (i & 7);
     lw[i] = (k < a.K && c < a.C) ? round_operand<FMT>(a.w[k * a.C + c]) : 0.f;
@@ -73,7 +80,12 @@
         for (int j = 0; j < 8; ++j) v[j] = (cb * 8 + j < a.C) ? xp[(size_t)j * plane] : 0.f;
       } else {
         const uint4 q = ((const uint4*)a.x)[(n * CB + cb) * plane + px];
-        if constexpr (FMT == ESS_FMT_BF16_C8) {
+        if constexpr (NORM) {
+          ess_unpack8_c8(__builtin_bit_cast(ess_u32x4, q), a.x_f16, v);
+          ess_norm_map8(v, ls + (n * a.C + (size_t)cb * 8) * 2, a.x_relu);
+#pragma unroll
+          for (int j = 0; j < 8; ++j) v[j] = round_operand<FMT>(v[j]);
+        } else if constexpr (FMT == ESS_FMT_BF16_C8) {
           const bf16x8 t = __builtin_bit_cast(bf16x8, q);
 #pragma unroll
           for (int j = 0; j < 8; ++j) v[j] = (float)t[j];
@@ -128,13 +140,14 @@
 
 inline int km_of(int K) { return K <= 4 ? 4 : K <= 8 ? 8 : K <= 12 ? 12 : K <= 16 ? 16 : K <= 20 ? 20 : K <= 32 ? 32 : 64; }
 inline size_t lds_of(int K, int C) { return (size_t)km_of(K) * (((C + 7) >> 3) * 8) * 4 + (size_t)km_of(K) * 4 + SH_PALETTE_BYTES; }
-
-template <int FMT>
+constexpr int SH_MAX_STATS = 2048;
+
+template <int FMT, bool NORM = false>
 int launch(const SegHeadArgs& a, hipStream_t st) {
   const size_t total = (size_t)a.N * a.Ho * a.Wo;
   const unsigned grid = wave_uniform_grid(total, 2048);
-  const size_t lds = lds_of(a.K, a.C);
-#define ESS_SH(KM_) hipLaunchKernelGGL((seg_head_kernel<FMT, KM_>), dim3(grid), dim3(256), lds, st, a)
+  const size_t lds = lds_of(a.K, a.C) + (NORM ? (size_t)a.N * a.C * 2 * 4 : 0);
+#define ESS_SH(KM_) hipLaunchKernelGGL((seg_head_kernel<FMT, KM_, NORM>), dim3(grid), dim3(256), lds, st, a)
   switch (km_of(a.K)) {
     case 4: ESS_SH(4); break;
     case 8: ESS_SH(8); break;
@@ -150,9 +163,10 @@
 
 }
 
-extern "C" int ess_seg_head(const void* x, int32_t fmt, const float* weight, const float* bias, const uint8_t* palette, uint8_t* labels,
-                            uint8_t* colour, float* confidence, int32_t N, int32_t C, int32_t K, int32_t H, int32_t W, int32_t win_y0,
-                            int32_t win_x0, int32_t win_h, int32_t win_w, int32_t H_out, int32_t W_out, ess_stream_t stream) {
+static int seg_head_run(const void* x, int32_t fmt, const float* stats, int32_t x_flags, const float* weight, const float* bias,
+                        const uint8_t* palette, uint8_t* labels, uint8_t* colour, float* confidence, int32_t N, int32_t C, int32_t K,
+                        int32_t H, int32_t W, int32_t win_y0, int32_t win_x0, int32_t win_h, int32_t win_w, int32_t H_out, int32_t W_out,
+                        ess_stream_t stream) {
   ESS_CHECK_ARG(x && weight && bias && labels, "seg_head: x, weight, bias and labels are required");
   ESS_CHECK_ARG(fmt == ESS_FMT_F32_NCHW || fmt == ESS_FMT_BF16_C8 || fmt == ESS_FMT_F16_C8, "seg_head: source format %d unsupported", fmt);
   ESS_CHECK_ARG(N > 0 && C > 0 && H > 0 && W > 0 && H_out > 0 && W_out > 0, "seg_head: bad extents N=%d C=%d H=%d W=%d H_out=%d W_out=%d", N, C,
@@ -163,9 +177,36 @@
                 "seg_head: window (%d, %d, %d, %d) leaves the %d x %d plane", win_y0, win_x0, win_h, win_w, H, W);
   ESS_CHECK_ARG(!colour || palette, "seg_head: colour needs a palette");
   ESS_CHECK_ARG(fmt == ESS_FMT_F32_NCHW || ((uintptr_t)x & 15) == 0, "seg_head: a C8 source must be 16-byte aligned");
-  SegHeadArgs a{x, weight, bias, palette, labels, colour, confidence, N, C, K, H, W, win_y0, win_x0, win_h, win_w, H_out, W_out};
+  SegHeadArgs a{x, weight, bias, palette, labels, colour, confidence, N, C, K, H, W, win_y0, win_x0, win_h, win_w, H_out, W_out,
+                stats, x_flags & 1, (x_flags >> 8) & 1};
   hipStream_t st = (hipStream_t)stream;
+  if (stats) {
+    ESS_CHECK_ARG(fmt != ESS_FMT_F32_NCHW, "seg_head(norm-on-load source): the operand type is ESS_FMT_F16_C8 or ESS_FMT_BF16_C8");
+    ESS_CHECK_ARG((C % 8) == 0, "seg_head(norm-on-load source): C = %d is not a multiple of 8", C);
+    ESS_CHECK_ARG((((uintptr_t)stats) & 7) == 0, "seg_head(norm-on-load source): stats must be 8-byte aligned ((mean, rstd) pairs)");
+    ESS_CHECK_ARG((int64_t)N * C <= SH_MAX_STATS && lds_of(K, C) + (size_t)N * C * 8 <= 64 * 1024,
+                  "seg_head(norm-on-load source): N * C = %lld statistics pairs do not fit the LDS budget (%d)", (long long)N * C, SH_MAX_STATS);
+    if (fmt == ESS_FMT_BF16_C8) return launch<ESS_FMT_BF16_C8, true>(a, st);
+    return launch<ESS_FMT_F16_C8, true>(a, st);
+  }
   if (fmt == ESS_FMT_BF16_C8) return launch<ESS_FMT_BF16_C8>(a, st);
   if (fmt == ESS_FMT_F16_C8) return launch<ESS_FMT_F16_C8>(a, st);
   return launch<ESS_FMT_F32_NCHW>(a, st);
 }
+
+extern "C" int ess_seg_head(const void* x, int32_t fmt, const float* weight, const float* bias, const uint8_t* palette, uint8_t* labels,
+                            uint8_t* colour, float* confidence, int32_t N, int32_t C, int32_t K, int32_t H, int32_t W, int32_t win_y0,
+                            int32_t win_x0, int32_t win_h, int32_t win_w, int32_t H_out, int32_t W_out, ess_stream_t stream) {
+  return seg_head_run(x, fmt, nullptr, 0, weight, bias, palette, labels, colour, confidence, N, C, K, H, W, win_y0, win_x0, win_h, win_w,
+                      H_out, W_out, stream);
+}
+
+extern "C" int ess_seg_head_norm_src(const void* x, int32_t x_f16, const float* stats, int32_t relu, int32_t fmt, const float* weight,
+                                     const float* bias, const uint8_t* palette, uint8_t* labels, uint8_t* colour, float* confidence,
+                                     int32_t N, int32_t C, int32_t K, int32_t H, int32_t W, int32_t win_y0, int32_t win_x0, int32_t win_h,
+                                     int32_t win_w, int32_t H_out, int32_t W_out, ess_stream_t stream) {
+  ESS_CHECK_ARG(stats != nullptr, "seg_head(norm-on-load source): stats is null");
+  ESS_CHECK_ARG((x_f16 == 0 || x_f16 == 1) && (relu == 0 || relu == 1), "seg_head(norm-on-load source): x_f16 and relu are 0 or 1");
+  return seg_head_run(x, fmt, stats, (relu & 1) | (x_f16 ? 0x100 : 0), weight, bias, palette, labels, colour, confidence, N, C, K, H, W,
+                      win_y0, win_x0, win_h, win_w, H_out, W_out, stream);
+}
diff --git a/ess_amd/functional.py b/ess_amd/functional.py
--- a/ess_amd/functional.py
+++ b/ess_amd/functional.py
@@ -434,7 +434,7 @@
         return d0, d1, dw, db, None, None, None, None, None, None, None
 
 
-def _weight_gradient(ctx, x0, x1, weight, dy, needw, needb):
+def _weight_gradient(ctx, x0, x1, weight, dy, needw, needb, wgrad=hip.conv_wgrad):
     spec = ctx.spec
     (N, Hv, Wv, C0, C1, mode0, mode1, Cout, k, s, p, _, _, _, _, _) = spec.key
     c8in = hip.is_c8(x0)
@@ -457,7 +457,7 @@
         else:
             if held is not None:
                 hip.conv_wgrad(held[0], held[1], held[2], held[3], weight.grad, held[5], accumulate=True)
-            hip.conv_wgrad(wspec, wx0, x1, dy, weight.grad, db_t, accumulate=True)
+            wgrad(wspec, wx0, x1, dy, weight.grad, db_t, accumulate=True)
         if GRAD_READY_HOOK is not None:
             GRAD_READY_HOOK(weight)
         return None, None
@@ -466,7 +466,7 @@
     if phases and not c8in:
         _wgrad_stride2_by_phases(x0, dy, dw, db)
     else:
-        hip.conv_wgrad(wspec, wx0, x1, dy, dw, db)
+        wgrad(wspec, wx0, x1, dy, dw, db)
     if not needw:
         dw = None
     if not needb:
@@ -549,6 +549,62 @@
     return InstanceNormFn.apply(x, residual, relu, eps, x_f16)
 
 
+def norm_on_load_applies(x):
+    if os.environ.get('ESS_NORM_ON_LOAD', '1')[:1] == '0':
+        return False
+    if not (c8_mode() and _blocked(x)) or copies.of(x).pair is not None:
+        return False
+    N, CB, H, W, _ = x.shape
+    return hip.instnorm_split_path(N, CB * 8, H * W)
+
+
+class NormReluConv1x1Fn(torch.autograd.Function):
+
+    @staticmethod
+    def forward(ctx, x, weight, bias, eps, x_f16=False):
+        x_f16 = bool(x_f16) or hip.is_f16_c8(x)
+        N, C, H, W = x.shape[0], _channels(x), x.shape[2], x.shape[3]
+        Cout = weight.shape[0]
+        if tuple(weight.shape[1:]) != (C, 1, 1):
+            raise hip.EssHipError(f'NormReluConv1x1Fn: weight must be [K, {C}, 1, 1], got {tuple(weight.shape)}')
+        spec = hip.conv_spec(N, H, W, C, 0, Cout, 1, 1, 0)
+        fspec = hip.conv_spec(N, H, W, C, 0, Cout, 1, 1, 0, compute=hip.COMPUTE_F16) if hip.mixed() else spec
+        stats = hip.instnorm_stats_c8(x, C, eps, x_f16)
+        out = torch.empty(N, Cout, H, W, dtype=torch.float32, device=x.device)
+        hip.conv_forward_norm_src(fspec, x, stats, True, x_f16, packed_weight(fspec, weight),
+                                  packed_rows(fspec, bias) if bias is not None else None, out)
+        ctx.spec, ctx.x_f16 = spec, x_f16
+        ctx.has_bias = bias is not None
+        ctx.bias_ref = weakref.ref(bias) if bias is not None else None
+        ctx.save_for_backward(x, stats, weight)
+        return out
+
+    @staticmethod
+    def backward(ctx, dy):
+        x, stats, weight = ctx.saved_tensors
+        spec = ctx.spec
+        N, C, Cout = x.shape[0], _channels(x), weight.shape[0]
+        dy = dy.contiguous()
+        needx, needw, needb = ctx.needs_input_grad[0], ctx.needs_input_grad[1], ctx.needs_input_grad[2] and ctx.has_bias
+        dx = dw = db = None
+        if needx:
+            dspec = hip.conv_spec(N, spec.H_out, spec.W_out, Cout, 0, C, 1, 1, 0)
+            g = hip.bf16_c8_empty(N, C, spec.H_out, spec.W_out, dy.device)
+            hip.conv_forward(dspec, dy, None, packed_weight(dspec, weight, kind=hip.W_TRANSPOSED), out=g, src_fmt=_fmt(dy), out_fmt=hip.FMT_BF16_C8)
+            dx = hip.instnorm_backward_c8(x, C, g, stats, True, ctx.x_f16)
+        if needw or needb:
+            def wgrad(wspec, x0, x1, dy_, dw_, db_, accumulate=False):
+                hip.conv_wgrad_norm_src(wspec, x0, stats, True, ctx.x_f16, dy_, dw_, db_, accumulate=accumulate)
+            dw, db = _weight_gradient(ctx, x, None, weight, dy, needw, needb, wgrad=wgrad)
+        return dx, dw, db, None, None
+
+
+def norm_relu_conv1x1(x, weight, bias=None, eps=1e-5, x_f16=False):
+    if norm_on_load_applies(x):
+        return NormReluConv1x1Fn.apply(x, weight, bias, eps, x_f16)
+    return conv2d(instance_norm(x, None, True, eps, x_f16=x_f16), weight, bias, 1, 0, out_c8=False, half=True)
+
+
 _MASK_FROM_X = os.environ.get('ESS_BN_MASK_FROM_X', '1') != '0'
 
 
diff --git a/ess_amd/hip.py b/ess_amd/hip.py
--- a/ess_amd/hip.py
+++ b/ess_amd/hip.py
@@ -17,6 +17,7 @@
 GRU_U_F32, GRU_U_F16 = 0, 1
 COMPUTE_FP32, COMPUTE_BF16, COMPUTE_BF16X3, COMPUTE_F16 = 0, 1, 2, 3
 FMT_F32_NCHW, FMT_BF16_C8, FMT_F32_C8, FMT_F16_C8, FMT_F16_C8_HILO = 0, 1, 2, 3, 4
+FMT_NORM_ON_LOAD, FMT_NORM_RELU = 0x10, 0x20
 LSTM_H_HILO = 1
 GRU_H_HILO = 2
 
@@ -59,6 +60,7 @@
     'ess_event_normalize_samples', 'ess_state_carry_masked', 'ess_state_carry_indexed',
     'ess_event_ingest_workspace', 'ess_event_ingest', 'ess_event_ingest_columns', 'ess_event_ingest_ring',
     'ess_event_ingest_columns_trilinear', 'ess_event_ingest_ring_trilinear',
+    'ess_instnorm_c8_split_path', 'ess_instnorm_stats_c8', 'ess_conv2d_forward_norm_src', 'ess_conv2d_wgrad_norm_src', 'ess_seg_head_norm_src',
 ]
 
 
@@ -157,6 +159,11 @@
             'ess_event_ingest_ring': [P, P, P, P, P, P, P, P, I64, I, I, I, I, I, P, c_size_t, P, P],
             'ess_event_ingest_columns_trilinear': [P, P, P, P, P, P, I64, I, I, I, I, P, c_size_t, P, P, P, I, I, I, P],
             'ess_event_ingest_ring_trilinear': [P, P, P, P, P, P, P, P, I64, I, I, I, I, I, P, c_size_t, P, P, P, I, I, I, P],
+            'ess_instnorm_c8_split_path': [I, I, I, I],
+            'ess_instnorm_stats_c8': [P, P, I, I, I, F, I, I, P, c_size_t, P],
+            'ess_conv2d_forward_norm_src': [D, P, P, P, P, P, P, P],
+            'ess_conv2d_wgrad_norm_src': [D, P, P, P, P, P, c_int, P, c_size_t, P],
+            'ess_seg_head_norm_src': [P, I, P, I, I, P, P, P, P, P, P, I, I, I, I, I, I, I, I, I, I, I, P],
         }
         for name, argtypes in sig.items():
             fn = getattr(L, name)
@@ -466,6 +473,43 @@
     _check(L.ess_instnorm_backward_c8(ptr(x, xdt), ptr(dy, torch.bfloat16), ptr(stats), ptr(dx, torch.bfloat16), N, C, H * W,
                                       int(relu), xf, c_void_p(ws.data_ptr()), c_size_t(ws.numel()), stream()), 'ess_instnorm_backward_c8')
     return dx
+
+
+def norm_src_fmt(x_f16, relu):
+    return (FMT_F16_C8 if x_f16 else FMT_BF16_C8) | FMT_NORM_ON_LOAD | (FMT_NORM_RELU if relu else 0)
+
+
+def instnorm_split_path(N, C, hw):
+    return bool(lib().ess_instnorm_c8_split_path(int(N), int(C), int(hw), int(_mixed)))
+
+
+def instnorm_stats_c8(x, C, eps=1e-5, x_f16=False):
+    N, CB, H, W, _ = x.shape
+    stats = torch.empty(N * C, 2, dtype=torch.float32, device=x.device)
+    L = lib()
+    ws = workspace(L.ess_norm_workspace_c8(N * CB), x.device, 'norm8')
+    _check(L.ess_instnorm_stats_c8(ptr(x, x.dtype), ptr(stats), N, C, H * W, c_float(eps), int(bool(x_f16)), int(_mixed),
+                                   c_void_p(ws.data_ptr()), c_size_t(ws.numel()), stream()), 'ess_instnorm_stats_c8')
+    return stats
+
+
+def conv_forward_norm_src(spec, x, stats, relu, x_f16, packed_w, shift, out):
+    desc = spec.desc_fmt(norm_src_fmt(x_f16, relu), FMT_F32_NCHW, FMT_F32_NCHW)
+    _check(lib().ess_conv2d_forward_norm_src(byref(desc), ptr(x, x.dtype, allow_none=False), ptr(stats, allow_none=False),
+                                             ptr(packed_w, torch.uint8), None, ptr(shift), ptr(out, allow_none=False), stream()),
+           'ess_conv2d_forward_norm_src')
+    return out
+
+
+def conv_wgrad_norm_src(spec, x, stats, relu, x_f16, dy, dw, db=None, accumulate=False):
+    desc = spec.desc_fmt(norm_src_fmt(x_f16, relu), FMT_F32_NCHW)
+    nbytes = lib().ess_conv2d_wgrad_workspace(byref(desc))
+    if nbytes == 0:
+        raise EssHipError('ess_conv2d_wgrad_workspace: ' + lib().ess_last_error().decode())
+    ws = workspace(nbytes, dy.device, 'wgrad')
+    _check(lib().ess_conv2d_wgrad_norm_src(byref(desc), ptr(x, x.dtype, allow_none=False), ptr(stats, allow_none=False), ptr(dy), ptr(dw),
+                                           ptr(db), int(accumulate), c_void_p(ws.data_ptr()), c_size_t(ws.numel()), stream()),
+           'ess_conv2d_wgrad_norm_src')
 
 
 def batchnorm_train_forward_c8(x, C, residual, gamma, beta, running_mean, running_var, momentum, eps, relu, x_f16=False):
@@ -1028,7 +1072,7 @@
 SEG_HEAD_MAX_K = 64
 
 
-def seg_head(x, C, weight, bias, out_hw=None, window=None, palette=None, want_confidence=False):
+def seg_head(x, C, weight, bias, out_hw=None, window=None, palette=None, want_confidence=False, norm_src=None):
     if not torch.is_tensor(x) or not x.is_cuda:
         raise EssHipError('seg_head: x must be a CUDA(HIP) tensor; there is no CPU path')
     if x.dim() == 5 and x.shape[-1] == 8 and x.dtype in (torch.bfloat16, torch.float16):
@@ -1067,6 +1111,15 @@
     labels = torch.empty(N, Ho, Wo, dtype=torch.uint8, device=dev)
     colour = torch.empty(N, Ho, Wo, 3, dtype=torch.uint8, device=dev) if palette is not None else None
     conf = torch.empty(N, Ho, Wo, dtype=torch.float32, device=dev) if want_confidence else None
+    if norm_src is not None:
+        stats, relu, op_fmt = norm_src
+        if fmt == FMT_F32_NCHW:
+            raise EssHipError('seg_head: a norm-on-load source is a C8 tensor')
+        _check(lib().ess_seg_head_norm_src(ptr(x, x.dtype, allow_none=False), int(fmt == FMT_F16_C8), ptr(stats, allow_none=False), int(bool(relu)),
+                                           int(op_fmt), ptr(weight.detach(), allow_none=False), ptr(bias.detach(), allow_none=False),
+                                           ptr(palette, torch.uint8), ptr(labels, torch.uint8), ptr(colour, torch.uint8), ptr(conf), N, C, K,
+                                           H, W, y0, x0, h, w, Ho, Wo, stream()), 'ess_seg_head_norm_src')
+        return labels, colour, conf
     _check(lib().ess_seg_head(ptr(x, x.dtype, allow_none=False), fmt, ptr(weight.detach(), allow_none=False), ptr(bias.detach(), allow_none=False),
                               ptr(palette, torch.uint8), ptr(labels, torch.uint8), ptr(colour, torch.uint8), ptr(conf), N, C, K, H, W,
                               y0, x0, h, w, Ho, Wo, stream()), 'ess_seg_head')
diff --git a/ess_amd/models/style_networks.py b/ess_amd/models/style_networks.py
--- a/ess_amd/models/style_networks.py
+++ b/ess_amd/models/style_networks.py
@@ -19,12 +19,16 @@
                                    nn.InstanceNorm2d(n_out, affine=False), nn.ReLU(inplace=True))
         self.model.apply(gaussian_weights_init)
 
-    def forward_fused(self, x, skip=None, up=False):
+    def forward_prenorm(self, x, skip=None, up=False):
         c = self.model[0]
         pre = Fn.pre_norm_fmt() if hip.is_c8(x) else None
         y = Fn.conv2d(x, c.weight, c.bias, c.stride[0], c.padding[0], x1=skip,
                       mode0=hip.SRC_NEAREST_UP2 if up else hip.SRC_DIRECT, out_c8=pre, half=True)
-        return Fn.instance_norm(y, None, True, self.model[1].eps, x_f16=pre == Fn.PRE_NORM)
+        return y, pre == Fn.PRE_NORM
+
+    def forward_fused(self, x, skip=None, up=False):
+        y, x_f16 = self.forward_prenorm(x, skip, up)
+        return Fn.instance_norm(y, None, True, self.model[1].eps, x_f16=x_f16)
 
     def forward(self, x):
         return self.forward_fused(x)
@@ -98,13 +102,16 @@
     def forward(self, input_dict):
         sz_in = input_dict[1].shape[3]
         out = {8: input_dict[8]}
-        x = self._trunk(input_dict, out, sz_in)
+        x, pending = self._trunk(input_dict, out, sz_in, on_load=torch.is_grad_enabled())
         c5 = self.decoder_scale_5[0]
-        x = Fn.conv2d(x, c5.weight, c5.bias, 1, 0, out_c8=False, half=True)
+        if pending is not None:
+            x = Fn.norm_relu_conv1x1(x, c5.weight, c5.bias, *pending)
+        else:
+            x = Fn.conv2d(x, c5.weight, c5.bias, 1, 0, out_c8=False, half=True)
         self.update_skip_dict(out, x, sz_in)
         return out
 
-    def _trunk(self, input_dict, out, sz_in):
+    def _trunk(self, input_dict, out, sz_in, on_load=False):
         x = input_dict[8]
         c8 = Fn.c8_mode()
         lat = (lambda t, deep=False: Fn.as_c8(t, want_hilo=deep).contiguous()) if c8 else (lambda t, deep=False: t.contiguous())
@@ -125,20 +132,32 @@
             x = record(self.decoder_scale_2[1](x))
             x = self.decoder_scale_3[0].forward_fused(x, lat(input_dict[2]), up=True)
             x = record(self.decoder_scale_3[1](x))
-            x = self.decoder_scale_4[0].forward_fused(x, None, up=True)
+            last = self.decoder_scale_4[0]
         else:
             x = self.decoder_scale_1[0](x, first=True)
             for blk in list(self.decoder_scale_1)[1:]:
                 x = blk(x)
             x = record(self.decoder_scale_2[1].forward_fused(x, None, up=True))
             x = record(self.decoder_scale_3[1].forward_fused(x, None, up=True))
-            x = self.decoder_scale_4[1].forward_fused(x, None, up=True)
-        return x
+            last = self.decoder_scale_4[1]
+        if on_load:
+            y, x_f16 = last.forward_prenorm(x, None, up=True)
+            if Fn.norm_on_load_applies(y):
+                return y, (last.model[1].eps, x_f16)
+            return Fn.instance_norm(y, None, True, last.model[1].eps, x_f16=x_f16), None
+        return last.forward_fused(x, None, up=True), None
 
     def predict(self, input_dict, out_hw=None, window=None, palette=None, want_confidence=False):
         with torch.no_grad():
-            x = self._trunk(input_dict, None, input_dict[1].shape[3])
+            x, pending = self._trunk(input_dict, None, input_dict[1].shape[3], on_load=True)
             c5 = self.decoder_scale_5[0]
+            if pending is not None:
+                eps, x_f16 = pending
+                C = x.shape[1] * 8
+                stats = hip.instnorm_stats_c8(x, C, eps, x_f16)
+                return hip.seg_head(x.contiguous(), C, c5.weight, c5.bias, out_hw=out_hw, window=window, palette=palette,
+                                    want_confidence=want_confidence,
+                                    norm_src=(stats, True, hip.FMT_F16_C8 if hip.mixed() else hip.FMT_BF16_C8))
             if hip.is_c8(x):
                 C = x.shape[1] * 8
                 if hip.mixed():
diff --git a/include/ess_hip.h b/include/ess_hip.h
--- a/include/ess_hip.h
+++ b/include/ess_hip.h
@@ -26,6 +26,7 @@
        ESS_COMPUTE_F16 = 3 };
 enum { ESS_FMT_F32_NCHW = 0, ESS_FMT_BF16_C8 = 1, ESS_FMT_F16_C8 = 3, ESS_FMT_F16_C8_HILO = 4,
        ESS_FMT_F32_C8 = 2  };
+enum { ESS_FMT_BASE_MASK = 15, ESS_FMT_NORM_ON_LOAD = 16, ESS_FMT_NORM_RELU = 32 };
 enum { ESS_GRU_U_F32 = 0, ESS_GRU_U_F16 = 1 };
 enum { ESS_LSTM_H_HILO = 1 };
 enum { ESS_GRU_H_HILO = 2 };
@@ -81,6 +82,8 @@
 int ess_conv2d_forward(const EssConvDesc* d, const void* src0, const void* src1, const void* packed_w,
                        const float* scale, const float* shift, const void* residual, const float* aux0,
                        const float* aux1, void* out, void* out2, void* out_bf16, ess_stream_t stream);
+int ess_conv2d_forward_norm_src(const EssConvDesc* d, const void* src0, const float* stats, const void* packed_w,
+                                const float* scale, const float* shift, void* out, ess_stream_t stream);
 
 int ess_to_bf16_c8(const float* x, void* y, int32_t N, int32_t C, int32_t H, int32_t W, ess_stream_t stream);
 int ess_from_bf16_c8(const void* x, float* y, int32_t N, int32_t C, int32_t H, int32_t W, ess_stream_t stream);
@@ -92,6 +95,8 @@
 int ess_conv2d_wgrad(const EssConvDesc* d, const void* src0, const void* src1, const void* dy,
                      float* dw, float* db, int accumulate, void* workspace, size_t workspace_bytes,
                      ess_stream_t stream);
+int ess_conv2d_wgrad_norm_src(const EssConvDesc* d, const void* src0, const float* stats, const void* dy, float* dw, float* db,
+                              int accumulate, void* workspace, size_t workspace_bytes, ess_stream_t stream);
 int ess_conv2d_wgrad_sets(const EssConvDesc* d, int32_t n_sets, const void* const* src0, const void* const* src1,
                           const void* const* dy, float* dw, float* db, int32_t accumulate, void* workspace,
                           size_t workspace_bytes, ess_stream_t stream);
@@ -111,6 +116,9 @@
                                   ess_stream_t stream);
 int ess_instnorm_backward_c8(const void* x, const void* dy, const float* stats, void* dx, int32_t N, int32_t C, int32_t hw,
                              int32_t relu, int32_t x_f16, void* workspace, size_t workspace_bytes, ess_stream_t stream);
+int ess_instnorm_c8_split_path(int32_t N, int32_t C, int32_t hw, int32_t mixed);
+int ess_instnorm_stats_c8(const void* x, float* stats, int32_t N, int32_t C, int32_t hw, float eps, int32_t x_f16, int32_t mixed,
+                          void* workspace, size_t workspace_bytes, ess_stream_t stream);
 int ess_batchnorm_train_forward_c8(const void* x, const void* residual, const float* gamma, const float* beta,
                                    float* running_mean, float* running_var, float momentum, float eps, void* y, float* stats,
                                    int32_t N, int32_t C, int32_t hw, int32_t relu, int32_t x_f16, void* workspace,
@@ -226,6 +234,10 @@
 int ess_seg_head(const void* x, int32_t fmt, const float* weight, const float* bias, const uint8_t* palette, uint8_t* labels,
                  uint8_t* colour, float* confidence, int32_t N, int32_t C, int32_t K, int32_t H, int32_t W, int32_t win_y0,
                  int32_t win_x0, int32_t win_h, int32_t win_w, int32_t H_out, int32_t W_out, ess_stream_t stream);
+int ess_seg_head_norm_src(const void* x, int32_t x_f16, const float* stats, int32_t relu, int32_t fmt, const float* weight,
+                          const float* bias, const uint8_t* palette, uint8_t* labels, uint8_t* colour, float* confidence, int32_t N,
+                          int32_t C, int32_t K, int32_t H, int32_t W, int32_t win_y0, int32_t win_x0, int32_t win_h, int32_t win_w,
+                          int32_t H_out, int32_t W_out, ess_stream_t stream);
 
 int ess_label_confusion(const int64_t* pred_lbl, const int64_t* labels, int64_t* conf, int64_t total, int32_t K,
                         int32_t ignore_index, ess_stream_t stream);
```

After: 1727 (median of 6 runs). No clear change (+0.7%).
